# anrieff/fray

Measured on AMD Instinct MI355X. Metric: Mrays/s (closest-hit + shadow rays) at 1920x1080, 64spp path trace, higher is better.
Workload: dtype f64

## Files before the change

### fray_amd/abi.py

```python
import ctypes as C

i32, u32, i64, u64, f32, f64 = C.c_int32, C.c_uint32, C.c_int64, C.c_uint64, C.c_float, C.c_double
P = C.POINTER

ABI_VERSION = 3

OK, E_ARG, E_PARSE, E_NODEVICE, E_UNSUPPORTED, E_NOMEM, E_HIP, E_CANCELLED = 0, -1, -2, -3, -4, -5, -6, -7
GEOM_PLANE, GEOM_SPHERE, GEOM_CUBE, GEOM_MESH, GEOM_CSG = range(5)
TEX_CHECKER, TEX_BITMAP, TEX_BUMP, TEX_FRESNEL = range(4)
SHADER_CONST, SHADER_LAMBERT, SHADER_PHONG, SHADER_REFL, SHADER_REFR, SHADER_LAYERED = range(6)
LIGHT_POINT, LIGHT_RECT = range(2)
MODE_PRIMARY_ID, MODE_RENDER = 0, 1
FRAME_STATS = 1
OPTION_NAMES = ("pt_lanes", "pt_budget_mib", "speculate_fans", "fused_whitted_max", "fp_contract", "seed_table_mib", "skip_null_segments",
                "segment_planes", "certified_segments")
FIGURE_NAMES = ("contracted_launches", "shadow_segments", "segment_plane_nodes", "certified_segments_eligible", "shadow_segments_certified",
                "shadow_nodes_skipped", "seed_table_bytes", "seed_launches", "seed_planes_reused", "batch_lanes", "whitted_path",
                "pt_budget_effective_mib", "scene_updates", "scene_update_bytes", "arena_bytes", "fans_filed", "fan_children",
                "fan_children_looked_up", "fans_given_up")


class Transform(C.Structure):
    _fields_ = [("offset", f64 * 3), ("m", f64 * 9), ("invM", f64 * 9)]

# ... 126 lines not shown
        return {n: getattr(self, n) for n, _ in self._fields_ if n != "rgb"}


PROGRESS_FN = C.CFUNCTYPE(C.c_int, C.c_void_p, P(Progress))


class Progressive(C.Structure):
    _fields_ = [("fn", PROGRESS_FN), ("user", C.c_void_p), ("preview_ms", f64)]


class ShadeRequest(C.Structure):
    _fields_ = [("seed", u32), ("spp", i32), ("sample_first", i32), ("rng_skip", i32), ("flags", i32), ("_pad", i32),
                ("keys", C.c_void_p)]


class Adaptive(C.Structure):
    _fields_ = [("min_spp", i32), ("_pad", i32), ("threshold", f64), ("err_floor", f64), ("rungs", i32), ("_pad2", i32),
                ("samples", u64)]


ACCUM_CHANNELS = 4


class Samples(C.Structure):
    _fields_ = [("sample_first", i32), ("sample_count", i32), ("samples_done", i32), ("_pad", i32)]


class Denoise(C.Structure):
    _fields_ = [("levels", i32), ("demodulate", i32), ("sigma_luminance", C.c_float), ("sigma_normal", C.c_float),
                ("sigma_depth", C.c_float), ("sigma_albedo", C.c_float)]


FEAT_CHANNELS = 10
MOTION_CHANNELS = 8


class View(C.Structure):
    _fields_ = [("pos", f32 * 3), ("right", f32 * 3), ("up", f32 * 3), ("front", f32 * 3), ("tan_x", C.c_float), ("tan_y", C.c_float),
                ("width", i32), ("height", i32)]


class Temporal(C.Structure):
    _fields_ = [("demodulate", i32), ("max_history", i32), ("variance_history", i32), ("alpha_min", C.c_float), ("film_offset", C.c_float),
                ("plane_tolerance", C.c_float), ("normal_min_dot", C.c_float)]


class Change(C.Structure):
    _fields_ = [("radius", i32), ("gain", C.c_float)]


HISTORY_CHANNELS = 12
HISTORY_SPLIT_CHANNELS = 20


STRUCTS = {"frayhip_transform": Transform, "frayhip_geom_ref": GeomRef, "frayhip_node": Node,
           "frayhip_plane": Plane, "frayhip_sphere": Sphere, "frayhip_cube": Cube,
           "frayhip_csg": Csg, "frayhip_triangle": Triangle, "frayhip_kdnode": KDNode,
           "frayhip_mesh": Mesh, "frayhip_texture": Texture, "frayhip_shader": Shader,
           "frayhip_layer": Layer, "frayhip_light": Light, "frayhip_camera": Camera,
           "frayhip_settings": Settings, "frayhip_environment": Environment,
           "frayhip_scene_desc": SceneDesc, "frayhip_frame": Frame, "frayhip_stats": Stats,
           "frayhip_progress": Progress, "frayhip_progressive": Progressive,
           "frayhip_shade_request": ShadeRequest, "frayhip_adaptive": Adaptive, "frayhip_samples": Samples,
           "frayhip_view": View}

VP = C.c_void_p
SYMBOLS = {
    "frayhip_scene_parse": (C.c_int, [C.c_char_p, P(VP)]),
    "frayhip_host_scene_desc": (P(SceneDesc), [VP]),
    "frayhip_host_scene_free": (None, [VP]),
    "frayhip_init": (C.c_int, [C.c_int]),
    "frayhip_scene_create": (C.c_int, [P(SceneDesc), P(VP)]),
    "frayhip_scene_destroy": (None, [VP]),
    "frayhip_scene_set_view": (C.c_int, [VP, P(Camera), P(Settings)]),
    "frayhip_scene_update": (C.c_int, [VP, P(SceneDesc)]),
    "frayhip_transform_identity": (C.c_int, [P(Transform)]),
    "frayhip_transform_scale": (C.c_int, [P(Transform), f64, f64, f64]),
    "frayhip_transform_rotate": (C.c_int, [P(Transform), f64, f64, f64]),
    "frayhip_transform_translate": (C.c_int, [P(Transform), f64, f64, f64]),
    "frayhip_light_begin_frame": (C.c_int, [P(Light)]),
    "frayhip_shader_begin_frame": (C.c_int, [P(Shader)]),
    "frayhip_scene_set_option": (C.c_int, [VP, C.c_char_p, i64]),
    "frayhip_scene_get_option": (C.c_int, [VP, C.c_char_p, P(i64)]),
    "frayhip_render": (C.c_int, [VP, P(Frame), VP, VP, VP, P(Stats)]),
    "frayhip_render_device": (C.c_int, [VP, P(Frame), VP, VP, VP, VP, P(Stats)]),
    "frayhip_render_progressive": (C.c_int, [VP, P(Frame), P(Progressive), VP, VP, VP, P(Stats)]),
    "frayhip_render_device_progressive": (C.c_int, [VP, P(Frame), P(Progressive), VP, VP, VP, VP, P(Stats)]),
    "frayhip_render_adaptive": (C.c_int, [VP, P(Frame), P(Adaptive), VP, VP, VP, P(Stats)]),
    "frayhip_render_device_adaptive": (C.c_int, [VP, P(Frame), P(Adaptive), VP, VP, VP, VP, P(Stats)]),
    "frayhip_render_samples": (C.c_int, [VP, P(Frame), P(Samples), P(Progressive), VP, VP, VP, P(Stats)]),
    "frayhip_render_samples_device": (C.c_int, [VP, P(Frame), P(Samples), P(Progressive), VP, VP, VP, VP, P(Stats)]),
    "frayhip_render_components": (C.c_int, [VP, P(Frame), P(Samples), P(Progressive), VP, VP, VP, VP, VP, VP, P(Stats)]),
    "frayhip_render_components_device": (C.c_int, [VP, P(Frame), P(Samples), P(Progressive), VP, VP, VP, VP, VP, VP, VP, P(Stats)]),
    "frayhip_render_features": (C.c_int, [VP, P(Frame), C.c_int, VP, P(Stats)]),
    "frayhip_render_features_device": (C.c_int, [VP, P(Frame), C.c_int, VP, VP, P(Stats)]),
    "frayhip_render_features_motion": (C.c_int, [VP, P(Frame), C.c_int, P(Transform), C.c_int, VP, VP, P(Stats)]),
    "frayhip_render_features_motion_device": (C.c_int, [VP, P(Frame), C.c_int, P(Transform), C.c_int, VP, VP, VP, P(Stats)]),
    "frayhip_denoise_defaults": (C.c_int, [P(Denoise)]),
    "frayhip_denoise": (C.c_int, [C.c_int, C.c_int, VP, VP, VP, P(Denoise), VP, P(Stats)]),
    "frayhip_denoise_device": (C.c_int, [C.c_int, C.c_int, VP, VP, VP, P(Denoise), VP, VP, P(Stats)]),
    "frayhip_denoise_signal": (C.c_int, [C.c_int, C.c_int, VP, VP, VP, P(Denoise), VP, P(Stats)]),
    "frayhip_denoise_signal_device": (C.c_int, [C.c_int, C.c_int, VP, VP, VP, P(Denoise), VP, VP, P(Stats)]),
    "frayhip_view_from_camera": (C.c_int, [P(Camera), C.c_int, C.c_int, P(View)]),
    "frayhip_temporal_defaults": (C.c_int, [P(Temporal)]),
    "frayhip_temporal_accumulate": (C.c_int, [C.c_int, C.c_int, VP, VP, P(View), VP, P(Temporal), VP, VP, VP, P(Stats)]),
    "frayhip_temporal_accumulate_device": (C.c_int, [C.c_int, C.c_int, VP, VP, P(View), VP, P(Temporal), VP, VP, VP, VP, P(Stats)]),
    "frayhip_temporal_accumulate_motion": (C.c_int, [C.c_int, C.c_int, VP, VP, VP, P(View), VP, P(Temporal), VP, VP, VP, P(Stats)]),
    "frayhip_temporal_accumulate_motion_device": (C.c_int, [C.c_int, C.c_int, VP, VP, VP, P(View), VP, P(Temporal), VP, VP, VP, VP, P(Stats)]),
    "frayhip_temporal_accumulate_split": (C.c_int, [C.c_int, C.c_int, VP, VP, VP, VP, P(View), VP, P(Temporal), P(Temporal), VP, VP, VP, VP, VP, P(Stats)]),
    "frayhip_temporal_accumulate_split_device": (C.c_int, [C.c_int, C.c_int, VP, VP, VP, VP, P(View), VP, P(Temporal), P(Temporal), VP, VP, VP, VP, VP, VP,
                                                           P(Stats)]),
    "frayhip_change_defaults": (C.c_int, [P(Change)]),
    "frayhip_change_frame": (C.c_int, [C.c_int, C.c_int, VP, VP, VP, P(Change), VP, P(Stats)]),
    "frayhip_change_frame_device": (C.c_int, [C.c_int, C.c_int, VP, VP, VP, P(Change), VP, VP, P(Stats)]),
    "frayhip_temporal_accumulate_adaptive": (C.c_int, [C.c_int, C.c_int, VP, VP, VP, VP, P(View), VP, P(Temporal), VP, VP, VP, P(Stats)]),
    "frayhip_temporal_accumulate_adaptive_device": (C.c_int, [C.c_int, C.c_int, VP, VP, VP, VP, P(View), VP, P(Temporal), VP, VP, VP, VP, P(Stats)]),
    "frayhip_temporal_accumulate_split_adaptive": (C.c_int, [C.c_int, C.c_int, VP, VP, VP, VP, VP, VP, P(View), VP, P(Temporal), P(Temporal), VP, VP, VP, VP,
                                                             VP, P(Stats)]),
    "frayhip_temporal_accumulate_split_adaptive_device": (C.c_int, [C.c_int, C.c_int, VP, VP, VP, VP, VP, VP, P(View), VP, P(Temporal), P(Temporal), VP, VP,
                                                                    VP, VP, VP, VP, P(Stats)]),
    "frayhip_camera_rays": (C.c_int, [VP, i64, VP, C.c_int, VP, VP]),
    "frayhip_camera_rays_device": (C.c_int, [VP, i64, VP, C.c_int, VP, VP, VP]),
    "frayhip_trace_rays": (C.c_int, [VP, i64, VP, VP, C.c_int, VP, VP, VP, P(Stats)]),
    "frayhip_trace_rays_device": (C.c_int, [VP, i64, VP, VP, C.c_int, VP, VP, VP, VP, P(Stats)]),
    "frayhip_visible": (C.c_int, [VP, i64, VP, VP, C.c_int, VP, P(Stats)]),
    "frayhip_visible_device": (C.c_int, [VP, i64, VP, VP, C.c_int, VP, VP, P(Stats)]),
    "frayhip_shade_rays": (C.c_int, [VP, i64, VP, VP, P(ShadeRequest), VP, P(Stats)]),
    "frayhip_shade_rays_device": (C.c_int, [VP, i64, VP, VP, P(ShadeRequest), VP, VP, P(Stats)]),
    "frayhip_bucket_count": (C.c_int, [C.c_int, C.c_int, C.c_int, C.c_int]),
    "frayhip_pack_buckets_device": (C.c_int, [VP, VP, C.c_int, C.c_int, C.c_int, C.c_int, C.c_int, VP]),
    "frayhip_unpack_buckets_device": (C.c_int, [VP, VP, C.c_int, C.c_int, C.c_int, C.c_int, C.c_int, VP]),
    "frayhip_bucket_xy": (C.c_int, [C.c_int, C.c_int, C.c_int, C.POINTER(C.c_int), C.POINTER(C.c_int)]),
    "frayhip_comm_available": (C.c_int, []),
    "frayhip_comm_library": (C.c_char_p, []),
    "frayhip_comm_unique_id": (C.c_int, [VP]),
    "frayhip_comm_create": (C.c_int, [VP, C.c_int, C.c_int, P(VP)]),
    "frayhip_comm_from_nccl": (C.c_int, [VP, C.c_int, C.c_int, P(VP)]),
    "frayhip_comm_ranks": (C.c_int, [VP]),
    "frayhip_comm_destroy": (None, [VP]),
    "frayhip_gather_buckets": (C.c_int, [VP, VP, C.c_int, C.c_int, C.c_int, C.c_int, VP]),
    "frayhip_to_rgb32": (C.c_int, [VP, VP, C.c_int]),
    "frayhip_save_bmp": (C.c_int, [C.c_char_p, VP, C.c_int, C.c_int]),
    "frayhip_debug_rng": (C.c_int, [u32, C.c_int, VP, VP, VP, C.c_int]),
    "frayhip_debug_libm": (C.c_int, [C.c_int, VP, VP, VP, VP, VP]),
    "frayhip_debug_arith": (C.c_int, [C.c_int, C.c_int, VP, VP, VP]),
    "frayhip_last_error": (C.c_char_p, []),
    "frayhip_abi_version": (C.c_int, []),
    "frayhip_sizeof": (C.c_int, [C.c_char_p]),
}


def bind(lib):
    for name, (res, args) in SYMBOLS.items():
        fn = getattr(lib, name)
        fn.restype = res
        fn.argtypes = args
    return lib
```

### fray_amd/csrc/capi.hip

```cpp
#include <hip/hip_runtime.h>

#include <algorithm>
#include <chrono>
#include <cstddef>
#include <cmath>
#include <cstring>
#include <string>
#include <vector>
#include <functional>
#include <cstdlib>


#include "entry_support.hpp"
#include "dev_rng.hpp"
#include "dev_pack.hpp"
#include "scene_arena.hpp"

namespace {

using frayhip_detail::set_error;

void put3(double* o, const double* p) { o[0] = p[0]; o[1] = p[1]; o[2] = p[2]; }
}

// ... 147 lines not shown
    SeedTable& T = sc->seedTab;
    if (T.d) (void)hipFree(T.d);
    T.d = nullptr;
    T.bytes = 0;
    T.valid.clear();
    T.serving = false;
}

void seed_table_begin(frayhip_scene* sc, const DFrame& F, int nItems, int spp)
{
    SeedTable& T = sc->seedTab;
    if (!sc->seedTableCapBytes) { seed_table_free(sc); T.keyed = false; return; }
    if (nItems <= 0 || spp <= 0) return;
    const int32_t key[7] = {F.W, F.H, F.BW, F.BH, F.bucketFirst, F.bucketStride, F.nBuckets};
    const size_t planeBytes = (size_t)nItems * sizeof(uint32_t);
    if (!T.keyed || memcmp(key, T.key, sizeof key) != 0 || F.seed != T.seed || nItems != T.nItems) {
        memcpy(T.key, key, sizeof key);
        T.seed = F.seed; T.nItems = nItems; T.keyed = true; T.noGrow = false;
        T.valid.assign(T.bytes / planeBytes, 0);
    }
    const size_t need = (size_t)spp * planeBytes;
    if (need > sc->seedTableCapBytes) return;
    if (T.valid.size() < (size_t)spp) {
        if (T.noGrow) return;
        uint32_t* d = nullptr;
        if (hipMalloc((void**)&d, need) != hipSuccess) {
            (void)hipGetLastError();
            seed_table_free(sc);
            T.noGrow = true;
            return;
        }
        size_t held = 0;
        for (size_t s = 0; s < T.valid.size(); s++) if (T.valid[s]) held = s + 1;
        if (held && hipMemcpy(d, T.d, held * planeBytes, hipMemcpyDeviceToDevice) != hipSuccess) { (void)hipGetLastError(); std::fill(T.valid.begin(), T.valid.end(), (unsigned char)0); }
        if (T.d) (void)hipFree(T.d);
        T.d = d;
        T.bytes = need;
        T.valid.resize((size_t)spp, 0);
    }
    T.serving = true;
}

hipEvent_t pool_event(std::vector<hipEvent_t>& pool, size_t i)
{
    while (pool.size() <= i) {
        hipEvent_t e = nullptr;
        hipError_t rc = hipEventCreate(&e);
        if (rc != hipSuccess) { set_error(std::string("hipEventCreate: ") + hipGetErrorString(rc)); return nullptr; }
        pool.push_back(e);
    }
    return pool[i];
}

int bad(const char* who, const std::string& why)
{
    set_error(std::string(who) + ": " + why);
    return FRAYHIP_E_ARG;
}
int unsupported(const char* who, const std::string& why)
{
    set_error(std::string(who) + ": " + why);
    return FRAYHIP_E_UNSUPPORTED;
}

int frame_spp(const frayhip_scene* s)
{
    int spp = s->settings.wantAA ? 5 : 1;
    if (s->camera.dof) spp = std::max(spp, s->camera.numDOFSamples);
    if (s->settings.gi) spp = std::max(spp, s->settings.numPaths);
    return spp;
}

DScene frame_scene(const frayhip_scene* s)
{
    const frayhip_settings& set = s->settings;
    DScene S = s->S;
    S.ambient[0] = set.ambientLight[0]; S.ambient[1] = set.ambientLight[1]; S.ambient[2] = set.ambientLight[2];
    S.maxTraceDepth = set.maxTraceDepth;
    S.gi = set.gi;
    S.saturation = set.saturation;
    S.skipNullSegments = s->skipNullSegments ? 1 : 0;
    S.segmentPlanes = s->segmentPlanes ? 1 : 0;
    S.certifiedSegments = (s->certifiedSegments && s->segmentPlanes && S.segCertAll) ? 1 : 0;
    return S;
}

DFrame frame_record(const frayhip_scene* s, int bucketFirst, int bucketStride, uint32_t seed)
{
    DFrame F = frame_grid(s->settings.frameWidth, s->settings.frameHeight);
    F.bucketStride = bucketStride > 0 ? bucketStride : 1;
    F.bucketFirst = bucketFirst;
    F.nBuckets = frayhip_bucket_count(F.W, F.H, F.bucketFirst, F.bucketStride);
    F.spp = frame_spp(s);
    F.seed = seed;
    F.jitter = (s->camera.dof || s->settings.gi) ? 1 : 0;
    return F;
}

int check_bucket_range(const char* who, int nBuckets) { return nBuckets < 0 ? bad(who, "bad bucket_first / bucket_stride") : FRAYHIP_OK; }
int check_pixel_cap(const char* who, int nBuckets)
{
    if ((long long)nBuckets * 2304 > (1ll << 30)) return unsupported(who, "more than 2^30 pixels in one call (shard the frame with bucket_first / bucket_stride)");
    return FRAYHIP_OK;
}
int refuse_stereo(const char* who, const frayhip_scene* s) { return s->camera.stereoSeparation > 0 ? unsupported(who, "stereo frames are not supported") : FRAYHIP_OK; }
int refuse_long_generators(const char* who, const frayhip_scene* s, const char* by)
{
    if (s->settings.gi && s->settings.maxTraceDepth >= 0 && long_generators(s->settings.maxTraceDepth))
        return unsupported(who, std::string("path tracing with maxTraceDepth >= 20 (generators past 227 words) is not supported by ") + by);
    return FRAYHIP_OK;
}

frayhip_stats finish_stats(frayhip_scene* sc, const DStats* blocks, int nBlocks, size_t nTraceEvents, size_t nShadowEvents, std::chrono::steady_clock::time_point t0)
{
    frayhip_stats o{};
    for (int k = 0; k < nBlocks; k++) {
        const DStats& d = blocks[k];
        o.closest_rays += d.closest; o.shadow_rays += d.shadow; o.node_tests += d.node; o.kd_inner_visits += d.kdInner; o.leaf_refs += d.leafRefs;
        o.tri_tests += d.tri; o.prim_tests += d.prim; o.smooth_hits += d.smooth; o.samples += d.samples; o.texture_fetches += d.tex;
    }
    float ms = 0;
    (void)hipEventElapsedTime(&ms, sc->evA, sc->evB);
    o.ms_kernels = ms;
    auto sumEvents = [](const std::vector<hipEvent_t>& pool, size_t n) {
        double t = 0;
        for (size_t i = 0; i + 1 < n; i += 2) {
            float m2 = 0;
            (void)hipEventElapsedTime(&m2, pool[i], pool[i + 1]);
            t += m2;
        }
        return t;
    };
    o.ms_trace = sumEvents(sc->evPool, nTraceEvents);
    o.trace_launches = nTraceEvents / 2;
    o.ms_shadow = sumEvents(sc->evPoolShadow, nShadowEvents);
    o.shadow_launches = nShadowEvents / 2;
    o.ms_total = std::chrono::duration<double, std::milli>(std::chrono::steady_clock::now() - t0).count();
    return o;
}

}

struct SceneEdit {
    frayhip_arena::ArenaFacts F;
    std::vector<frayhip_arena::ArenaTable> tables;
    std::vector<frayhip_arena::ArenaMeshTables> meshTables;
    std::vector<int64_t> texelOffset;
    std::vector<unsigned char> host;
    std::vector<int64_t> hostOff;
    int32_t counts[11];
    int64_t nTexels;
    std::vector<frayhip_geom_ref> geoms;
    std::vector<frayhip_csg> csgs;
    std::vector<frayhip_mesh> meshes;
    std::vector<frayhip_texture> textures;
    frayhip_environment environment;
};

namespace frayhip_detail {
const DNode* host_nodes(const frayhip_scene* s) { return (const DNode*)(s->edit->host.data() + s->edit->hostOff[s->edit->F.tNodes]); }
}

namespace {

using frayhip_detail::kStatsBytes;
using frayhip_detail::grid_for;
// ... 166 lines not shown
    sc->kdMeshes = F.kdMeshes != 0;
    sc->textured = F.textured != 0;
    sc->whittedNeedsRecursion = F.whittedNeedsRecursion != 0;
    sc->lightDraws = F.lightDraws != 0;
    sc->lightSampleCount = F.lightSampleCount;
    sc->specFanMax = F.specFanMax;
}

}

extern "C" {

int frayhip_init(int device_id)
{
    int n = 0;
    hipError_t e = hipGetDeviceCount(&n);
    if (e != hipSuccess || n <= 0) { set_error("frayhip_init: no HIP device available"); return FRAYHIP_E_NODEVICE; }
    if (device_id < 0 || device_id >= n) { set_error("frayhip_init: bad device id"); return FRAYHIP_E_ARG; }
    HIP_TRY(hipSetDevice(device_id));
    return FRAYHIP_OK;
}

int frayhip_scene_create(const frayhip_scene_desc* desc, frayhip_scene** out)
{
    if (!desc || !out) { set_error("frayhip_scene_create: null argument"); return FRAYHIP_E_ARG; }
    if (desc->abi_version != FRAYHIP_ABI_VERSION) { set_error("frayhip_scene_create: ABI version mismatch"); return FRAYHIP_E_ARG; }
    const frayhip_scene_desc& d = *desc;
    {
        const std::string why = validate_desc(d);
        if (!why.empty()) { set_error(why); return FRAYHIP_E_ARG; }
    }
    {
        std::vector<int> levels(d.n_csgs, 0);
        std::function<int(int, int)> depth = [&](int i, int guard) -> int {
            if (guard > d.n_csgs) return 1 << 20;
            if (levels[i]) return levels[i];
            int m = 1;
            for (int side = 0; side < 2; side++) {
                const frayhip_geom_ref& g = d.geoms[side == 0 ? d.csgs[i].left : d.csgs[i].right];
                if (g.kind == FRAYHIP_GEOM_CSG) m = std::max(m, 1 + depth(g.index, guard + 1));
            }
            return levels[i] = m;
        };
        for (int i = 0; i < d.n_csgs; i++)
            if (depth(i, 0) > FRAY_CSG_DEPTH) {
                set_error("frayhip_scene_create: CSG operands nested more than " + std::to_string(FRAY_CSG_DEPTH) + " levels deep are not implemented on the device path");
                return FRAYHIP_E_UNSUPPORTED;
            }
    }
    frayhip_arena::ArenaBuilt B;
    frayhip_arena::arena_build(d, B);
    frayhip_scene* sc = new frayhip_scene();
    commit_facts(sc, B.F);
    if (hipMalloc(&sc->d_arena, B.host.size() ? B.host.size() : 256) != hipSuccess) {
        set_error("frayhip_scene_create: hipMalloc failed (no device?)");
        delete sc;
        return FRAYHIP_E_NODEVICE;
    }
    {
        unsigned char* const base = (unsigned char*)sc->d_arena;
        std::vector<unsigned char*> stage(B.tables.size());
        std::vector<const unsigned char*> addr(B.tables.size());
        for (size_t t = 0; t < B.tables.size(); t++) { stage[t] = B.host.data() + B.tables[t].off; addr[t] = base + B.tables[t].off; }
        frayhip_arena::arena_place(B.F, B.meshTables.data(), B.texelOffset.data(), stage.data(), addr.data(), sc->S);
    }
    hipError_t e = hipMemcpy(sc->d_arena, B.host.data(), B.host.size(), hipMemcpyHostToDevice);
    if (e != hipSuccess) { set_error(std::string("frayhip_scene_create: upload failed: ") + hipGetErrorString(e)); (void)hipFree(sc->d_arena); delete sc; return FRAYHIP_E_NODEVICE; }
    sc->arena_bytes = B.host.size();
    sc->edit = make_scene_edit(d, B);
    sc->camera = d.camera;
    sc->settings = d.settings;
    if (hipMalloc((void**)&sc->d_stats, kStatsBytes) != hipSuccess || hipMalloc((void**)&sc->d_qmeta, 3 * FRAY_PT_LANES * sizeof(QMeta)) != hipSuccess ||
        hipEventCreate(&sc->evA) != hipSuccess || hipEventCreate(&sc->evB) != hipSuccess || !create_lanes(sc)) {
        set_error("frayhip_scene_create: could not allocate the per-scene device state");
        frayhip_scene_destroy(sc);
        return FRAYHIP_E_NOMEM;
    }
    if (const char* e = getenv("FRAYHIP_PT_LANES")) { long v = atol(e); if (v >= 1 && v <= FRAY_PT_LANES) sc->ptLanes = (int)v; }
    if (const char* e = getenv("FRAYHIP_SPECULATE_FANS")) sc->speculateFans = atol(e) != 0;
    if (const char* e = getenv("FRAYHIP_FP_CONTRACT")) sc->fpContract = atol(e) == 1;
    if (const char* e = getenv("FRAYHIP_SKIP_NULL_SEGMENTS")) sc->skipNullSegments = atol(e) != 0;
    if (const char* e = getenv("FRAYHIP_SEGMENT_PLANES")) sc->segmentPlanes = atol(e) != 0;
    if (const char* e = getenv("FRAYHIP_CERTIFIED_SEGMENTS")) sc->certifiedSegments = atol(e) != 0;
    if (const char* e = getenv("FRAYHIP_FUSED_WHITTED_MAX")) { long v = atol(e); if (v >= 0 && v <= 1024) sc->fusedWhittedMax = (int)v; }
    if (const char* e = getenv("FRAYHIP_CSG_LANES")) { long v = atol(e); if (v >= 1 && v <= FRAY_PT_LANES) sc->csgLanes = (int)v; }
    if (const char* e = getenv("FRAYHIP_SEED_TABLE_MIB")) { long v = atol(e); if (v >= 0 && v <= (1 << 20)) sc->seedTableCapBytes = (size_t)v << 20; }
    if (const char* e = getenv("FRAYHIP_PT_BUDGET_MIB")) { long v = atol(e); if (v >= 1 && v <= (1 << 20)) { sc->ptBudgetBytes = (size_t)v << 20; sc->ptBudgetEff = 0; } }
    *out = sc;
    return FRAYHIP_OK;
}

int frayhip_scene_get_option(frayhip_scene* s, const char* name, int64_t* value)
{
    if (!s || !name || !value) { set_error("frayhip_scene_get_option: null argument"); return FRAYHIP_E_ARG; }
    const std::string n(name);
    if (n == "pt_lanes") *value = s->ptLanes;
    else if (n == "pt_budget_mib") *value = (int64_t)(s->ptBudgetBytes >> 20);
    else if (n == "speculate_fans") *value = s->speculateFans ? 1 : 0;
    else if (n == "fp_contract") *value = s->fpContract ? 1 : 0;
    else if (n == "contracted_launches") *value = s->lastContracted;
    else if (n == "skip_null_segments") *value = s->skipNullSegments ? 1 : 0;
    else if (n == "shadow_segments") *value = s->lastShadowSegments;
    else if (n == "segment_planes") *value = s->segmentPlanes ? 1 : 0;
    else if (n == "segment_plane_nodes") *value = s->S.nSegNodes;
    else if (n == "certified_segments") *value = s->certifiedSegments ? 1 : 0;
    else if (n == "certified_segments_eligible") *value = s->S.segCertAll;
    else if (n == "shadow_segments_certified") *value = s->lastShadowCertified;
    else if (n == "shadow_nodes_skipped") *value = s->lastShadowNodesSkipped;
    else if (n == "seed_table_mib") *value = (int64_t)(s->seedTableCapBytes >> 20);
    else if (n == "seed_table_bytes") *value = (int64_t)s->seedTab.bytes;
    else if (n == "seed_launches") *value = s->lastSeedLaunches;
    else if (n == "seed_planes_reused") *value = s->lastSeedReused;
    else if (n == "batch_lanes") *value = s->lastBatchLanes;
    else if (n == "whitted_path") *value = s->lastWhittedPath;
    else if (n == "fused_whitted_max") *value = s->fusedWhittedMax;
    else if (n == "pt_budget_effective_mib") *value = (int64_t)(frayhip_detail::work_budget(s) >> 20);
    else if (n == "scene_updates") *value = s->sceneUpdates;
    else if (n == "scene_update_bytes") *value = s->sceneUpdateBytes;
    else if (n == "arena_bytes") *value = (int64_t)s->arena_bytes;
    else if (n == "fans_filed") *value = s->lastFans[0];
    else if (n == "fan_children") *value = s->lastFans[1];
    else if (n == "fan_children_looked_up") *value = s->lastFans[2];
    else if (n == "fans_given_up") *value = s->lastFans[3];
    else { set_error("frayhip_scene_get_option: unknown option " + n); return FRAYHIP_E_ARG; }
    return FRAYHIP_OK;
}

int frayhip_scene_set_option(frayhip_scene* s, const char* name, int64_t value)
{
    if (!s || !name) { set_error("frayhip_scene_set_option: null argument"); return FRAYHIP_E_ARG; }
    if (s->rendering) { set_error("frayhip_scene_set_option: the scene is rendering a frame"); return FRAYHIP_E_ARG; }
    const std::string n(name);
    if (n == "pt_lanes") {
        if (value < 1 || value > FRAY_PT_LANES) { set_error("frayhip_scene_set_option: pt_lanes must be 1.." + std::to_string(FRAY_PT_LANES)); return FRAYHIP_E_ARG; }
        s->ptLanes = (int)value;
    } else if (n == "pt_budget_mib") {
        if (value < 1 || value > (1 << 20)) { set_error("frayhip_scene_set_option: pt_budget_mib must be 1..1048576"); return FRAYHIP_E_ARG; }
        s->ptBudgetBytes = (size_t)value << 20;
        s->ptBudgetEff = 0;
    } else if (n == "speculate_fans") {
        if (value != 0 && value != 1) { set_error("frayhip_scene_set_option: speculate_fans must be 0 or 1"); return FRAYHIP_E_ARG; }
        s->speculateFans = value != 0;
    } else if (n == "fused_whitted_max") {
        if (value < 0 || value > 1024) { set_error("frayhip_scene_set_option: fused_whitted_max must be 0..1024"); return FRAYHIP_E_ARG; }
        s->fusedWhittedMax = (int)value;
    } else if (n == "fp_contract") {
        if (value != 0 && value != 1) { set_error("frayhip_scene_set_option: fp_contract must be 0 or 1"); return FRAYHIP_E_ARG; }
        s->fpContract = value != 0;
    } else if (n == "seed_table_mib") {
        if (value < 0 || value > (1 << 20)) { set_error("frayhip_scene_set_option: seed_table_mib must be 0..1048576"); return FRAYHIP_E_ARG; }
        s->seedTableCapBytes = (size_t)value << 20;
        if (s->seedTab.bytes > s->seedTableCapBytes) { frayhip_detail::seed_table_free(s); s->seedTab.keyed = false; }
    } else if (n == "skip_null_segments") {
        if (value != 0 && value != 1) { set_error("frayhip_scene_set_option: skip_null_segments must be 0 or 1"); return FRAYHIP_E_ARG; }
        s->skipNullSegments = value != 0;
    } else if (n == "segment_planes") {
        if (value != 0 && value != 1) { set_error("frayhip_scene_set_option: segment_planes must be 0 or 1"); return FRAYHIP_E_ARG; }
        s->segmentPlanes = value != 0;
    } else if (n == "certified_segments") {
        if (value != 0 && value != 1) { set_error("frayhip_scene_set_option: certified_segments must be 0 or 1"); return FRAYHIP_E_ARG; }
        s->certifiedSegments = value != 0;
    } else {
        set_error("frayhip_scene_set_option: unknown option " + n);
        return FRAYHIP_E_ARG;
    }
    return FRAYHIP_OK;
}

int frayhip_scene_set_view(frayhip_scene* s, const frayhip_camera* camera, const frayhip_settings* settings)
{
    if (!s) { set_error("frayhip_scene_set_view: null scene"); return FRAYHIP_E_ARG; }
    if (s->rendering) { set_error("frayhip_scene_set_view: the scene is rendering a frame"); return FRAYHIP_E_ARG; }
    if (settings && (settings->frameWidth <= 0 || settings->frameHeight <= 0)) { set_error("frayhip_scene_set_view: bad frame size"); return FRAYHIP_E_ARG; }
    if (camera) s->camera = *camera;
    if (settings) s->settings = *settings;
    return FRAYHIP_OK;
}

int frayhip_scene_update(frayhip_scene* s, const frayhip_scene_desc* desc)
{
    if (!s || !desc) { set_error("frayhip_scene_update: null argument"); return FRAYHIP_E_ARG; }
    if (s->rendering) { set_error("frayhip_scene_update: the scene is rendering a frame"); return FRAYHIP_E_ARG; }
    if (desc->abi_version != FRAYHIP_ABI_VERSION) { set_error("frayhip_scene_update: ABI version mismatch"); return FRAYHIP_E_ARG; }
    const frayhip_scene_desc& d = *desc;
    SceneEdit& E = *s->edit;
    if (const char* what = fixed_part_differs(E, d)) {
        set_error(std::string("frayhip_scene_update: ") + what + " differs from the description the scene was created from (only nodes, primitives, shaders, layers, lights and texture parameters can be edited)");
        return FRAYHIP_E_ARG;
    }
    {
        const std::string why = validate_editable(d, "frayhip_scene_update");
        if (!why.empty()) { set_error(why); return FRAYHIP_E_ARG; }
    }
    std::vector<unsigned char> next(E.host);
    frayhip_arena::ArenaFacts F = E.F;
    std::vector<unsigned char*> tab(E.tables.size());
    std::vector<const unsigned char*> addr(E.tables.size());
    for (size_t t = 0; t < E.tables.size(); t++) {
        tab[t] = E.hostOff[t] >= 0 ? next.data() + E.hostOff[t] : nullptr;
        addr[t] = (const unsigned char*)s->d_arena + E.tables[t].off;
    }
    frayhip_arena::arena_update(d, E.meshTables.data(), F, tab.data());
    DScene S = s->S;
    frayhip_arena::arena_place(F, E.meshTables.data(), E.texelOffset.data(), tab.data(), addr.data(), S);
    long long bytes = 0;
    for (int32_t t : frayhip_arena::arena_editable_tables(F)) {
        if (!E.tables[t].bytes) continue;
// ... 197 lines not shown
```

### fray_amd/csrc/dev_misscert.hpp

```cpp
#pragma once
#ifndef FRAY_CERT_FN
#define FRAY_CERT_FN __device__ __forceinline__
#endif
#ifndef FRAY_MISSCERT_SCALE
#define FRAY_MISSCERT_SCALE 1.0
#endif

FRAY_CERT_FN bool ray_surely_misses_box(double cx, double cy, double cz, double hx, double hy, double hz, double M,
                                        double sx, double sy, double sz, double dx, double dy, double dz)
{
    const double px = sx - cx, py = sy - cy, pz = sz - cz;
    const double sm = __builtin_fmax(__builtin_fmax(__builtin_fabs(sx), __builtin_fabs(sy)), __builtin_fabs(sz));
    const double eta = FRAY_MISSCERT_SCALE * 0x1p-22 * (sm + M);
    const double Hx = hx + eta, Hy = hy + eta, Hz = hz + eta;
    bool miss = (px > Hx && dx >= 0) || (px < -Hx && dx <= 0) || (py > Hy && dy >= 0) || (py < -Hy && dy <= 0) || (pz > Hz && dz >= 0) || (pz < -Hz && dz <= 0);
    const double pm = FRAY_MISSCERT_SCALE * 0x1p-40 * __builtin_fmax(__builtin_fmax(__builtin_fabs(px), __builtin_fabs(py)), __builtin_fabs(pz));
    const double g = 1.0 + FRAY_MISSCERT_SCALE * 0x1p-40;
    const double ax = __builtin_fabs(dx), ay = __builtin_fabs(dy), az = __builtin_fabs(dz);
    miss = miss || __builtin_fabs(dy * pz - dz * py) > (az * Hy + ay * Hz) * g + pm;
    miss = miss || __builtin_fabs(dx * pz - dz * px) > (az * Hx + ax * Hz) * g + pm;
    miss = miss || __builtin_fabs(dx * py - dy * px) > (ay * Hx + ax * Hy) * g + pm;
    return miss;
}

FRAY_CERT_FN bool ray_surely_misses_box_f32(float cx, float cy, float cz, float hx, float hy, float hz, float M,
                                            float ox, float oy, float oz, float dx, float dy, float dz, float omax, float dsum)
{
    const float px = ox - cx, py = oy - cy, pz = oz - cz;
    const float pmax = __builtin_fmaxf(__builtin_fmaxf(__builtin_fabsf(px), __builtin_fabsf(py)), __builtin_fabsf(pz));
    const float slack = (float)FRAY_MISSCERT_SCALE * 0x1p-19f * (omax + pmax);
    const float eta = (float)FRAY_MISSCERT_SCALE * 0x1p-21f * (omax + M) + slack;
    const float Hx = hx + eta, Hy = hy + eta, Hz = hz + eta;
    bool miss = (px > Hx && dx >= 0) || (px < -Hx && dx <= 0) || (py > Hy && dy >= 0) || (py < -Hy && dy <= 0) || (pz > Hz && dz >= 0) || (pz < -Hz && dz <= 0);
    const float g = 1.0f + (float)FRAY_MISSCERT_SCALE * 0x1p-20f, sl = slack * dsum;
    const float ax = __builtin_fabsf(dx), ay = __builtin_fabsf(dy), az = __builtin_fabsf(dz);
    miss = miss || __builtin_fabsf(dy * pz - dz * py) > (az * Hy + ay * Hz) * g + sl;
    miss = miss || __builtin_fabsf(dx * pz - dz * px) > (az * Hx + ax * Hz) * g + sl;
    miss = miss || __builtin_fabsf(dx * py - dy * px) > (ay * Hx + ax * Hy) * g + sl;
    return miss;
}
```

### fray_amd/csrc/dev_scene.hpp

```cpp
#pragma once
#include <stdint.h>
#include "frayhip.h"
#include "dev_tricert.hpp"
#include "dev_segcert.hpp"

#ifdef __HIP_DEVICE_COMPILE__
#define FRAY_RO __attribute__((address_space(4)))
#else
#define FRAY_RO
#endif

#define FRAY_CSG_MAX 30
#ifndef FRAY_CSG_DEPTH
#define FRAY_CSG_DEPTH 16
#endif

#define FRAY_KD_LDS_STACK 16
#define FRAY_KD_MAX_DEPTH 72

struct DXform { double off[3]; double m[9]; double inv[9]; };

struct DTri;
struct DNode {
    DXform T;
// ... 24 lines not shown
    double A[3];
    double N[3];
    double AC[3];
    double AB[3];
    int32_t index;
    int32_t pad;
};

struct DTriAttr {
    double nA[3], nB[3], nC[3];
    double tA[2], tB[2], tC[2];
    double dNdx[3], dNdy[3];
};

struct alignas(16) DKd {
    union {
        double split;
        struct { int32_t triBegin, triCount; };
    };
    int32_t child0;
    int32_t meta;
};
struct DKdBox { double lo[3], hi[3]; };

struct DMesh {
    double bmin[3], bmax[3];
    const FRAY_RO DTri* tris;
    const FRAY_RO DTriAttr* attrs;
    const FRAY_RO DKd* kd;
    const FRAY_RO DKdBox* kdBox;
    const FRAY_RO int32_t* refs;
    const FRAY_RO DTri* ltris;
    int32_t nTris, hasKd, smooth, culling, hasUV, pad;
    double boxMax;
    const FRAY_RO DTri32* ltris32;
    double ref[3];
};

struct DTexture {
    int32_t kind, width, height, pad;
    float color1[3], color2[3];
    double scaling, bumpIntensity, ior;
    const FRAY_RO float* texels;
};

struct DShader {
    int32_t kind, texture;
    float color[3], specularColor[3], mult[3];
    int32_t numSamples;
    double exponent, specularMultiplier, glossiness, deflectionScaling, ior;
    int32_t layerBegin, layerCount;
    int32_t usesUV, pad;
};

struct DLayer { int32_t shader, texture; float opacity[3]; int32_t pad; };

struct DLight {
    int32_t kind, xSubd, ySubd, pad;
    float color[3], power;
    double pos[3];
    DXform T;
    double center[3];
    double area;
    double areaXsize, areaYsize;
};

struct DEnv {
    int32_t present, loaded;
    int32_t width[6], height[6];
    const FRAY_RO float* face[6];
};

struct DCamera {
    double topLeft[3], topRight[3], bottomLeft[3];
    double frontDir[3], upDir[3], rightDir[3], pos[3];
    double w, h, apertureSize, focalPlaneDist, stereoSeparation;
    float leftMask[3], rightMask[3];
    int32_t dof, pad;
};

#define FRAY_MAX_GATES 8
#define FRAY_GATE_MIN_TRIS 6
struct DGate { double lo[3], hi[3]; float cf[3], hf[3]; float Mf; int32_t exact; };

struct DScene {
    const FRAY_RO DNode* nodes;
    const FRAY_RO DNodeX* nodesX;
    const FRAY_RO DGate* gates;
    int32_t nGates, gatesExact;
    const FRAY_RO DPlane* planes;
    const FRAY_RO DSphere* spheres;
    const FRAY_RO DCube* cubes;
    const FRAY_RO DCsg* csgs;
    const FRAY_RO DMesh* meshes;
    const FRAY_RO DShader* shaders;
    const FRAY_RO DLayer* layers;
    const FRAY_RO DTexture* textures;
    const FRAY_RO DLight* lights;
    DEnv env;
    int32_t nNodes, nLights;
    float probPickLight;
    float ambient[3];
    int32_t maxTraceDepth, gi;
    float saturation;
    const FRAY_RO DSegPlane* segPlanes;
    const FRAY_RO uint32_t* segNodeMasks;
    int32_t nSegPlanes, nSegNodes;
    int32_t segmentPlanes;
    int32_t skipNullSegments;
    int32_t segCertAll;
    int32_t certifiedSegments;
};

struct DFrame {
    int32_t W, H, BW, BH;
    int32_t bucketFirst, bucketStride, nBuckets , spp;
    uint32_t seed;
    int32_t jitter;
};

struct DStats {
    unsigned long long closest, shadow, node, kdInner, leafRefs, tri, prim, smooth, samples, tex, rngOverflow;
#ifdef FRAY_STAMPS
    unsigned long long stamp[24];
    unsigned long long stampLanes[24];
#endif
};
struct DCursors { unsigned int v[8][32]; };
```

### fray_amd/csrc/dev_trace.hpp

```cpp
#pragma once
#ifndef FRAY_IDENTITY_SKIP
#define FRAY_IDENTITY_SKIP 1
#endif
#ifndef FRAY_FILTER_STRAIGHT
#define FRAY_FILTER_STRAIGHT 1
#endif
#include "dev_math.hpp"
#include "dev_scene.hpp"
#include "dev_sort.hpp"
#define FRAY_CERT_SEQ() __builtin_amdgcn_sched_barrier(0)
#include "dev_boxcert.hpp"
#include "dev_misscert.hpp"
#include "dev_segcert.hpp"

#ifdef FRAY_LEAFSTAT
static __device__ unsigned long long g_leafStat[4];
#endif
struct Cnt {
    unsigned long long closest, shadow, node, kdInner, leafRefs, tri, prim, smooth, samples, tex;
    unsigned envelope;
};
template <int ST> FD void bump(unsigned long long& c, unsigned long long n = 1) { if (ST & 1) c += n; }
constexpr bool kd_variant(int st) { return (st & 6) != 0; }
constexpr bool tex_variant(int st) { return (st & 14) != 0; }
// ... 832 lines not shown
    V3 ip = ls + ldir * scaling;
    if (fabs(ip.x) > 0.5 || fabs(ip.z) > 0.5) return false;
    ip = mulM(ip, L.T.m) + ld3(L.T.off);
    dist = length(o - ip);
    return true;
}

FD void light_record(const FRAY_RO DLight& L, V3 o, V3 d, V3& ip, V3& norm)
{
    V3 ls = mulM(o - ld3(L.T.off), L.T.inv);
    V3 ldir = normalized(mulM(d, L.T.inv));
    double scaling = fray_div(fabs(ls.y), fabs(ldir.y));
    ip = mulM(ls + ldir * scaling, L.T.m) + ld3(L.T.off);
    norm = normalized(mulM(v3(0, -1, 0), L.T.m));
}

template <int ST>
FD void closest_hit(const DScene& S, V3 o, V3 d, HitT<ST>& best, Cnt& c, bool gateFree = false)
{
    bump<ST>(c.closest);
    best.node = -1;
    best.tri = -1;
    best.dist = 1e99;
    best.t = 0; best.l2 = 0; best.l3 = 0;
    const int nn = S.nNodes;
    LocalRay lr;
    lr.cls = -1;
    lr.haveRd = false;
    for (int i = 0; i < nn; i++) {
        double dist, t, l2 = 0, l3 = 0;
        int tri = -1;
        if constexpr (!(ST & 1)) { if (S.nodes[i].gated) { if (gateFree) continue; } }
        if constexpr ((ST & 2) != 0) {
            V3 ipl;
            LeafOut lo{0, 0};
            if (node_intersect<ST>(S, i, o, d, lr, dist, t, tri, l2, l3, &ipl, &lo, c) && dist < best.dist) {
                best.node = i; best.tri = tri; best.dist = dist; best.t = t; best.l2 = l2; best.l3 = l3;
                best.ipl = ipl; best.leafKind = lo.kind; best.leafIndex = lo.index;
            }
        } else if (node_intersect<ST>(S, i, o, d, lr, dist, t, tri, l2, l3, nullptr, nullptr, c) && dist < best.dist) {
            best.node = i; best.tri = tri; best.dist = dist; best.t = t; best.l2 = l2; best.l3 = l3;
        }
    }
    if ((ST & 1) && best.node >= 0) {
        const FRAY_RO DNode& W = S.nodes[best.node];
        if (W.geomKind == 3 && S.meshes[W.geomIndex].smooth) c.smooth++;
    }
    STAMP(6);
    const int nl = S.nLights;
    for (int i = 0; i < nl; i++) {
        double dist;
        if (light_intersect<ST>(S.lights[i], o, d, dist, c) && dist < best.dist) {
            best.node = -2 - i;
            best.dist = dist;
        }
    }
    STAMP(7);
}

FD uint32_t segment_skip_nodes(const DScene& S, V3 a, V3 b, bool live)
{
    const int nP = S.segmentPlanes ? S.nSegPlanes : 0;
    if (nP <= 0) return 0u;
    const V3 e = b - a;
    const double m = seg_cert_scale(a.x, a.y, a.z, b.x, b.y, b.z, e.x, e.y, e.z);
    const lanes_t all = lanes(true);
    uint32_t certified = 0;
    for (int p = 0; p < nP; p++) {
        const FRAY_RO DSegPlane& P = S.segPlanes[p];
        if (lanes(!live || seg_same_side(P.N[0], P.N[1], P.N[2], P.k, P.t0, P.t1, m, a.x, a.y, a.z, b.x, b.y, b.z)) == all) certified |= 1u << p;
    }
    uint32_t skipNodes = 0;
    const int nS = S.nSegNodes;
    for (int j = 0; j < nS; j++)
        if ((S.segNodeMasks[j] & ~certified) == 0u) skipNodes |= 1u << j;
    return skipNodes;
}

#ifdef __HIP__
#define FRAY_RCPF(x) __builtin_amdgcn_rcpf(x)
#else
#define FRAY_RCPF(x) (1.0f / (x))
#endif
FD uint32_t ray_gate_class(const DScene& S, V3 o, V3 d)
{
    const int ng = S.nGates;
    if (ng == 0) return 0u;
    const float ox = (float)o.x, oy = (float)o.y, oz = (float)o.z;
    if (S.gatesExact) {
        const float dx = (float)d.x, dy = (float)d.y, dz = (float)d.z;
        const float omax = fmaxf(fmaxf(fabsf(ox), fabsf(oy)), fabsf(oz)), dsum = fabsf(dx) + fabsf(dy) + fabsf(dz);
        uint32_t first = 0;
        for (int g = ng - 1; g >= 0; g--) {
            const FRAY_RO DGate& G = S.gates[g];
            if (!ray_surely_misses_box_f32(G.cf[0], G.cf[1], G.cf[2], G.hf[0], G.hf[1], G.hf[2], G.Mf, ox, oy, oz, dx, dy, dz, omax, dsum)) first = (uint32_t)g + 1u;
        }
        return !(omax < 1e9f) && !first ? 1u : first;
    }
    const float rx = FRAY_RCPF((float)d.x), ry = FRAY_RCPF((float)d.y), rz = FRAY_RCPF((float)d.z);
    uint32_t first = 0;
    for (int g = ng - 1; g >= 0; g--) {
        const FRAY_RO DGate& G = S.gates[g];
        const float ax = ((float)G.lo[0] - ox) * rx, bx = ((float)G.hi[0] - ox) * rx;
        const float ay = ((float)G.lo[1] - oy) * ry, by = ((float)G.hi[1] - oy) * ry;
        const float az = ((float)G.lo[2] - oz) * rz, bz = ((float)G.hi[2] - oz) * rz;
        const float t0 = fmaxf(fmaxf(fminf(ax, bx), fminf(ay, by)), fmaxf(fminf(az, bz), 0.0f));
        const float t1 = fminf(fminf(fmaxf(ax, bx), fmaxf(ay, by)), fmaxf(az, bz));
        if (!(t0 > t1 * 1.0001f + 1e-3f)) first = (uint32_t)g + 1u;
    }
    return first;
}

FD bool segment_certified(const DScene& S, V3 a, V3 b)
{
    const int nP = S.nSegPlanes;
    const V3 e = b - a;
    const double m = seg_cert_scale(a.x, a.y, a.z, b.x, b.y, b.z, e.x, e.y, e.z);
    bool ok = m == m;
    for (int p = 0; p < nP; p++) {
        const FRAY_RO DSegPlane& P = S.segPlanes[p];
        ok = ok & seg_same_side(P.N[0], P.N[1], P.N[2], P.k, P.t0, P.t1, m, a.x, a.y, a.z, b.x, b.y, b.z);
    }
    return ok;
}
FD bool segment_surely_visible(const DScene& S, V3 a, V3 b, uint32_t gateClass)
{
    return S.certifiedSegments && gateClass == 0u && segment_certified(S, a, b);
}

template <int ST, bool GATES = false, bool SEGP = false>
FD bool visible(const DScene& S, V3 a, V3 b, Cnt& c, bool gateFree = false, uint32_t skipNodes = 0u)
{
    bump<ST>(c.shadow);
    V3 d = b - a;
    const double maxDist = length(d);
    d = d * fray_rcp(maxDist);
    const int nn = S.nNodes;
    LocalRay lr;
    lr.cls = -1;
    lr.haveRd = false;
    for (int i = 0; i < nn; i++) {
        double dist, t, l2, l3;
        int tri;
        LeafOut lo;
        if constexpr (GATES && !(ST & 1)) { if (S.nodes[i].gated) { if (gateFree) continue; } }
        if constexpr (SEGP) { const int sn = S.nodes[i].segNode; if (sn && ((skipNodes >> (sn - 1)) & 1u)) continue; }
        if (node_intersect<ST>(S, i, a, d, lr, dist, t, tri, l2, l3, nullptr, (ST & 2) ? &lo : nullptr, c) && dist < maxDist) return false;
    }
    return true;
}
```

### fray_amd/csrc/kernels.hpp

```cpp
#pragma once
#include "dev_shade.hpp"
#include "dev_whitted.hpp"
#include "dev_queues.hpp"
#include <type_traits>

#ifndef FRAY_PRIMARY_WAVES
#define FRAY_PRIMARY_WAVES 5
#endif
#ifndef FRAY_WHITTED_WAVES
#define FRAY_WHITTED_WAVES 3
#endif
#ifndef FRAY_WHITTED_REFILL
#define FRAY_WHITTED_REFILL 64
#endif
#ifndef FRAY_CSG_WAVES
#define FRAY_CSG_WAVES 3
#endif
constexpr int waves_for(int st, int n) { return (st & 2) ? (FRAY_CSG_WAVES < n ? FRAY_CSG_WAVES : n) : ((st & 1) && n > 2 ? n - 1 : n); }
#ifndef FRAY_MT_EARLY
#define FRAY_MT_EARLY 160
#endif
#ifndef FRAY_WH_SHADE_WAVES
#define FRAY_WH_SHADE_WAVES 4
#endif
// ... 618 lines not shown
    if ((threadIdx.x & 63) < 24) { atomicAdd(&st->stamp[threadIdx.x & 63], g_stampAcc[threadIdx.x >> 6][threadIdx.x & 63]); atomicAdd(&st->stampLanes[threadIdx.x & 63], g_stampLanes[threadIdx.x >> 6][threadIdx.x & 63]); }
#endif
    if (ST & 1) flush_stats(st, c);
    if ((ST & 2) && c.envelope) atomicAdd(&st->rngOverflow, 1ull);
}

static __global__ __launch_bounds__(256) void k_wh_gather(DScene S, WhittedQueue Q, size_t N, size_t slots, float* __restrict__ radL, float* __restrict__ radR)
{
    for (size_t e = (size_t)blockIdx.x * blockDim.x + threadIdx.x; e < N; e += (size_t)gridDim.x * blockDim.x) {
        C3 result = c3(Q.base[3 * e], Q.base[3 * e + 1], Q.base[3 * e + 2]);
        if (Q.hit[e]) {
            size_t t = e;
            const int nl = S.nLights;
            for (int li = 0; li < nl; li++) {
                const int ns = light_num_samples(S.lights[li]);
                C3 sum = c3(0, 0, 0);
                for (int k = 0; k < ns; k++, t += N)
                    if (Q.vis[t]) sum = sum + c3(Q.rr[t], Q.rg[t], Q.rb[t]);
                result = result + sum / (float)ns;
            }
        }
        float* out = e < slots ? radL + 3 * e : radR + 3 * (e - slots);
        out[0] = result.r; out[1] = result.g; out[2] = result.b;
    }
}

template <class G>
struct PathStateT {
    V3 o, d;
    C3 pm;
    uint32_t slot;
    int depth;
    unsigned flags;
    G rnd, tab;
};
typedef PathStateT<Mt> PathState;
FD Mt& cursor(Mt& g) { return g; }
FD Mt& cursor(MtPath& g) { return g.r; }
FD const Mt& cursor(const Mt& g) { return g; }
FD const Mt& cursor(const MtPath& g) { return g.r; }

template <int ST>
FD uint32_t ray_sort_class(V3 d, uint32_t gate)
{
    const uint32_t g = (d.x < 0 ? 1u : 0u) | (d.y < 0 ? 2u : 0u) | (d.z < 0 ? 4u : 0u);
    if constexpr ((ST & 2) != 0) { if (gate) return 8u + (gate - 1u < 6u ? gate - 1u : 6u); }
    return (g ^ (g >> 1) ^ (g >> 2)) | (gate ? 8u : 0u);
}
template <bool STORE_CLS, class G>
FD void path_store(const PathQueue& Q, uint32_t i, const PathStateT<G>& s, uint32_t cls)
{
    PathRec* r = Q.rec + i;
    r->o[0] = s.o.x; r->o[1] = s.o.y; r->o[2] = s.o.z;
    r->d[0] = s.d.x; r->d[1] = s.d.y; r->d[2] = s.d.z;
    r->pm[0] = s.pm.r; r->pm[1] = s.pm.g; r->pm[2] = s.pm.b;
    r->slot = s.slot;
    r->depthFlags = (uint32_t)s.depth | (s.flags << 16);
    const Mt &g = cursor(s.rnd), &t = cursor(s.tab);
    r->rnd[0] = g.j; r->rnd[1] = g.a; r->rnd[2] = g.b;
    r->tab[0] = t.j; r->tab[1] = t.a; r->tab[2] = t.b;
    if constexpr (STORE_CLS) Q.cls[i] = (unsigned char)cls;
}
template <class G>
FD void path_load_ray(const PathQueue& Q, uint32_t i, PathStateT<G>& s)
{
    const PathRec* r = Q.rec + i;
    s.o = v3(r->o[0], r->o[1], r->o[2]);
    s.d = v3(r->d[0], r->d[1], r->d[2]);
}
template <class G>
FD void path_load_rest(const PathQueue& Q, uint32_t i, PathStateT<G>& s)
{
    const PathRec* r = Q.rec + i;
    s.pm = c3(r->pm[0], r->pm[1], r->pm[2]);
    s.slot = r->slot;
    uint32_t df = r->depthFlags;
    s.depth = (int)(df & 0xffffu);
    s.flags = df >> 16;
    Mt &g = cursor(s.rnd), &t = cursor(s.tab);
    g.j = r->rnd[0]; g.a = r->rnd[1]; g.b = r->rnd[2];
    t.j = r->tab[0]; t.a = r->tab[1]; t.b = r->tab[2];
}

static __global__ __launch_bounds__(1024) void k_scan(QMeta* m0, QMeta* m1, unsigned long long* shadowTotal)
{
    QMeta* m = blockIdx.x == 0 ? m0 : m1;
    __shared__ uint32_t part[1024];
    const uint32_t nSeg = m->nSeg;
    const uint32_t per = (nSeg + 1023u) / 1024u;
    const uint32_t b = threadIdx.x * per;
    uint32_t sum = 0;
    for (uint32_t k = 0; k < per; k++) if (b + k < nSeg) sum += m->cnt[b + k];
    part[threadIdx.x] = sum;
    __syncthreads();
    for (uint32_t d = 1; d < 1024; d <<= 1) {
        uint32_t v = threadIdx.x >= d ? part[threadIdx.x - d] : 0;
        __syncthreads();
        part[threadIdx.x] += v;
        __syncthreads();
    }
    uint32_t run = part[threadIdx.x] - sum;
    for (uint32_t k = 0; k < per; k++)
        if (b + k < nSeg) { m->off[b + k] = run; run += m->cnt[b + k]; }
    if (threadIdx.x == 1023) {
        m->off[nSeg] = part[1023]; m->n = part[1023];
        if (blockIdx.x == 1 && shadowTotal) *shadowTotal += part[1023];
    }
}

static __global__ void k_meta_dense(QMeta* m, uint32_t n)
{
    if (blockIdx.x == 0 && threadIdx.x == 0) { m->n = n; m->chunk = n; m->nSeg = 1; m->certFront = 0; m->nf[0] = n; m->off[0] = 0; m->off[1] = n; }
}

FD uint32_t seg_first(const FRAY_RO uint32_t* off, uint32_t nSeg, uint32_t begin)
{
    uint32_t lo = 0, hi = nSeg;
    while (hi - lo > 1) {
        const uint32_t mid = (lo + hi) >> 1;
        if (off[mid] <= begin) lo = mid; else hi = mid;
    }
    return lo;
}
FD uint32_t seg_slot_of(uint32_t s, uint32_t chunk, uint32_t e, uint32_t nf) { return s * chunk + (e < nf ? e : chunk - 1u - (e - nf)); }
#define FRAY_FRONT_BIT 0x80000000u
FD uint32_t seg_map(const FRAY_RO uint32_t* off, const FRAY_RO uint32_t* nf, uint32_t nSeg, uint32_t chunk, uint32_t base, uint32_t di, bool live, uint32_t& seg)
{
    while (seg + 1 < nSeg && off[seg + 1] <= base) seg++;
    uint32_t i = 0, s = seg, lo = off[s];
    for (;;) {
        const uint32_t hi = off[s + 1];
        if (live && di >= lo && di < hi) i = seg_slot_of(s, chunk, di - lo, nf[s]) | (di - lo < nf[s] ? FRAY_FRONT_BIT : 0u);
        if (hi >= base + 64u || s + 1 >= nSeg) break;
        s++;
        lo = hi;
    }
    return i;
}

#ifndef FRAY_SORT
#define FRAY_SORT 1
#endif
#ifndef FRAY_SORT_N
#define FRAY_SORT_N 1024
#endif
#ifdef FRAY_SORT_BY_MATERIAL
constexpr bool sort_variant(int) { return true; }
#else
#ifndef FRAY_SORT_CSG
#define FRAY_SORT_CSG 0
#endif
constexpr bool sort_variant(int st) { return (st & 6) == 4 || (FRAY_SORT_CSG && (st & 2) != 0); }
#endif
FD void wave_lds_sync()
{
    __builtin_amdgcn_fence(__ATOMIC_RELEASE, "wavefront");
    __builtin_amdgcn_wave_barrier();
    __builtin_amdgcn_fence(__ATOMIC_ACQUIRE, "wavefront");
}
template <class KeyOf>
FD void sort_share(const FRAY_RO uint32_t* off, const FRAY_RO uint32_t* nf, uint32_t nSeg, uint32_t chunk, uint32_t b0, uint32_t b1, uint32_t& seg,
                   uint32_t* buf, uint32_t* cnt, KeyOf keyOf)
{
    const uint32_t lane = threadIdx.x & 63u;
    if (lane < 16) cnt[lane] = 0;
    wave_lds_sync();
    uint32_t s1 = seg;
    for (uint32_t base = b0; base < b1; base += 64u) {
        const uint32_t di = base + lane;
        const bool live = di < b1;
        const uint32_t i = seg_map(off, nf, nSeg, chunk, base, di, live, s1) & ~FRAY_FRONT_BIT;
        if (live) atomicAdd(cnt + keyOf(i), 1u);
    }
    wave_lds_sync();
    {
        const uint32_t v = lane < 16 ? cnt[lane] : 0u;
        uint32_t inc = v;
        for (int d = 1; d < 16; d <<= 1) { const uint32_t t = __shfl_up(inc, d, 64); if ((int)lane >= d) inc += t; }
        wave_lds_sync();
        if (lane < 16) cnt[lane] = inc - v;
    }
    wave_lds_sync();
    uint32_t s2 = seg;
    for (uint32_t base = b0; base < b1; base += 64u) {
        const uint32_t di = base + lane;
        const bool live = di < b1;
        const uint32_t raw = seg_map(off, nf, nSeg, chunk, base, di, live, s2);
        if (live) buf[atomicAdd(cnt + keyOf(raw & ~FRAY_FRONT_BIT), 1u)] = raw;
    }
// ... 47 lines not shown
                }
            } else {
                ps.rnd.j = SB.g[0][slot]; ps.rnd.a = SB.g[1][slot]; ps.rnd.b = SB.g[2][slot];
                ps.tab.j = SB.g[3][slot]; ps.tab.a = SB.g[4][slot]; ps.tab.b = SB.g[5][slot];
                ps.o = v3(SB.r[0][slot], SB.r[1][slot], SB.r[2][slot]);
                ps.d = v3(SB.r[3][slot], SB.r[4][slot], SB.r[5][slot]);
            }
            ps.pm = c3(1, 1, 1);
            ps.slot = slot;
            ps.depth = 0;
            ps.flags = 0;
            bump<ST>(c.samples);
            path_store<FRAY_SORT && sort_variant(ST)>(Q, slot, ps, ray_sort_class<ST>(ps.d, 0u));
        } else {
            PathRec* r = Q.rec + slot;
            r->d[0] = 0; r->d[1] = 0; r->d[2] = 0;
            r->depthFlags = FRAY_DEAD;
            if constexpr (FRAY_SORT && sort_variant(ST)) Q.cls[slot] = 15;
        }
        termCount[slot] = 0;
    }
    if (ST & 1) flush_stats(st, c);
}

struct WaveShare { uint32_t begin, end, chunk, w, W; };
FD WaveShare wave_share(uint32_t n)
{
    WaveShare r;
    r.W = gridDim.x * (blockDim.x >> 6);
    r.w = blockIdx.x * (blockDim.x >> 6) + (threadIdx.x >> 6);
    r.chunk = (((n + r.W - 1u) / r.W) + 63u) & ~63u;
    r.begin = r.w * r.chunk;
    r.end = r.begin + r.chunk < n ? r.begin + r.chunk : n;
    if (r.begin > n) r.begin = r.end = n;
    return r;
}


struct SegEnds { uint32_t begin, chunk, nF, nB; };
struct SegEndsShared { uint32_t begin, chunk; uint32_t* n; };
FD uint32_t seg_take(const SegEndsShared& E, bool back)
{
    const uint32_t k = atomicAdd(E.n + (back ? 1 : 0), 1u);
    return back ? E.begin + E.chunk - 1u - k : E.begin + k;
}
FD uint32_t seg_slot(const SegEnds& E, bool put, bool back)
{
    const uint32_t lane = threadIdx.x & 63u;
    const unsigned long long mF = __ballot(put && !back), mB = __ballot(put && back);
    const unsigned long long below = (1ull << lane) - 1ull;
    return back ? E.begin + E.chunk - 1u - (E.nB + (uint32_t)__popcll(mB & below)) : E.begin + E.nF + (uint32_t)__popcll(mF & below);
}
FD void seg_advance(SegEnds& E, bool put, bool back)
{
    E.nF += (uint32_t)__popcll(__ballot(put && !back));
    E.nB += (uint32_t)__popcll(__ballot(put && back));
}

template <int ST, bool BARY, class G>
FD void path_shade(const DScene& S, PathStateT<G>& ps, const HitT<ST>& h, const TermBuf& TB, DStats* st, const StereoBuf& SB, bool& cont, bool& shadow, uint32_t& shadowBack,
                   const ShadowQueue& SQ, const SegEndsShared& shadowEnds, Cnt& c)
{
    C3 own = c3(0, 0, 0);
    if (h.node <= -2) {
        own = (ps.flags & RF_DIFFUSE) ? c3(0, 0, 0) : light_color(S.lights[-2 - h.node]) * ps.pm;
        path_finish(TB, st, ps, SB);
    } else if (h.node < 0) {
        own = environment<ST>(S, ps.d, c) * ps.pm;
        path_finish(TB, st, ps, SB);
    } else {
        const FRAY_RO DNode& N = S.nodes[h.node];
        const FRAY_RO DShader& sh = S.shaders[N.shader];
        HitInfo info;
        finalize_hit<ST, BARY>(S, h, ps.o, ps.d, sh.usesUV || N.bumpTex >= 0, info);
        apply_bump<ST>(S, h.node, info, c);
        mt_skip(ps.tab, spawn_words(sh));
        {
            V3 sa, sb;
            C3 sc;
            shadow = nee_prepare(S, ps.d, info, ps.pm, sh, ps.rnd, ps.tab, sa, sb, sc, !(ST & 1) && S.skipNullSegments != 0);
            if (shadow) {
                bool planesPass = false;
                if constexpr (ST == 0 && FRAY_ARITH == 0) { if (S.certifiedSegments) planesPass = segment_certified(S, sa, sb); }
                shadowBack = ray_gate_class(S, sa, sb - sa);
                if constexpr (ST == 0) {
                    if (FRAY_ARITH == 0 ? planesPass && shadowBack == 0 : segment_surely_visible(S, sa, sb, shadowBack)) {
                        own = sc;
                        shadow = false;
                        atomicAdd(shadowEnds.n + 2, 1u);
                    }
                }
                if (ST != 0 || shadow) {
                    const uint32_t j = seg_take(shadowEnds, shadowBack != 0);
                    SQ.ax[j] = sa.x; SQ.ay[j] = sa.y; SQ.az[j] = sa.z;
                    SQ.bx[j] = sb.x; SQ.by[j] = sb.y; SQ.bz[j] = sb.z;
                    SQ.cr[j] = sc.r; SQ.cg[j] = sc.g; SQ.cb[j] = sc.b;
                    SQ.slot[j] = ps.slot;
                    if constexpr (FRAY_SORT && sort_variant(ST)) SQ.cls[j] = (unsigned char)ray_sort_class<ST>(sb - sa, shadowBack);
                }
            }
        }
        PathRay win, wout;
        win.o = ps.o; win.d = ps.d; win.depth = ps.depth; win.flags = ps.flags;
        C3 brdf;
        float pdf;
        spawn_ray(sh, info, win, ps.tab, wout, brdf, pdf);
        {
            ps.pm = ps.pm * brdf / pdf;
            ps.o = wout.o; ps.d = wout.d; ps.depth = wout.depth; ps.flags = wout.flags;
#ifdef FRAY_SORT_BY_MATERIAL
            ps.flags = (ps.flags & 0xffu) | ((sh.kind == 1 ? 0u : sh.kind == 3 ? 1u : sh.kind == 4 ? 2u : 3u) << 8);
#endif
            if (ps.depth > S.maxTraceDepth || intensity(ps.pm) < 0.01) path_finish(TB, st, ps, SB);
            else cont = true;
        }
    }
    if (!shadow) term_store(TB, ps.slot, own);
}

struct LongRng { uint32_t* cols; uint32_t nPaths; DFrame F; int nItems, s0; };
struct FirstArgs { DCamera C; DFrame F; int nItems, s0; uint32_t n; const uint32_t* x397; unsigned short* termCount; };
struct BounceArgs { DScene S; PathQueue Qin, Qout; ShadowQueue SQ; QMetaRO metaIn; QMeta* metaOut; QMeta* metaShadow; TermBuf TB; StereoBuf SB; LongRng LR; DStats* st; FirstArgs FA; unsigned long long* segCertified; };
#ifndef FRAY_ARITH
#define FRAY_ARITH 0
#endif
template <int ST, bool LONG, bool FIRST = false, int ARITH = FRAY_ARITH>
static __global__ __launch_bounds__(256, waves_for(ST, kd_variant(ST) ? FRAY_BOUNCE_WAVES : FRAY_BOUNCE_WAVES_NOKD)) void k_pt_bounce(BounceArgs A)
{
    static_assert(!(LONG && FIRST), "long generators start from k_pt_init");
    typedef typename std::conditional<LONG, MtPath, Mt>::type G;
    Cnt c = zero_cnt();
    const QMetaRO metaIn = A.metaIn;
    QMeta* const metaOut = A.metaOut;
    QMeta* const metaShadow = A.metaShadow;
    DStats* const st = A.st;
    const FRAY_RO uint32_t* off = FIRST ? nullptr : metaIn.p->off;
    const FRAY_RO uint32_t* nfIn = FIRST ? nullptr : metaIn.p->nf;
    const uint32_t nSeg = FIRST ? 1u : metaIn.p->nSeg, chunkIn = FIRST ? A.FA.n : metaIn.p->chunk;
    const bool certFront = !FIRST && metaIn.p->certFront != 0;
    const WaveShare ws = wave_share(FIRST ? A.FA.n : metaIn.p->n);
    const uint32_t lane = threadIdx.x & 63u;
    SegEnds outEnds{ws.begin, ws.chunk, 0, 0};
    __shared__ uint32_t shadowCount[4][ST == 0 ? 3 : 2];
    if (lane < (ST == 0 ? 3u : 2u)) shadowCount[threadIdx.x >> 6][lane] = 0;
    const SegEndsShared shadowEnds{ws.begin, ws.chunk, shadowCount[threadIdx.x >> 6]};
    uint32_t seg = (!FIRST && ws.begin < ws.end) ? seg_first(off, nSeg, ws.begin) : 0;
#ifdef FRAY_STAMPS
    stamp_begin();
#endif
    constexpr bool SORT = FRAY_SORT && !FIRST && sort_variant(ST);
    const uint32_t sortN = (uint32_t)FRAY_SORT_N;
    for (uint32_t b0 = ws.begin, b1 = 0; b0 < ws.end; b0 = b1) {
    b1 = (SORT && ws.end - b0 > sortN) ? b0 + sortN : ws.end;
    uint32_t* sorted = nullptr;
    if constexpr (SORT) {
        __shared__ uint32_t sortBuf[4][FRAY_SORT_N];
        __shared__ uint32_t sortCnt[4][16];
        sorted = sortBuf[threadIdx.x >> 6];
        const unsigned char* const cls = KARG(BounceArgs, kernel_args<BounceArgs>(), Qin).cls;
        sort_share(off, nfIn, nSeg, chunkIn, b0, b1, seg, sorted, sortCnt[threadIdx.x >> 6], [&](uint32_t i) { return (uint32_t)cls[i] & 15u; });
    }
    for (uint32_t base = b0; base < b1; base += 64u) {
        const FRAY_RO BounceArgs* AP = kernel_args<BounceArgs>();
        const FirstArgs& FA = KARG(BounceArgs, AP, FA);
        const DScene& S = KARG(BounceArgs, AP, S);
        const PathQueue& Qin = KARG(BounceArgs, AP, Qin);
        const PathQueue& Qout = KARG(BounceArgs, AP, Qout);
        const ShadowQueue& SQ = KARG(BounceArgs, AP, SQ);
        const TermBuf& TB = KARG(BounceArgs, AP, TB);
        const StereoBuf& SB = KARG(BounceArgs, AP, SB);
        const LongRng& LR = KARG(BounceArgs, AP, LR);
        const uint32_t di = base + lane;
        bool cont = false, shadow = false, gateFree = false;
        uint32_t shadowBack = 0;
        PathStateT<G> ps;
        bool live = di < b1;
        uint32_t i = di, seed0 = 0;
        if constexpr (FIRST) {
            if (live) {
                FA.termCount[di] = 0;
                int px, py;
                live = item_pixel(FA.F, (int)(di % (uint32_t)FA.nItems), px, py);
                if (live) {
                    seed0 = sample_seed(FA.F.seed, (uint32_t)py * (uint32_t)FA.F.W + (uint32_t)px, (uint32_t)(FA.s0 + (int)(di / (uint32_t)FA.nItems)));
                    Mt rnd = mt_seed_with(seed0, FA.x397[di]), tab = rnd;
                    const float ox = rng_float(rnd), oy = rng_float(rnd);
                    const double fx = (double)((float)px + ox), fy = (double)((float)py + oy);
                    if (FA.C.dof) dof_ray(FA.C, fx, fy, tab, ps.o, ps.d, 0); else screen_ray(FA.C, fx, fy, ps.o, ps.d, 0);
                }
            }
        } else {
            if constexpr (SORT) i = live ? sorted[di - b0] : 0u;
            else i = seg_map(off, nfIn, nSeg, chunkIn, base, di, live, seg);
            gateFree = certFront && (i & FRAY_FRONT_BIT);
            i &= ~FRAY_FRONT_BIT;
            if (live) {
                path_load_ray(Qin, i, ps);
                live = !(ps.d.x == 0 && ps.d.y == 0 && ps.d.z == 0);
            }
        }
        if (live) {
            STAMP(0);
            HitT<ST> h;
            closest_hit<ST>(S, ps.o, ps.d, h, c, gateFree);
            if constexpr (FIRST) {
                ps.pm = c3(1, 1, 1); ps.slot = di; ps.depth = 0; ps.flags = 0;
                ps.rnd = mt_seed_with(seed0, FA.x397[di]);
                ps.tab = ps.rnd;
                mt_skip(ps.rnd, 2);
                if (FA.C.dof) mt_skip(ps.tab, 4);
                bump<ST>(c.samples);
            } else {
                path_load_rest(Qin, i, ps);
            }
#ifdef FRAY_QCHECK
            if (ps.slot >= TB.nPaths) { atomicAdd(&st->rngOverflow, 1ull << 32); ps.slot = 0; ps.pm = c3(0, 0, 0); ps.depth = 0x7fff; }
            else Qin.rec[i].slot = 0xffffffffu;
#endif
            if constexpr (LONG) {
                int px, py;
                item_pixel(LR.F, (int)(ps.slot % (uint32_t)LR.nItems), px, py);
                const uint32_t sd = sample_seed(LR.F.seed, (uint32_t)py * (uint32_t)LR.F.W + (uint32_t)px, (uint32_t)(LR.s0 + (int)(ps.slot / (uint32_t)LR.nItems)));
                ps.rnd.seed = ps.tab.seed = sd;
                ps.rnd.stride = ps.tab.stride = LR.nPaths;
                ps.rnd.col = LR.cols + ps.slot;
                ps.tab.col = LR.cols + (size_t)624 * LR.nPaths + ps.slot;
            }
            STAMP(8);
            path_shade<ST, false>(S, ps, h, TB, st, SB, cont, shadow, shadowBack, SQ, shadowEnds, c);
            STAMP(10);
        }
        const uint32_t gate = cont ? ray_gate_class(S, ps.o, ps.d) : 0u;
        const bool back = gate != 0;
        const uint32_t slotOut = seg_slot(outEnds, cont, back);
#ifdef FRAY_SORT_BY_MATERIAL
        if (cont) path_store<true>(Qout, slotOut, ps, (ps.flags >> 8) & 3u);
#else
        if (cont) path_store<FRAY_SORT && sort_variant(ST)>(Qout, slotOut, ps, ray_sort_class<ST>(ps.d, gate));
#endif
        seg_advance(outEnds, cont, back);
        STAMP(13);
    }
    }
#ifdef FRAY_STAMPS
    if (lane < 24) { atomicAdd(&st->stamp[lane], g_stampAcc[threadIdx.x >> 6][lane]); atomicAdd(&st->stampLanes[lane], g_stampLanes[threadIdx.x >> 6][lane]); }
#endif
    if (lane == 0) {
        metaOut->cnt[ws.w] = outEnds.nF + outEnds.nB; metaOut->nf[ws.w] = outEnds.nF;
        metaShadow->cnt[ws.w] = shadowCount[threadIdx.x >> 6][0] + shadowCount[threadIdx.x >> 6][1]; metaShadow->nf[ws.w] = shadowCount[threadIdx.x >> 6][0];
        if constexpr (ST == 0) {
            unsigned long long* const total = KARG(BounceArgs, kernel_args<BounceArgs>(), segCertified);
            const uint32_t nCert = shadowCount[threadIdx.x >> 6][2];
            if (total && nCert) atomicAdd(total, (unsigned long long)nCert);
        }
    }
    if (blockIdx.x == 0 && threadIdx.x == 0) {
        metaOut->chunk = ws.chunk; metaOut->nSeg = ws.W; metaShadow->chunk = ws.chunk; metaShadow->nSeg = ws.W;
        metaOut->certFront = metaShadow->certFront = A.S.gatesExact ? 1u : 0u;
    }
    if (ST & 1) flush_stats(st, c);
    if ((ST & 2) && c.envelope) atomicAdd(&st->rngOverflow, 1ull);
}

struct ShadowArgs { DScene S; ShadowQueue SQ; QMetaRO meta; TermBuf TB; DStats* st; unsigned long long* segSkipped; };
template <int ST, int ARITH = FRAY_ARITH>
static __global__ __launch_bounds__(256, anyhit_waves(ST)) void k_pt_shadow(ShadowArgs A)
{
    Cnt c = zero_cnt();
    const QMetaRO meta = A.meta;
    DStats* const st = A.st;
    const FRAY_RO uint32_t* off = meta.p->off;
    const FRAY_RO uint32_t* nfIn = meta.p->nf;
    const uint32_t nSeg = meta.p->nSeg, chunkIn = meta.p->chunk;
    const bool certFront = meta.p->certFront != 0;
    const WaveShare ws = wave_share(meta.p->n);
    const uint32_t lane = threadIdx.x & 63u;
    if (ws.begin >= ws.end) return;
    uint32_t seg = seg_first(off, nSeg, ws.begin);
#ifdef FRAY_STAMPS
    stamp_begin();
#endif
    constexpr bool SORT = FRAY_SORT && sort_variant(ST);
    constexpr bool SEGP = identity_variant(ST) && !(ST & 1);
    uint32_t segSkipped = 0;
    const uint32_t sortN = (uint32_t)FRAY_SORT_N;
    for (uint32_t b0 = ws.begin, b1 = 0; b0 < ws.end; b0 = b1) {
    b1 = (SORT && ws.end - b0 > sortN) ? b0 + sortN : ws.end;
    uint32_t* sorted = nullptr;
    if constexpr (SORT) {
        __shared__ uint32_t sortBuf[4][FRAY_SORT_N];
        __shared__ uint32_t sortCnt[4][16];
        sorted = sortBuf[threadIdx.x >> 6];
        const unsigned char* const cls = KARG(ShadowArgs, kernel_args<ShadowArgs>(), SQ).cls;
        sort_share(off, nfIn, nSeg, chunkIn, b0, b1, seg, sorted, sortCnt[threadIdx.x >> 6], [&](uint32_t i) { return (uint32_t)cls[i] & 15u; });
    }
    for (uint32_t base = b0; base < b1; base += 64u) {
        const FRAY_RO ShadowArgs* AP = kernel_args<ShadowArgs>();
        const DScene& S = KARG(ShadowArgs, AP, S);
        const ShadowQueue& SQ = KARG(ShadowArgs, AP, SQ);
        const TermBuf& TB = KARG(ShadowArgs, AP, TB);
        const uint32_t di = base + lane;
        const bool live = di < b1;
        uint32_t i;
        if constexpr (SORT) i = live ? sorted[di - b0] : 0u;
        else i = seg_map(off, nfIn, nSeg, chunkIn, base, di, live, seg);
        const bool gateFree = certFront && (i & FRAY_FRONT_BIT);
        i &= ~FRAY_FRONT_BIT;
        if constexpr (SEGP) {
            V3 a = v3(0, 0, 0), b = a;
            if (live) { a = v3(SQ.ax[i], SQ.ay[i], SQ.az[i]); b = v3(SQ.bx[i], SQ.by[i], SQ.bz[i]); }
            const uint32_t skipNodes = segment_skip_nodes(S, a, b, live);
            segSkipped += (uint32_t)__builtin_popcount(skipNodes);
            if (live) {
                STAMP(0);
                const bool vis = certFront ? visible<ST, true, true>(S, a, b, c, gateFree, skipNodes) : visible<ST, false, true>(S, a, b, c, false, skipNodes);
// ... 138 lines not shown
```

### fray_amd/csrc/render_impl.hpp

```cpp
#pragma once
#include <algorithm>
#include <chrono>
#include <cstring>
#include <cstdio>

#include "accum.hpp"
#include "entry_support.hpp"
#include "kernels.hpp"

namespace frayhip_detail {

namespace {
unsigned char* carve_queue(unsigned char* p, size_t n, PathQueue& Q)
{
    Carve c{p};
    Q.rec = (PathRec*)c.take(n * sizeof(PathRec));
    Q.cls = c.take(n);
    return c.p;
}
size_t queue_bytes(size_t n) { return r256(n * sizeof(PathRec)) + r256(n); }
unsigned char* carve_shadow(unsigned char* p, size_t n, ShadowQueue& Q)
{
    Carve c{p};
    Q.ax = (double*)c.take(n * 8); Q.ay = (double*)c.take(n * 8); Q.az = (double*)c.take(n * 8);
    Q.bx = (double*)c.take(n * 8); Q.by = (double*)c.take(n * 8); Q.bz = (double*)c.take(n * 8);
    Q.cr = (float*)c.take(n * 4); Q.cg = (float*)c.take(n * 4); Q.cb = (float*)c.take(n * 4);
    Q.slot = (uint32_t*)c.take(n * 4);
    Q.cls = c.take(n);
    return c.p;
}
size_t shadow_bytes(size_t n) { return 6 * r256(n * 8) + 4 * r256(n * 4) + r256(n); }

template <int ST>
int pt_bounces(frayhip_scene* sc, const DScene& S, const PathQueue (&Q)[2], const ShadowQueue& SQ, TermBuf TB, int nBounce, int grid, hipStream_t stream,
               size_t& nTraceEvents, size_t& nShadowEvents)
{
    QMeta* meta = sc->d_qmeta;
    for (int b = 0; b < nBounce; b++) {
        const QMetaRO mIn{(const FRAY_RO QMeta*)(meta + (b & 1))}, mSh{(const FRAY_RO QMeta*)(meta + 2)};
        hipEvent_t ea = pool_event(sc->evPool, nTraceEvents), eb = pool_event(sc->evPool, nTraceEvents + 1);
        hipEvent_t ec = pool_event(sc->evPoolShadow, nShadowEvents), ed = pool_event(sc->evPoolShadow, nShadowEvents + 1);
        if (!ea || !eb || !ec || !ed) return FRAYHIP_E_NOMEM;
        TB.b = b;
        const BounceArgs BA{S, Q[b & 1], Q[(b + 1) & 1], SQ, mIn, meta + ((b + 1) & 1), meta + 2, TB, StereoBuf{}, LongRng{}, sc->d_stats, FirstArgs{}};
        HIP_TRY(hipEventRecord(ea, stream));
        hipLaunchKernelGGL((k_pt_bounce<ST, false>), dim3(grid), dim3(256), 0, stream, BA);
        HIP_TRY(hipEventRecord(eb, stream));
        nTraceEvents += 2;
        hipLaunchKernelGGL(k_scan, dim3(2), dim3(1024), 0, stream, meta + ((b + 1) & 1), meta + 2, (unsigned long long*)nullptr);
        HIP_TRY(hipEventRecord(ec, stream));
        hipLaunchKernelGGL(k_pt_shadow<ST>, dim3(grid), dim3(256), 0, stream, ShadowArgs{S, SQ, mSh, TB, sc->d_stats + 1, (unsigned long long*)((unsigned char*)sc->d_stats + kSegSkippedOffset)});
        HIP_TRY(hipEventRecord(ed, stream));
        nShadowEvents += 2;
    }
    return FRAYHIP_OK;
}

inline int seed_batch(frayhip_scene* sc, const DFrame& F, int nItems, int s0, int cn, uint32_t* scratch, hipStream_t ls, const uint32_t*& out)
{
    auto launch = [&](int a, int n, uint32_t* to) {
        hipLaunchKernelGGL(k_seed, dim3(seed_grid(((size_t)nItems * n + FRAY_SEED_CHAINS - 1) / FRAY_SEED_CHAINS)), dim3(256), 0, ls, F, nItems, a, n, to);
        sc->lastSeedLaunches++;
    };
    SeedTable& T = sc->seedTab;
    if (!T.serving) { launch(s0, cn, scratch); out = scratch; return FRAYHIP_OK; }
    for (int a = s0; a < s0 + cn;) {
        if (T.valid[a]) { sc->lastSeedReused++; a++; continue; }
        int n = 1;
        while (a + n < s0 + cn && !T.valid[a + n]) n++;
        launch(a, n, T.d + (size_t)a * nItems);
        HIP_TRY(hipGetLastError());
        std::fill(T.valid.begin() + a, T.valid.begin() + a + n, (unsigned char)1);
        a += n;
    }
    out = T.d + (size_t)s0 * nItems;
    return FRAYHIP_OK;
}

struct Batches {
    frayhip_scene* sc = nullptr;
    const Progress* prog = nullptr;
    std::chrono::steady_clock::time_point t0;
    DFrame F{};
    int nItems = 0;
    float* d_rgb = nullptr;
    size_t frameBytes = 0;
    float* sum = nullptr;
    AccumCall* acc = nullptr;
    int first = 0;
    int total = 1, chunk = 1, nBatches = 1, window = 1;
    int resolved = 1, samplesDone = 1;
    bool cancelled = false;
    double lastPreviewMs = 0;

    double elapsed_ms() const { return std::chrono::duration<double, std::milli>(std::chrono::steady_clock::now() - t0).count(); }
    int call(bool preview, bool final, const float* rgb) const
    {
        if (!prog->req->fn) return 0;
        frayhip_progress p{};
        p.samples_done = samplesDone; p.samples_total = total;
        p.batches_done = resolved; p.batches_total = nBatches;
        p.ms_elapsed = elapsed_ms();
        p.preview = preview ? 1 : 0; p.final = final ? 1 : 0;
        p.rgb = rgb;
        return prog->req->fn(prog->req->user, &p);
    }
    int samples_after(int r) const { return std::min(total, first + (r + 1) * chunk); }
    void mean(hipStream_t ls, int n, bool withNoise) const
    {
        if (acc) {
            launch_acc_mean(grid_for(nItems), ls, F, nItems, n, acc->accum, acc->accum2 ? acc->rgb1 : d_rgb, withNoise ? acc->noise : nullptr);
            if (acc->accum2) launch_acc_mean(grid_for(nItems), ls, F, nItems, n, acc->accum2, acc->rgb2, withNoise ? acc->noise2 : nullptr);
        }
        else hipLaunchKernelGGL(k_resolve_mean, dim3(grid_for(nItems)), dim3(256), 0, ls, F, nItems, n, (const float*)sum, d_rgb);
    }
    bool preview_due()
    {
        const double every = prog->req->preview_ms;
        if (every < 0 || !d_rgb) return false;
        const double now = elapsed_ms();
        if (every > 0 && now - lastPreviewMs < every) return false;
        lastPreviewMs = now;
        return true;
    }
    template <class Trace, class Resolve, class LaneOf>
    int run(Trace&& trace, Resolve&& resolve, LaneOf&& laneOf, hipEvent_t* evOrder)
    {
        if (!prog) {
            for (int j = 0; j < nBatches; j++) {
                if (const int rc = trace(j)) return rc;
                if (const int rc = resolve(j)) return rc;
                if (evOrder) HIP_TRY(hipEventRecord(evOrder[j % window], laneOf(j)));
// ... 257 lines not shown
                };
                auto resolve = [&](int j) -> int {
                    const int s0 = first + j * chunk, cn = std::min(chunk, spp - j * chunk);
                    if (acc) launch_acc_resolve(grid_for(nItems), stream, F, C, set.saturation, nItems, s0, cn, radL, stereo ? radR : nullptr, acc->accum);
                    else if (!direct) hipLaunchKernelGGL(k_pt_resolve, dim3(grid_for(nItems)), dim3(256), 0, stream, F, C, set.saturation, nItems, s0, cn, radL, stereo ? radR : nullptr, sum, d_rgb);
                    return FRAYHIP_OK;
                };
                B.sum = sum; B.chunk = chunk; B.nBatches = (spp + chunk - 1) / chunk;
                if (const int rc = B.run(trace, resolve, [&](int) { return stream; }, nullptr)) return rc;
            }
        } else if (nItems > 0) {
            if (set.maxTraceDepth > 2000) { set_error("frayhip_render: maxTraceDepth above 2000 is not supported (three launches per level and batch)"); return FRAYHIP_E_UNSUPPORTED; }
            const bool longRng = long_generators(set.maxTraceDepth);
            const size_t termBytes = (size_t)(set.maxTraceDepth + 2) * 12 + 2;
            const size_t perPath = 240 + termBytes + (longRng ? 2 * 624 * sizeof(uint32_t) : 0);
            int maxLanes = std::max(1, std::min(sc->ptLanes, FRAY_PT_LANES));
            if (ST & 2) maxLanes = std::max(1, std::min(maxLanes, sc->csgLanes));
            if (ST & 1) maxLanes = 1;
            const bool longRngW = long_generators(set.maxTraceDepth);
            const unsigned warmKey = 1u << ((longRngW ? 1 : 0) | (sc->fpContract ? 2 : 0) | (sc->camera.stereoSeparation > 0 ? 4 : 0));
            if (maxLanes > 1 && !(sc->warmMask & warmKey) && !getenv("FRAYHIP_NO_PRIME")) {
                HIP_TRY(hipMemsetAsync(sc->d_qmeta, 0, 3 * FRAY_PT_LANES * sizeof(QMeta), stream));
                HIP_TRY(hipStreamSynchronize(stream));
                for (int k = 0; k < maxLanes; k++) {
                    hipStream_t ws = k == 0 ? stream : sc->laneStream[k];
                    QMeta* m = sc->d_qmeta + 3 * k;
                    const QMetaRO mIn{(const FRAY_RO QMeta*)m};
                    BounceArgs BA{};
                    BA.S = S; BA.metaIn = mIn; BA.metaOut = m + 1; BA.metaShadow = m + 2; BA.st = sc->d_stats;
                    ShadowArgs SA{};
                    SA.S = S; SA.meta = mIn; SA.st = sc->d_stats + 1;
                    if (longRngW) hipLaunchKernelGGL((k_pt_bounce<ST, true>), dim3(1), dim3(256), 0, ws, BA);
                    else {
                        hipLaunchKernelGGL((k_pt_bounce<ST, false>), dim3(1), dim3(256), 0, ws, BA);
                        hipLaunchKernelGGL((k_pt_bounce<ST, false, true>), dim3(1), dim3(256), 0, ws, BA);
                    }
                    hipLaunchKernelGGL(k_pt_shadow<ST>, dim3(1), dim3(256), 0, ws, SA);
                    if constexpr (!(ST & 2)) {
                        if (sc->fpContract) { launch_bounce_contracted<ST>(1, ws, BA); launch_shadow_contracted<ST>(1, ws, SA); }
                    }
                    HIP_TRY(hipStreamSynchronize(ws));
                }
                sc->warmMask |= warmKey;
            }
            if (maxLanes > 3 && (size_t)nItems * (size_t)spp < ((size_t)24 << 20)) maxLanes = 3;
            const bool stereo = sc->camera.stereoSeparation > 0;
            int chunk = 0, nBatches = 0, nLanes = 0;
            size_t nPaths = 0, nQueue = 0, laneBytes = 0;
            if (first == 0) seed_table_begin(sc, F, nItems, spp);
            for (;;) {
                const bool tabled = sc->seedTab.serving;
                const size_t budget = std::max<size_t>(work_budget(sc) / perPath, 1);
                chunk = f->spp_chunk > 0 ? f->spp_chunk : (int)std::max<size_t>(1, budget / maxLanes / (size_t)nItems);
                if (chunk > spp) chunk = spp;
                if (f->spp_chunk <= 0 && spp >= 2 * maxLanes && chunk * maxLanes > spp) chunk = (spp + maxLanes - 1) / maxLanes;
                while (chunk > 1 && (size_t)nItems * chunk > ((size_t)1 << 30)) chunk /= 2;
                nBatches = (spp + chunk - 1) / chunk;
                nLanes = std::min(nBatches, maxLanes);
                nPaths = (size_t)nItems * chunk;
                nQueue = nPaths + (size_t)bounce_grid(nPaths, (ST & 2) != 0 && maxLanes == 1) * 4 * 128;
                laneBytes = 2 * queue_bytes(nQueue) + shadow_bytes(nQueue) + nPaths * 12 + (tabled ? 0 : nPaths * 4) + 4096 + nPaths * termBytes + 512 + (longRng ? nPaths * 2 * 624 * sizeof(uint32_t) + 256 : 0) +
                            (stereo ? nPaths * (12 + 6 * 8 + 6 * 4) + 16 * 256 : 0);
                const int rc = ensure_work_or_shrink(sc, (size_t)nLanes * laneBytes + (size_t)nItems * 12 + 4096, f->spp_chunk <= 0 && (chunk > 1 || nLanes > 1));
                if (rc == FRAYHIP_RETRY_SMALLER) { if (chunk == 1 && maxLanes > 1) maxLanes--; continue; }
                if (rc) return rc;
                if (tabled && !sc->seedTab.serving) continue;
                break;
            }
            sc->lastBatchLanes = nLanes;
            struct Lane {
                hipStream_t stream;
                PathQueue Q[2];
                ShadowQueue SQ;
                float *sampleRad, *sampleRadR;
                uint32_t* seedWords;
                uint32_t* mtCols;
                float* terms;
                unsigned short* termCount;
                StereoBuf SB;
                QMeta* meta;
                unsigned long long* segTotal;
                unsigned long long* segSkipped;
                unsigned long long* segCertified;
            } lane[FRAY_PT_LANES];
            unsigned char* p = (unsigned char*)sc->d_work;
            float* sum = (float*)p; p += ((size_t)nItems * 12 + 255) / 256 * 256;
            for (int k = 0; k < nLanes; k++) {
                Lane& L = lane[k];
                L.stream = k == 0 ? stream : sc->laneStream[k];
                L.meta = sc->d_qmeta + 3 * k;
                L.segTotal = (unsigned long long*)((unsigned char*)sc->d_stats + kSegTotalsOffset) + k;
                L.segSkipped = (unsigned long long*)((unsigned char*)sc->d_stats + kSegSkippedOffset) + k;
                L.segCertified = (unsigned long long*)((unsigned char*)sc->d_stats + kSegCertifiedOffset) + k;
                p = carve_queue(p, nQueue, L.Q[0]);
                p = carve_queue(p, nQueue, L.Q[1]);
                p = carve_shadow(p, nQueue, L.SQ);
                L.sampleRad = (float*)p; p += (nPaths * 12 + 255) / 256 * 256;
                L.seedWords = nullptr;
                if (!sc->seedTab.serving) { L.seedWords = (uint32_t*)p; p += (nPaths * 4 + 255) / 256 * 256; }
                L.terms = (float*)p; p += (nPaths * (size_t)(set.maxTraceDepth + 2) * 12 + 255) / 256 * 256;
                L.termCount = (unsigned short*)p; p += (nPaths * 2 + 255) / 256 * 256;
                L.mtCols = nullptr;
                if (longRng) { L.mtCols = (uint32_t*)p; p += (nPaths * 2 * 624 * sizeof(uint32_t) + 255) / 256 * 256; }
                L.SB = StereoBuf{};
                L.sampleRadR = nullptr;
                if (stereo) {
                    L.sampleRadR = (float*)p; p += (nPaths * 12 + 255) / 256 * 256;
                    for (int q = 0; q < 6; q++) { L.SB.r[q] = (double*)p; p += (nPaths * 8 + 255) / 256 * 256; }
                    for (int q = 0; q < 6; q++) { L.SB.g[q] = (uint32_t*)p; p += (nPaths * 4 + 255) / 256 * 256; }
                }
            }
            const StereoBuf SBnone{};
            const int nBounce = set.maxTraceDepth + 2;
            HIP_TRY(hipEventRecord(sc->evLaneStart, stream));
            for (int k = 1; k < nLanes; k++) HIP_TRY(hipStreamWaitEvent(sc->laneStream[k], sc->evLaneStart, 0));
            auto trace = [&](int batch) -> int {
                const int s0 = first + batch * chunk, cn = std::min(chunk, spp - batch * chunk);
                Lane& L = lane[batch % nLanes];
                hipStream_t ls = L.stream;
                const uint32_t* x397 = nullptr;
                if (const int rc = seed_batch(sc, F, nItems, s0, cn, L.seedWords, ls, x397)) return rc;
                for (int eye = 0; eye < (stereo ? 2 : 1); eye++) {
                    const bool fused = !stereo && !longRng;
                    float* rad = eye == 0 ? L.sampleRad : L.sampleRadR;
                    const StereoBuf& save = (stereo && eye == 0) ? L.SB : SBnone;
                    if (!fused) {
                        hipLaunchKernelGGL(k_meta_dense, dim3(1), dim3(64), 0, ls, L.meta, (uint32_t)((size_t)nItems * cn));
                        hipLaunchKernelGGL(k_pt_init<ST>, dim3(grid_for((size_t)nItems * cn)), dim3(256), 0, ls, S, C, F, nItems, s0, cn, L.Q[0],
                                           L.termCount, x397, L.SB, eye, sc->d_stats);
                    }
                    for (int b = 0; b < nBounce; b++) {
                        const QMetaRO mIn{(const FRAY_RO QMeta*)(L.meta + (b & 1))}, mSh{(const FRAY_RO QMeta*)(L.meta + 2)};
                        const int grid = bounce_grid((size_t)nItems * cn, (ST & 2) != 0 && nLanes == 1);
                        hipEvent_t ea = pool_event(sc->evPool, nTraceEvents), eb = pool_event(sc->evPool, nTraceEvents + 1);
                        hipEvent_t ec = pool_event(sc->evPoolShadow, nShadowEvents), ed = pool_event(sc->evPoolShadow, nShadowEvents + 1);
                        if (!ea || !eb || !ec || !ed) return FRAYHIP_E_NOMEM;
                        HIP_TRY(hipEventRecord(ea, ls));
                        const LongRng LR{L.mtCols, (uint32_t)nPaths, F, nItems, s0};
                        const TermBuf TB{L.terms, L.termCount, (uint32_t)nPaths, b};
                        const FirstArgs FA{C, F, nItems, s0, (uint32_t)((size_t)nItems * cn), x397, L.termCount};
                        const BounceArgs BA{S, L.Q[b & 1], L.Q[(b + 1) & 1], L.SQ, mIn, L.meta + ((b + 1) & 1), L.meta + 2, TB, save, LR, sc->d_stats, FA, L.segCertified};
                        bool contractedLaunch = false;
                        if constexpr (!(ST & 2)) {
                            if (sc->fpContract && !longRng && b > 0) { launch_bounce_contracted<ST>(grid, ls, BA); contractedLaunch = true; nContracted++; }
                        }
                        if (contractedLaunch) {}
                        else if (longRng) hipLaunchKernelGGL((k_pt_bounce<ST, true>), dim3(grid), dim3(256), 0, ls, BA);
                        else if (fused && b == 0) hipLaunchKernelGGL((k_pt_bounce<ST, false, true>), dim3(grid), dim3(256), 0, ls, BA);
                        else hipLaunchKernelGGL((k_pt_bounce<ST, false>), dim3(grid), dim3(256), 0, ls, BA);
                        HIP_TRY(hipEventRecord(eb, ls));
                        nTraceEvents += 2;
                        hipLaunchKernelGGL(k_scan, dim3(2), dim3(1024), 0, ls, L.meta + ((b + 1) & 1), L.meta + 2, L.segTotal);
                        HIP_TRY(hipEventRecord(ec, ls));
                        bool contractedShadow = false;
                        if constexpr (!(ST & 2)) {
                            if (sc->fpContract) { launch_shadow_contracted<ST>(grid, ls, ShadowArgs{S, L.SQ, mSh, TB, sc->d_stats + 1, L.segSkipped}); contractedShadow = true; nContracted++; }
                        }
                        if (!contractedShadow) hipLaunchKernelGGL(k_pt_shadow<ST>, dim3(grid), dim3(256), 0, ls, ShadowArgs{S, L.SQ, mSh, TB, sc->d_stats + 1, L.segSkipped});
                        HIP_TRY(hipEventRecord(ed, ls));
                        nShadowEvents += 2;
                    }
                    if (stereo) hipLaunchKernelGGL(k_pt_fold, dim3(grid_for((size_t)nItems * cn)), dim3(256), 0, ls, TermBuf{L.terms, L.termCount, (uint32_t)nPaths, 0},
                                                   (uint32_t)((size_t)nItems * cn), rad);
                }
                return FRAYHIP_OK;
            };
            auto resolve = [&](int batch) -> int {
                const int s0 = first + batch * chunk, cn = std::min(chunk, spp - batch * chunk);
                Lane& L = lane[batch % nLanes];
                hipStream_t ls = L.stream;
                if (batch > 0 && nLanes > 1) HIP_TRY(hipStreamWaitEvent(ls, sc->evResolved[(batch - 1) % nLanes], 0));
                if (acc && stereo) launch_acc_resolve(grid_for(nItems), ls, F, C, set.saturation, nItems, s0, cn, L.sampleRad, L.sampleRadR, acc->accum);
                else if (acc && acc->accum2) launch_acc_resolve_terms_split(grid_for(nItems), ls, F, nItems, s0, cn, TermBuf{L.terms, L.termCount, (uint32_t)nPaths, 0}, acc->accum, acc->accum2);
                else if (acc) launch_acc_resolve_terms(grid_for(nItems), ls, F, nItems, s0, cn, TermBuf{L.terms, L.termCount, (uint32_t)nPaths, 0}, acc->accum);
                else if (stereo) hipLaunchKernelGGL(k_pt_resolve, dim3(grid_for(nItems)), dim3(256), 0, ls, F, C, set.saturation, nItems, s0, cn, L.sampleRad, L.sampleRadR, sum, d_rgb);
                else hipLaunchKernelGGL(k_pt_resolve_terms, dim3(grid_for(nItems)), dim3(256), 0, ls, F, nItems, s0, cn, TermBuf{L.terms, L.termCount, (uint32_t)nPaths, 0}, sum, d_rgb);
                return FRAYHIP_OK;
            };
            B.sum = sum; B.chunk = chunk; B.nBatches = nBatches; B.window = nLanes;
            if (const int rc = B.run(trace, resolve, [&](int batch) { return lane[batch % nLanes].stream; }, sc->evResolved)) return rc;
            if (nLanes > 1) HIP_TRY(hipStreamWaitEvent(stream, sc->evResolved[(B.resolved - 1) % nLanes], 0));
        }
    } else {
        set_error("frayhip_render: unknown mode");
        return FRAYHIP_E_ARG;
    }
    B.finish(stream);
    HIP_TRY(hipGetLastError());
    HIP_TRY(hipEventRecord(sc->evB, stream));
    HIP_TRY(hipStreamSynchronize(stream));
    drain.armed = false;
    struct Back { DStats ds[2]; unsigned long long segTotal[FRAY_PT_LANES], segSkipped[FRAY_PT_LANES], segCertified[FRAY_PT_LANES]; } back;
    static_assert(offsetof(Back, segTotal) == kSegTotalsOffset && offsetof(Back, segSkipped) == kSegSkippedOffset && offsetof(Back, segCertified) == kSegCertifiedOffset,
                  "the shadow-queue totals, the skipped nodes and the certified segments follow the counter blocks");
    HIP_TRY(hipMemcpy(&back, sc->d_stats, sizeof back, hipMemcpyDeviceToHost));
    const DStats (&dsv)[2] = back.ds;
    sc->lastShadowSegments = 0;
    for (int k = 0; k < FRAY_PT_LANES; k++) sc->lastShadowSegments += (long long)back.segTotal[k];
    sc->lastShadowCertified = 0;
    for (int k = 0; k < FRAY_PT_LANES; k++) sc->lastShadowCertified += (long long)back.segCertified[k];
    sc->lastShadowSegments += sc->lastShadowCertified;
    sc->lastShadowNodesSkipped = 0;
    for (int k = 0; k < FRAY_PT_LANES; k++) sc->lastShadowNodesSkipped += (long long)back.segSkipped[k];
    {
        unsigned long long ft[4] = {0, 0, 0, 0};
        if (fanTotals) HIP_TRY(hipMemcpy(ft, fanTotals, sizeof ft, hipMemcpyDeviceToHost));
        for (int q = 0; q < 4; q++) sc->lastFans[q] = (long long)ft[q];
        sc->lastContracted = nContracted;
    }
#ifdef FRAY_LEAFSTAT
    {
        unsigned long long ls[4] = {0, 0, 0, 0}, zero[4] = {0, 0, 0, 0};
        (void)hipMemcpyFromSymbol(ls, HIP_SYMBOL(g_leafStat), sizeof ls);
        (void)hipMemcpyToSymbol(HIP_SYMBOL(g_leafStat), zero, sizeof zero);
        if (ls[0]) fprintf(stderr, "[leafstat] wave leaf phases %llu, all active lanes in ONE leaf %.1f %%, active lanes per phase %.1f, distinct leaves per phase %.2f\n",
                           ls[0], 100.0 * (double)ls[1] / (double)ls[0], (double)ls[2] / (double)ls[0], (double)ls[3] / (double)ls[0]);
    }
#endif
#ifdef FRAY_TILESTAT
    if (const char* out = getenv("FRAY_TILESTAT_OUT")) {
        std::vector<unsigned long long> ts(65536 * 8);
        (void)hipMemcpyFromSymbol(ts.data(), HIP_SYMBOL(g_tileStat), ts.size() * sizeof(unsigned long long));
        if (FILE* fp = fopen(out, "wb")) { fwrite(ts.data(), sizeof(unsigned long long), ts.size(), fp); fclose(fp); }
    }
#endif
#ifdef FRAY_STAMPS
    {
        static const char* names[24] = {"queue lookup + ray load / camera ray", "local ray (transform)", "root box test", "tree-less triangle loop", "KD walk: child tests", "other geometry (plane / sphere / KD leaf accept)",
                                        "node result + world distance", "lights", "load rest of path", "KD walk: climbs", "shading (finalize .. spawn / light loops)", "KD leaves: FP64 tests of the candidates",
                                        "k_whitted: cheap steps (returns, loop heads, pushes; pixel / sample set-up)", "queue stores / loop overhead", "k_whitted: rest of the trace step (attributes, bump)", "KD leaves: FP32 filter",
                                        "CsgOp: bounding-box certificate", "CsgOp over two plain operands (no machine)", "CsgOp machine: plain operand asked", "CsgOp machine: answers delivered (sort, in / out walk)", "CsgOp machine: pushes, mesh operand's remainder", "", "", ""};
        for (int q = 0; q < 2; q++) {
            double tot = 0;
            for (int k = 0; k < 24; k++) tot += (double)dsv[q].stamp[k];
            fprintf(stderr, "[stamps] %s: total %.4g wave-cycles\n", q == 0 ? "closest-hit kernel (k_pt_bounce / k_primary / k_wh_shade)" : "any-hit kernel (k_pt_shadow / k_wh_visible)", tot);
            for (int k = 0; k < 24; k++) if (dsv[q].stamp[k]) fprintf(stderr, "[stamps]   %2d %-36s %6.2f %%   lanes %.3f   (%llu)\n", k, names[k], 100.0 * (double)dsv[q].stamp[k] / tot, (double)dsv[q].stampLanes[k] / (64.0 * (double)dsv[q].stamp[k]), (unsigned long long)dsv[q].stamp[k]);
        }
    }
#endif
    if (dsv[0].rngOverflow || dsv[1].rngOverflow) {
#ifdef FRAY_QCHECK
        fprintf(stderr, "[qcheck] bounce kernel: %llu stale path entries, %llu other events; shadow kernel: %llu stale segments\n", (unsigned long long)(dsv[0].rngOverflow >> 32),
                (unsigned long long)(dsv[0].rngOverflow & 0xffffffffull), (unsigned long long)dsv[1].rngOverflow);
#endif
        set_error("frayhip_render: a camera sample left the supported envelope (Whitted: shade() nesting deeper than 40, or a camera sample whose pixel jitter stream passed 227 words)");
        return FRAYHIP_E_UNSUPPORTED;
    }
    if (st) {
        auto model = [](const DStats& d) {
            return 88.0 * (double)d.closest + 73.0 * (double)d.shadow + 168.0 * (double)d.node + 16.0 * (double)d.kdInner + 4.0 * (double)d.leafRefs +
                   120.0 * (double)d.tri + 32.0 * (double)d.prim + 144.0 * (double)d.smooth + 12.0 * (double)d.tex;
        };
        frayhip_stats o = finish_stats(sc, dsv, 2, nTraceEvents, nShadowEvents, t0);
        const DStats &a = dsv[0], &b = dsv[1];
        o.alg_bytes_trace = model(a);
        o.alg_bytes_shadow = model(b);
        auto flops = [](const DStats& d) {
            return 90.0 * (double)d.node + 45.0 * (double)d.tri + 30.0 * (double)d.prim + 30.0 * ((double)d.node + 2.0 * (double)d.kdInner);
        };
        o.alg_flops_trace = flops(a);
        o.alg_flops_shadow = flops(b);
        *st = o;
    }
    if (prog) {
        const bool rgbOut = f->mode == FRAYHIP_MODE_RENDER && d_rgb;
        if (rgbOut && prog->h_rgb) HIP_TRY(hipMemcpy(prog->h_rgb, d_rgb, B.frameBytes, hipMemcpyDeviceToHost));
        (void)B.call(rgbOut, true, rgbOut ? (prog->h_rgb ? prog->h_rgb : d_rgb) : nullptr);
        if (B.cut_short()) { set_error(std::string(who) + ": cancelled by the progress callback"); return FRAYHIP_E_CANCELLED; }
    }
    return FRAYHIP_OK;
}

}
```

### fray_amd/csrc/render_state.hpp

```cpp
#pragma once
#include <hip/hip_runtime.h>

#include <cstddef>
#include <string>
#include <vector>

#include "capi_common.h"
#include "dev_scene.hpp"
#include "dev_queues.hpp"

namespace frayhip_detail {
inline int hip_error_code(hipError_t e)
{
    switch (e) {
        case hipErrorOutOfMemory: return FRAYHIP_E_NOMEM;
        case hipErrorNoDevice: case hipErrorInvalidDevice: case hipErrorInsufficientDriver: case hipErrorNotInitialized: return FRAYHIP_E_NODEVICE;
        default: return FRAYHIP_E_HIP;
    }
}
}
#define HIP_TRY(expr)                                                                             \
    do {                                                                                          \
        hipError_t e_ = (expr);                                                                   \
        if (e_ != hipSuccess) {                                                                   \
            frayhip_detail::set_error(std::string(#expr) + ": " + hipGetErrorString(e_));         \
            return frayhip_detail::hip_error_code(e_);                                            \
        }                                                                                         \
    } while (0)

#ifndef FRAY_PT_BUDGET_MIB
#define FRAY_PT_BUDGET_MIB 24576
#endif
#ifndef FRAY_SEED_TABLE_MIB
#define FRAY_SEED_TABLE_MIB 4096
#endif
#ifndef FRAY_PT_LANES
#define FRAY_PT_LANES 4
#endif

struct SeedTable {
    uint32_t* d = nullptr;
    size_t bytes = 0;
    bool keyed = false;
    int32_t key[7] = {};
    uint32_t seed = 0;
    int nItems = 0;
    std::vector<unsigned char> valid;
    bool noGrow = false;
    bool serving = false;
};

struct SceneEdit;

struct frayhip_scene {
    void* d_arena = nullptr;
    size_t arena_bytes = 0;
    SceneEdit* edit = nullptr;
    long long sceneUpdates = 0, sceneUpdateBytes = 0;
    DScene S{};
    frayhip_camera camera{};
    frayhip_settings settings{};
    bool whittedNeedsRecursion = false;
    int specFanMax = 0;
    bool speculateFans = true;
    bool lightDraws = false;
    int lastWhittedPath = 0;
    int fusedWhittedMax = 4;
    int csgLanes = 1;
    unsigned warmMask = 0;
    bool fpContract = false;
    long long lastContracted = 0;
    bool skipNullSegments = true;
    bool segmentPlanes = true;
    bool certifiedSegments = true;
    long long lastShadowCertified = 0;
    long long lastShadowNodesSkipped = 0;
    long long lastShadowSegments = 0;
    long long lastFans[4] = {0, 0, 0, 0};
    int lightSampleCount = 0;
    bool extGeometry = false;
    bool textured = false;
    bool kdMeshes = false;
    void* d_work = nullptr;
    size_t work_bytes = 0;
    DStats* d_stats = nullptr;
    void* d_motionTab = nullptr;
    size_t motionTabBytes = 0;
    std::vector<unsigned char> motionTabHost;
    QMeta* d_qmeta = nullptr;
    hipEvent_t evA = nullptr, evB = nullptr;
    std::vector<hipEvent_t> evPool, evPoolShadow;
    hipStream_t laneStream[FRAY_PT_LANES] = {};
    hipEvent_t evLaneStart = nullptr, evResolved[FRAY_PT_LANES] = {};
    int ptLanes = FRAY_PT_LANES;
    size_t ptBudgetBytes = (size_t)FRAY_PT_BUDGET_MIB << 20;
    size_t ptBudgetEff = 0;
    size_t seedTableCapBytes = (size_t)FRAY_SEED_TABLE_MIB << 20;
    SeedTable seedTab;
    int lastBatchLanes = 0;
    long long lastSeedLaunches = 0, lastSeedReused = 0;
    bool rendering = false;
};

namespace frayhip_detail {

constexpr size_t kSegTotalsOffset = 2 * sizeof(DStats);
constexpr size_t kSegSkippedOffset = kSegTotalsOffset + FRAY_PT_LANES * sizeof(unsigned long long);
constexpr size_t kSegCertifiedOffset = kSegSkippedOffset + FRAY_PT_LANES * sizeof(unsigned long long);
constexpr size_t kCursorOffset = (kSegCertifiedOffset + FRAY_PT_LANES * sizeof(unsigned long long) + 255) / 256 * 256;
constexpr size_t kStatsBytes = kCursorOffset + 3 * sizeof(DCursors);

DCamera camera_begin_frame(const frayhip_camera& c, int W, int H);
int persistent_grid(size_t n, int wavesPerSimd);
size_t work_budget(frayhip_scene* sc);
enum { FRAYHIP_RETRY_SMALLER = 1 };
int ensure_work_or_shrink(frayhip_scene* sc, size_t bytes, bool canRetry);
int bounce_grid(size_t n, bool alone);
int grid_for(size_t n);
int seed_grid(size_t n);
int ensure_work(frayhip_scene* sc, size_t bytes);
void seed_table_begin(frayhip_scene* sc, const DFrame& F, int nItems, int spp);
void seed_table_invalidate(frayhip_scene* sc);
void seed_table_free(frayhip_scene* sc);

struct Progress {
    const frayhip_progressive* req;
    float* h_rgb;
};
hipEvent_t pool_event(std::vector<hipEvent_t>& pool, size_t i);

}
```

### fray_amd/csrc/scene_arena.hpp

```cpp
#pragma once
#include <algorithm>
#include <cmath>
#include <cstddef>
#include <cstdint>
#include <cstring>
#include <functional>
#include <vector>

#include "dev_scene.hpp"

namespace frayhip_arena {

struct ArenaTable { uint64_t off, bytes; };

struct ArenaMeshTables { int32_t tris, attrs, kd, kdBox, refs, ltris, ltris32; };

struct ArenaFacts {
    int32_t extGeometry, kdMeshes, textured, whittedNeedsRecursion, lightDraws, lightSampleCount, specFanMax;
    int32_t nGates, gatesExact, nSegPlanes, nSegNodes, segCertAll;
    int32_t nNodes, nLights, nMeshes, nTextures;
    int32_t envPresent, envLoaded, envWidth[6], envHeight[6];
    int64_t envTexelOffset[6];
    int32_t tNodes, tNodesX, tGates, tSegPlanes, tSegMasks, tPlanes, tSpheres, tCubes, tCsgs, tTexels, tShaders, tLayers, tLights, tMeshes, tTex;
};

struct ArenaBuilt {
    std::vector<unsigned char> host;
    std::vector<ArenaTable> tables;
    std::vector<ArenaMeshTables> meshTables;
    std::vector<int64_t> texelOffset;
    ArenaFacts F;
};

namespace detail {

struct Arena {
    std::vector<unsigned char>& host;
    std::vector<ArenaTable>& tables;
    size_t add(const void* p, size_t bytes, size_t align = 256)
    {
        size_t off = (host.size() + align - 1) / align * align;
        host.resize(off + bytes);
        if (bytes) memcpy(host.data() + off, p, bytes);
        tables.push_back(ArenaTable{(uint64_t)off, (uint64_t)bytes});
        return off;
    }
    size_t reserve(size_t bytes)
    {
        size_t off = add(nullptr, 0);
        host.resize(off + bytes);
        tables.back().bytes = bytes;
        return off;
    }
    int32_t last() const { return (int32_t)tables.size() - 1; }
};

inline void put3(double* o, const double* p) { o[0] = p[0]; o[1] = p[1]; o[2] = p[2]; }
inline void putX(DXform& X, const frayhip_transform& T)
{
    put3(X.off, T.offset);
    memcpy(X.m, T.m, sizeof X.m);
    memcpy(X.inv, T.invM, sizeof X.inv);
}

inline bool shader_uses_uv(const frayhip_scene_desc& d, int s, int depth = 0)
{
    if (s < 0 || s >= d.n_shaders || depth > 40) return false;
    const frayhip_shader& sh = d.shaders[s];
    auto texUV = [&](int t) { return t >= 0 && t < d.n_textures && d.textures[t].kind != FRAYHIP_TEX_FRESNEL; };
    if (texUV(sh.texture)) return true;
    if (sh.kind == FRAYHIP_SHADER_LAYERED)
        for (int i = 0; i < sh.layer_count; i++) {
            const frayhip_layer& L = d.layers[sh.layer_begin + i];
            if (texUV(L.texture) || shader_uses_uv(d, L.shader, depth + 1)) return true;
        }
    return false;
}

inline bool arena_keeps_tris(const DMesh& M) { return !M.hasKd && M.nTris > 0 && M.nTris < FRAY_GATE_MIN_TRIS; }
inline void fill_editable(const frayhip_scene_desc& d, const ArenaMeshTables* meshTables, ArenaFacts& F, unsigned char* const* tab)
{
    const DMesh* const meshes = (const DMesh*)tab[F.tMeshes];
    F.extGeometry = F.whittedNeedsRecursion = F.lightDraws = F.lightSampleCount = F.specFanMax = 0;
    for (int i = 0; i < d.n_nodes; i++) {
        int k = d.geoms[d.nodes[i].geom].kind;
        if (k == FRAYHIP_GEOM_CUBE || k == FRAYHIP_GEOM_CSG) F.extGeometry = 1;
    }
    std::vector<DNode> nodes(d.n_nodes);
    for (int i = 0; i < d.n_nodes; i++) {
        const frayhip_node& n = d.nodes[i];
        putX(nodes[i].T, n.T);
        nodes[i].geomKind = d.geoms[n.geom].kind;
        nodes[i].geomIndex = d.geoms[n.geom].index;
        nodes[i].shader = n.shader;
        nodes[i].bumpTex = n.bump_tex;
        nodes[i].xfClass = i;
        {
            static const double I9[9] = {1, 0, 0, 0, 1, 0, 0, 0, 1}, Z3[3] = {0, 0, 0};
            nodes[i].xfIdentity = (!memcmp(n.T.offset, Z3, sizeof Z3) && !memcmp(n.T.m, I9, sizeof I9) && !memcmp(n.T.invM, I9, sizeof I9)) ? 1 : 0;
        }
        for (int j = 0; j < i; j++)
            if (!memcmp(d.nodes[j].T.offset, n.T.offset, sizeof n.T.offset) && !memcmp(d.nodes[j].T.invM, n.T.invM, sizeof n.T.invM) &&
                !memcmp(d.nodes[j].T.m, n.T.m, sizeof n.T.m)) {
                nodes[i].xfClass = nodes[j].xfClass;
                break;
            }
        int sk = d.shaders[n.shader].kind;
        if (sk == FRAYHIP_SHADER_REFL || sk == FRAYHIP_SHADER_REFR || sk == FRAYHIP_SHADER_LAYERED) F.whittedNeedsRecursion = 1;
    }
    DPlane* const planes = (DPlane*)tab[F.tPlanes];
    for (int i = 0; i < d.n_planes; i++) { planes[i].limit = d.planes[i].limit; planes[i].height = d.planes[i].height; }
    DSphere* const spheres = (DSphere*)tab[F.tSpheres];
    for (int i = 0; i < d.n_spheres; i++) { put3(spheres[i].O, d.spheres[i].O); spheres[i].R = d.spheres[i].R; }
    DCube* const cubes = (DCube*)tab[F.tCubes];
    for (int i = 0; i < d.n_cubes; i++) { put3(cubes[i].O, d.cubes[i].O); cubes[i].halfSide = d.cubes[i].halfSide; }
    std::vector<DTexture> tex(d.n_textures);
    for (int i = 0; i < d.n_textures; i++) {
        const frayhip_texture& t = d.textures[i];
        DTexture& o = tex[i];
        o.kind = t.kind; o.width = t.width; o.height = t.height; o.pad = 0;
        memcpy(o.color1, t.color1, sizeof o.color1);
        memcpy(o.color2, t.color2, sizeof o.color2);
        o.scaling = t.scaling; o.bumpIntensity = t.bumpIntensity; o.ior = t.ior;
        o.texels = nullptr;
    }
    std::vector<DShader> shaders(d.n_shaders);
    for (int i = 0; i < d.n_shaders; i++) {
        const frayhip_shader& s = d.shaders[i];
        DShader& o = shaders[i];
        o.kind = s.kind; o.texture = s.texture;
        memcpy(o.color, s.color, sizeof o.color);
        memcpy(o.specularColor, s.specularColor, sizeof o.specularColor);
        memcpy(o.mult, s.mult, sizeof o.mult);
        o.numSamples = s.numSamples;
        o.exponent = s.exponent; o.specularMultiplier = s.specularMultiplier; o.glossiness = s.glossiness;
        o.deflectionScaling = s.deflectionScaling; o.ior = s.ior;
        o.layerBegin = s.layer_begin; o.layerCount = s.layer_count;
        o.usesUV = shader_uses_uv(d, i);
        o.pad = 0;
    }
    if (!shaders.empty()) memcpy(tab[F.tShaders], shaders.data(), shaders.size() * sizeof(DShader));
    std::vector<DLayer> layers(d.n_layers);
    for (int i = 0; i < d.n_layers; i++) {
        layers[i].shader = d.layers[i].shader; layers[i].texture = d.layers[i].texture;
        memcpy(layers[i].opacity, d.layers[i].opacity, sizeof layers[i].opacity);
        layers[i].pad = 0;
    }
    if (!layers.empty()) memcpy(tab[F.tLayers], layers.data(), layers.size() * sizeof(DLayer));
    std::vector<DLight> lights(d.n_lights);
    bool anyLightDraws = false;
    for (int i = 0; i < d.n_lights; i++) {
        const frayhip_light& l = d.lights[i];
        DLight& o = lights[i];
        o.kind = l.kind; o.xSubd = l.xSubd; o.ySubd = l.ySubd; o.pad = 0;
        memcpy(o.color, l.color, sizeof o.color);
        o.power = l.power;
        put3(o.pos, l.pos);
        putX(o.T, l.T);
        put3(o.center, l.center);
        o.area = l.area;
        F.lightSampleCount += l.kind == FRAYHIP_LIGHT_RECT ? l.xSubd * l.ySubd : 1;
        if (l.kind == FRAYHIP_LIGHT_RECT) F.lightDraws = 1;
// ... 25 lines not shown
    std::function<GB(int, int)> bounds = [&](int g, int depth) -> GB {
        GB b{true, {0, 0, 0}, {0, 0, 0}};
        if (g < 0 || g >= d.n_geoms || depth > FRAY_CSG_DEPTH + 1) { b.ok = false; return b; }
        const int kind = d.geoms[g].kind, idx = d.geoms[g].index;
        if (kind == FRAYHIP_GEOM_PLANE) {
            b.ok = false; return b;
        } else if (kind == FRAYHIP_GEOM_SPHERE) {
            for (int k = 0; k < 3; k++) { b.lo[k] = d.spheres[idx].O[k] - std::fabs(d.spheres[idx].R); b.hi[k] = d.spheres[idx].O[k] + std::fabs(d.spheres[idx].R); }
        } else if (kind == FRAYHIP_GEOM_CUBE) {
            for (int k = 0; k < 3; k++) { b.lo[k] = d.cubes[idx].O[k] - std::fabs(d.cubes[idx].halfSide); b.hi[k] = d.cubes[idx].O[k] + std::fabs(d.cubes[idx].halfSide); }
        } else if (kind == FRAYHIP_GEOM_MESH) {
            for (int k = 0; k < 3; k++) { b.lo[k] = meshes[idx].bmin[k]; b.hi[k] = meshes[idx].bmax[k]; }
        } else if (kind == FRAYHIP_GEOM_CSG) {
            const frayhip_csg& C = d.csgs[idx];
            const GB L = bounds(C.left, depth + 1), R = bounds(C.right, depth + 1);
            auto vol = [](const GB& q) { return (q.hi[0] - q.lo[0]) * (q.hi[1] - q.lo[1]) * (q.hi[2] - q.lo[2]); };
            if (C.op == FRAYHIP_CSG_MINUS) return L;
            if (C.op == FRAYHIP_CSG_AND) { if (L.ok && R.ok) return vol(L) <= vol(R) ? L : R; return L.ok ? L : R; }
            if (!L.ok || !R.ok) { b.ok = false; return b; }
            for (int k = 0; k < 3; k++) { b.lo[k] = std::min(L.lo[k], R.lo[k]); b.hi[k] = std::max(L.hi[k], R.hi[k]); }
        } else b.ok = false;
        for (int k = 0; k < 3; k++) if (!(std::isfinite(b.lo[k]) && std::isfinite(b.hi[k]) && b.lo[k] <= b.hi[k])) b.ok = false;
        return b;
    };
    std::vector<GB> csgLocal(d.n_nodes, GB{false, {0, 0, 0}, {0, 0, 0}});
    for (int i = 0; i < d.n_nodes; i++) {
        DNodeX& X = nodesX[i];
        for (int k = 0; k < 3; k++) X.cc[k] = X.ch[k] = 0;
        X.cM = 0; X.csgBox = 0; X.padX = 0;
        if (nodes[i].geomKind != FRAYHIP_GEOM_CSG) continue;
        const GB b = bounds(d.nodes[i].geom, 0);
        if (!b.ok) continue;
        csgLocal[i] = b;
        for (int k = 0; k < 3; k++) {
            X.cc[k] = 0.5 * (b.lo[k] + b.hi[k]);
            X.ch[k] = std::max(b.hi[k] - X.cc[k], X.cc[k] - b.lo[k]) * (1.0 + 1e-12) + 1e-5;
            X.cM = std::max(X.cM, std::fabs(X.cc[k]) + X.ch[k]);
        }
        X.csgBox = X.cM < 1e9 ? 1 : 0;
    }
    int nSegPlanes = 0, nSegNodes = 0;
    {
        DSegPlane planes[FRAY_SEG_MAX_PLANES];
        double planeAmax[FRAY_SEG_MAX_PLANES];
        uint32_t masks[FRAY_SEG_MAX_NODES];
        int segNodeOf[FRAY_SEG_MAX_NODES];
        bool fits = true;
        for (int i = 0; i < d.n_nodes && fits; i++) {
            const DNode& N = nodes[i];
            if (!(N.tlTris > 0 && N.tlTris < FRAY_GATE_MIN_TRIS && N.xfIdentity)) continue;
            const DTri* const tris = (const DTri*)tab[meshTables[N.geomIndex].tris];
            bool ok = true;
            for (int t = 0; t < N.tlTris && ok; t++) ok = segcert_triangle_ok(tris[t].N, tris[t].A);
            if (!ok) continue;
            if (nSegNodes == FRAY_SEG_MAX_NODES) { fits = false; break; }
            uint32_t mask = 0;
            for (int t = 0; t < N.tlTris; t++) {
                const double* TN = tris[t].N;
                const double* TA = tris[t].A;
                const double k = segcert_offset(TN, TA), am = std::max(std::fabs(TA[0]), std::max(std::fabs(TA[1]), std::fabs(TA[2])));
                int p = 0;
                while (p < nSegPlanes && (memcmp(planes[p].N, TN, 3 * sizeof(double)) != 0 || memcmp(&planes[p].k, &k, sizeof k) != 0)) p++;
                if (p == nSegPlanes) {
                    if (nSegPlanes == FRAY_SEG_MAX_PLANES) { fits = false; break; }
                    memcpy(planes[p].N, TN, 3 * sizeof(double)); planes[p].k = k; planeAmax[p] = 0;
                    nSegPlanes++;
                }
                planeAmax[p] = std::max(planeAmax[p], am);
                mask |= 1u << p;
            }
            if (!fits) break;
            segNodeOf[nSegNodes] = i;
            masks[nSegNodes++] = mask;
        }
        if (!fits) nSegPlanes = nSegNodes = 0;
        for (int p = 0; p < nSegPlanes; p++) { const DSegPlane q = planes[p]; segcert_make(planes[p], q.N, q.k, planeAmax[p]); }
        for (int j = 0; j < nSegNodes; j++) nodes[segNodeOf[j]].segNode = j + 1;
        memset(tab[F.tSegPlanes], 0, FRAY_SEG_MAX_PLANES * sizeof(DSegPlane));
        memset(tab[F.tSegMasks], 0, FRAY_SEG_MAX_NODES * sizeof(uint32_t));
        if (nSegPlanes) memcpy(tab[F.tSegPlanes], planes, (size_t)nSegPlanes * sizeof(DSegPlane));
        if (nSegNodes) memcpy(tab[F.tSegMasks], masks, (size_t)nSegNodes * sizeof(uint32_t));
    }
    if (!nodesX.empty()) memcpy(tab[F.tNodesX], nodesX.data(), nodesX.size() * sizeof(DNodeX));
    int nGates = 0;
    bool gatesExact = false;
    {
        DGate gates[FRAY_MAX_GATES];
        int gateNode[FRAY_MAX_GATES];
        double smallest = 1e300;
        for (int i = 0; i < d.n_nodes; i++)
            if (csgLocal[i].ok) for (int k = 0; k < 3; k++) smallest = std::min(smallest, std::max(csgLocal[i].hi[k] - csgLocal[i].lo[k], 1e-9));
        for (int i = 0; i < d.n_nodes && nGates < FRAY_MAX_GATES; i++) {
            const DNode& N = nodes[i];
            double bmin[3], bmax[3];
            if (N.tlTris >= FRAY_GATE_MIN_TRIS) { put3(bmin, N.bmin); put3(bmax, N.bmax); }
            else if (csgLocal[i].ok) {
                bool huge = false;
                for (int k = 0; k < 3; k++) { bmin[k] = csgLocal[i].lo[k]; bmax[k] = csgLocal[i].hi[k]; huge = huge || bmax[k] - bmin[k] > 30.0 * smallest; }
                if (huge) continue;
            } else continue;
            DGate g;
            for (int k = 0; k < 3; k++) { g.lo[k] = 1e300; g.hi[k] = -1e300; }
            for (int c = 0; c < 8; c++) {
                const double p[3] = {c & 1 ? bmax[0] : bmin[0], c & 2 ? bmax[1] : bmin[1], c & 4 ? bmax[2] : bmin[2]};
                for (int k = 0; k < 3; k++) {
                    const double w = p[0] * N.T.m[k] + p[1] * N.T.m[3 + k] + p[2] * N.T.m[6 + k] + N.T.off[k];
                    g.lo[k] = std::min(g.lo[k], w); g.hi[k] = std::max(g.hi[k], w);
                }
            }
            g.exact = N.xfIdentity ? 1 : 0;
            g.Mf = 0;
            for (int k = 0; k < 3; k++) {
                const double c = 0.5 * (bmin[k] + bmax[k]), half = std::max(bmax[k] - c, c - bmin[k]);
                g.cf[k] = (float)c;
                g.hf[k] = std::nextafterf((float)(half * (1.0 + 1e-12) + 1e-5 + std::fabs(c - (double)g.cf[k])), INFINITY);
                g.Mf = std::max(g.Mf, std::nextafterf(std::fabs(g.cf[k]) + g.hf[k], INFINITY));
            }
            if (!(g.Mf < 1e9f)) g.exact = 0;
            for (int k = 0; k < 3; k++) { const double e = 1e-6 * (1.0 + std::fabs(g.lo[k]) + std::fabs(g.hi[k])); g.lo[k] -= e; g.hi[k] += e; }
            gateNode[nGates] = i;
            gates[nGates++] = g;
        }
        gatesExact = nGates > 0;
        for (int q = 0; q < nGates; q++) gatesExact = gatesExact && gates[q].exact;
        if (gatesExact)
            for (int q = 0; q < nGates; q++) nodes[gateNode[q]].gated = 1;
        memset(tab[F.tGates], 0, FRAY_MAX_GATES * sizeof(DGate));
        if (nGates) memcpy(tab[F.tGates], gates, (size_t)nGates * sizeof(DGate));
    }
    if (!nodes.empty()) memcpy(tab[F.tNodes], nodes.data(), nodes.size() * sizeof(DNode));
    if (!tex.empty()) memcpy(tab[F.tTex], tex.data(), tex.size() * sizeof(DTexture));

    F.nGates = nGates; F.gatesExact = gatesExact ? 1 : 0;
    F.nSegPlanes = nSegPlanes; F.nSegNodes = nSegNodes;
    bool segCertAll = true;
    for (int i = 0; i < d.n_nodes; i++) segCertAll = segCertAll && (nodes[i].segNode != 0 || nodes[i].gated != 0);
    segCertAll = segCertAll && d.n_lights > 0;
    const DSegPlane* const entries = (const DSegPlane*)tab[F.tSegPlanes];
    for (int p = 0; p < nSegPlanes && segCertAll; p++) {
        const DSegPlane& P = entries[p];
        bool off = false;
        for (int i = 0; i < d.n_lights && !off; i++) {
            const frayhip_light& l = d.lights[i];
            for (int c = 0; c < (l.kind == FRAYHIP_LIGHT_RECT ? 4 : 1) && !off; c++) {
                const double px = c & 1 ? 0.5 : -0.5, pz = c & 2 ? 0.5 : -0.5;
                double w[3];
                for (int k = 0; k < 3; k++) w[k] = l.kind == FRAYHIP_LIGHT_RECT ? px * l.T.m[k] + pz * l.T.m[6 + k] + l.T.offset[k] : l.pos[k];
                off = std::fabs(P.N[0] * w[0] + P.N[1] * w[1] + P.N[2] * w[2] - P.k) > P.t0;
            }
        }
        segCertAll = off;
    }
    const uint32_t* const nodeMasks = (const uint32_t*)tab[F.tSegMasks];
    bool starts = false;
    for (int j = 0; j < nSegNodes && !starts; j++) {
        bool clear = true;
        for (int p = 0; p < nSegPlanes; p++)
            if (nodeMasks[j] >> p & 1u) {
                const DSegPlane& P = entries[p];
                clear = clear && 1e-6 * std::sqrt(P.N[0] * P.N[0] + P.N[1] * P.N[1] + P.N[2] * P.N[2]) > P.t0;
            }
        starts = clear;
    }
    segCertAll = segCertAll && starts;
    F.segCertAll = segCertAll ? 1 : 0;
}

}

inline void arena_build(const frayhip_scene_desc& d, ArenaBuilt& B)
{
    using detail::put3;
    B.host.clear(); B.tables.clear(); B.meshTables.clear(); B.texelOffset.clear();
    ArenaFacts& F = B.F;
    memset(&F, 0, sizeof F);
    detail::Arena A{B.host, B.tables};
    A.reserve((size_t)d.n_nodes * sizeof(DNode));
    F.tNodes = A.last();
    A.reserve((size_t)d.n_nodes * sizeof(DNodeX));
    F.tNodesX = A.last();
    A.reserve(FRAY_MAX_GATES * sizeof(DGate));
    F.tGates = A.last();
    A.reserve(FRAY_SEG_MAX_PLANES * sizeof(DSegPlane));
    F.tSegPlanes = A.last();
    A.reserve(FRAY_SEG_MAX_NODES * sizeof(uint32_t));
    F.tSegMasks = A.last();
    A.reserve((size_t)d.n_planes * sizeof(DPlane));
    F.tPlanes = A.last();
    A.reserve((size_t)d.n_spheres * sizeof(DSphere));
    F.tSpheres = A.last();
    A.reserve((size_t)d.n_cubes * sizeof(DCube));
    F.tCubes = A.last();
    std::vector<DCsg> csgs(d.n_csgs);
    for (int i = 0; i < d.n_csgs; i++) {
        const frayhip_csg& g = d.csgs[i];
        csgs[i].op = g.op;
        csgs[i].leftKind = d.geoms[g.left].kind; csgs[i].leftIndex = d.geoms[g.left].index; csgs[i].leftGeom = g.left;
        csgs[i].rightKind = d.geoms[g.right].kind; csgs[i].rightIndex = d.geoms[g.right].index; csgs[i].rightGeom = g.right;
        csgs[i].flat = (csgs[i].leftKind <= FRAYHIP_GEOM_CUBE && csgs[i].rightKind <= FRAYHIP_GEOM_CUBE) ? 1 : 0;
    }
    A.add(csgs.data(), csgs.size() * sizeof(DCsg));
    F.tCsgs = A.last();
    std::vector<DMesh> meshes(d.n_meshes);
    B.meshTables.resize(d.n_meshes);
    for (int mi = 0; mi < d.n_meshes; mi++) {
        const frayhip_mesh& m = d.meshes[mi];
        DMesh& M = meshes[mi];
        put3(M.bmin, m.bbox_min);
        put3(M.bmax, m.bbox_max);
        M.boxMax = 0;
        for (int k = 0; k < 3; k++) M.boxMax = std::max(M.boxMax, std::max(std::fabs(m.bbox_min[k]), std::fabs(m.bbox_max[k])));
        M.nTris = m.n_triangles;
        M.hasKd = m.has_kd;
        if (m.has_kd) F.kdMeshes = 1;
        M.smooth = !(m.faceted || m.n_normals == 0);
        M.culling = m.backfaceCulling;
        M.hasUV = m.n_uvs != 0;
        std::vector<DTri> tris(m.n_triangles);
        std::vector<DTriAttr> attrs(m.n_triangles);
        for (int t = 0; t < m.n_triangles; t++) {
            const frayhip_triangle& T = m.triangles[t];
            DTri& o = tris[t];
            put3(o.g, T.gnormal);
            put3(o.A, m.vertices + 3 * (size_t)T.v[0]);
            put3(o.N, T.ABcrossAC);
            put3(o.AC, T.AC);
            put3(o.AB, T.AB);
            o.index = t; o.pad = 0;
            DTriAttr& a = attrs[t];
            memset(&a, 0, sizeof a);
            if (M.smooth) {
                put3(a.nA, m.normals + 3 * (size_t)T.n[0]);
                put3(a.nB, m.normals + 3 * (size_t)T.n[1]);
                put3(a.nC, m.normals + 3 * (size_t)T.n[2]);
            }
            if (M.hasUV) {
                const double* tA = m.uvs + 3 * (size_t)T.t[0]; const double* tB = m.uvs + 3 * (size_t)T.t[1]; const double* tC = m.uvs + 3 * (size_t)T.t[2];
                a.tA[0] = tA[0]; a.tA[1] = tA[1]; a.tB[0] = tB[0]; a.tB[1] = tB[1]; a.tC[0] = tC[0]; a.tC[1] = tC[1];
            }
            put3(a.dNdx, T.dNdx);
            put3(a.dNdy, T.dNdy);
        }
        std::vector<DKd> kd(m.n_kdnodes);
        std::vector<DKdBox> kdBox(m.n_kdnodes);
        if (m.n_kdnodes > 0) {
            for (int k = 0; k < 3; k++) { kdBox[0].lo[k] = m.bbox_min[k]; kdBox[0].hi[k] = m.bbox_max[k]; }
            for (int n = 0; n < m.n_kdnodes; n++) {
                const frayhip_kdnode& K = m.kdnodes[n];
                DKd& o = kd[n];
                o.child0 = K.child0; o.meta = K.axis;
                if (K.axis != 3) {
                    o.split = K.split;
                    o.meta |= (m.kdnodes[K.child0].axis == 3 ? 4 : 0) | (m.kdnodes[K.child0 + 1].axis == 3 ? 8 : 0);
                    kdBox[K.child0] = kdBox[n];
                    kdBox[K.child0 + 1] = kdBox[n];
                    kdBox[K.child0].hi[K.axis] = K.split;
                    kdBox[K.child0 + 1].lo[K.axis] = K.split;
                } else {
                    o.triBegin = K.tri_begin; o.triCount = K.tri_count;
                }
            }
        }
        ArenaMeshTables& MT = B.meshTables[mi];
        A.add(tris.data(), tris.size() * sizeof(DTri)); MT.tris = A.last();
        A.add(attrs.data(), attrs.size() * sizeof(DTriAttr)); MT.attrs = A.last();
        A.add(kd.data(), kd.size() * sizeof(DKd)); MT.kd = A.last();
        A.add(kdBox.data(), kdBox.size() * sizeof(DKdBox)); MT.kdBox = A.last();
        A.add(m.trirefs, (size_t)m.n_trirefs * sizeof(int32_t)); MT.refs = A.last();
        std::vector<DTri> ltris((size_t)m.n_trirefs);
        for (int r = 0; r < m.n_trirefs; r++) ltris[r] = tris[m.trirefs[r]];
        A.add(ltris.data(), ltris.size() * sizeof(DTri)); MT.ltris = A.last();
        for (int k = 0; k < 3; k++) M.ref[k] = (m.bbox_min[k] + m.bbox_max[k]) * 0.5;
        std::vector<DTri32> l32(ltris.size());
        for (size_t r = 0; r < ltris.size(); r++) tricert_make(l32[r], ltris[r].A, ltris[r].AB, ltris[r].AC, ltris[r].N, M.ref);
        A.add(l32.data(), l32.size() * sizeof(DTri32)); MT.ltris32 = A.last();
    }
    A.add(d.texels, (size_t)d.n_texels * sizeof(float));
    F.tTexels = A.last();
    B.texelOffset.resize(d.n_textures);
    for (int i = 0; i < d.n_textures; i++) B.texelOffset[i] = d.textures[i].texel_offset;
    A.reserve((size_t)d.n_shaders * sizeof(DShader));
    F.tShaders = A.last();
    A.reserve((size_t)d.n_layers * sizeof(DLayer));
    F.tLayers = A.last();
    A.reserve((size_t)d.n_lights * sizeof(DLight));
    F.tLights = A.last();
    size_t oMeshes = A.reserve(meshes.size() * sizeof(DMesh));
    F.tMeshes = A.last();
    A.reserve((size_t)d.n_textures * sizeof(DTexture));
    F.tTex = A.last();
    if (!meshes.empty()) memcpy(A.host.data() + oMeshes, meshes.data(), meshes.size() * sizeof(DMesh));

    F.nNodes = d.n_nodes; F.nLights = d.n_lights; F.nMeshes = d.n_meshes; F.nTextures = d.n_textures;
    F.envPresent = d.environment.present;
    F.envLoaded = d.environment.loaded;
    if (d.n_textures > 0 || (d.environment.present && d.environment.loaded)) F.textured = 1;
    for (int f = 0; f < 6; f++) {
        F.envWidth[f] = d.environment.width[f];
        F.envHeight[f] = d.environment.height[f];
        F.envTexelOffset[f] = d.environment.texel_offset[f];
    }
    std::vector<unsigned char*> tab(B.tables.size());
    for (size_t t = 0; t < B.tables.size(); t++) tab[t] = B.host.data() + B.tables[t].off;
    detail::fill_editable(d, B.meshTables.data(), F, tab.data());
}

inline void arena_update(const frayhip_scene_desc& d, const ArenaMeshTables* meshTables, ArenaFacts& F, unsigned char* const* tab)
{
    detail::fill_editable(d, meshTables, F, tab);
}
inline void arena_update(const frayhip_scene_desc& d, ArenaBuilt& B)
{
    std::vector<unsigned char*> tab(B.tables.size());
    for (size_t t = 0; t < B.tables.size(); t++) tab[t] = B.host.data() + B.tables[t].off;
    arena_update(d, B.meshTables.data(), B.F, tab.data());
}
inline std::vector<int32_t> arena_editable_tables(const ArenaFacts& F)
{
    return {F.tNodes, F.tNodesX, F.tGates, F.tSegPlanes, F.tSegMasks, F.tPlanes, F.tSpheres, F.tCubes, F.tShaders, F.tLayers, F.tLights, F.tTex};
}

inline void arena_place(const ArenaFacts& F, const ArenaMeshTables* meshTables, const int64_t* texelOffset, unsigned char* const* write,
                        const unsigned char* const* addr, DScene& S)
{
    DMesh* const meshes = (DMesh*)write[F.tMeshes];
    for (int mi = 0; mi < F.nMeshes; mi++) {
        const ArenaMeshTables& MT = meshTables[mi];
        meshes[mi].tris = (const FRAY_RO DTri*)addr[MT.tris];
        meshes[mi].attrs = (const FRAY_RO DTriAttr*)addr[MT.attrs];
        meshes[mi].kd = (const FRAY_RO DKd*)addr[MT.kd];
        meshes[mi].kdBox = (const FRAY_RO DKdBox*)addr[MT.kdBox];
        meshes[mi].refs = (const FRAY_RO int32_t*)addr[MT.refs];
        meshes[mi].ltris = (const FRAY_RO DTri*)addr[MT.ltris];
        meshes[mi].ltris32 = (const FRAY_RO DTri32*)addr[MT.ltris32];
    }
    DNode* const nodes = (DNode*)write[F.tNodes];
    for (int i = 0; i < F.nNodes; i++)
        if (nodes[i].geomKind == FRAYHIP_GEOM_MESH && !meshes[nodes[i].geomIndex].hasKd) nodes[i].tlPtr = meshes[nodes[i].geomIndex].tris;
    DTexture* const tex = (DTexture*)write[F.tTex];
    for (int i = 0; i < F.nTextures; i++) tex[i].texels = (const FRAY_RO float*)addr[F.tTexels] + texelOffset[i];

    S.nodes = (const FRAY_RO DNode*)addr[F.tNodes];
    S.nodesX = (const FRAY_RO DNodeX*)addr[F.tNodesX];
    S.gates = (const FRAY_RO DGate*)addr[F.tGates];
    S.nGates = F.nGates; S.gatesExact = F.gatesExact;
    S.segPlanes = (const FRAY_RO DSegPlane*)addr[F.tSegPlanes];
    S.segNodeMasks = (const FRAY_RO uint32_t*)addr[F.tSegMasks];
    S.nSegPlanes = F.nSegPlanes; S.nSegNodes = F.nSegNodes; S.segCertAll = F.segCertAll;
    S.planes = (const FRAY_RO DPlane*)addr[F.tPlanes];
    S.spheres = (const FRAY_RO DSphere*)addr[F.tSpheres];
    S.cubes = (const FRAY_RO DCube*)addr[F.tCubes];
    S.csgs = (const FRAY_RO DCsg*)addr[F.tCsgs];
    S.meshes = (const FRAY_RO DMesh*)addr[F.tMeshes];
    S.shaders = (const FRAY_RO DShader*)addr[F.tShaders];
    S.layers = (const FRAY_RO DLayer*)addr[F.tLayers];
    S.textures = (const FRAY_RO DTexture*)addr[F.tTex];
    S.lights = (const FRAY_RO DLight*)addr[F.tLights];
    S.env.present = F.envPresent;
    S.env.loaded = F.envLoaded;
    for (int f = 0; f < 6; f++) {
        S.env.width[f] = F.envWidth[f];
        S.env.height[f] = F.envHeight[f];
        S.env.face[f] = (const FRAY_RO float*)addr[F.tTexels] + F.envTexelOffset[f];
    }
    S.nNodes = F.nNodes;
    S.nLights = F.nLights;
    S.probPickLight = F.nLights > 0 ? 1.0f / (float)F.nLights : 0.0f;
}

}
```

### fray_amd/scene.py

```python
import ctypes as C
import math
import os
import sys

import numpy as np

from . import abi

P = C.POINTER

_HERE = os.path.dirname(os.path.abspath(__file__))
_LIB_PATH = os.environ.get("FRAYHIP_LIB") or os.path.join(_HERE, "libfrayhip.so")


class FrayError(RuntimeError):
    def __init__(self, code, msg):
        super().__init__("frayhip error %d: %s" % (code, msg))
        self.code = code


def _load():
    if "torch" not in sys.modules and not os.environ.get("FRAYHIP_NO_TORCH"):
        try:
            import torch
# ... 477 lines not shown
            state = np.ascontiguousarray(z["state"], dtype=np.float32)
            return cls(state, int(z["samples_done"]), int(z["seed"]), tuple(int(v) for v in z["size"]), int(z["share"][0]), int(z["share"][1]))


class Scene:

    def __init__(self):
        self._hs = C.c_void_p()
        self._dev = C.c_void_p()
        self.desc = None

    @classmethod
    def parseScene(cls, path):
        s = cls()
        _check(lib.frayhip_scene_parse(os.fspath(path).encode(), C.byref(s._hs)))
        s.desc = lib.frayhip_host_scene_desc(s._hs).contents
        return s

    @property
    def settings(self):
        return self.desc.settings

    @property
    def camera(self):
        return self.desc.camera

    def _table(self, name, rec):
        n = getattr(self.desc, "n_" + name)
        return C.cast(getattr(self.desc, name), P(rec * n)).contents if n else (rec * 0)()

    nodes = property(lambda self: self._table("nodes", abi.Node), doc="desc.nodes[] as a mutable array of abi.Node")
    lights = property(lambda self: self._table("lights", abi.Light), doc="desc.lights[] (abi.Light)")
    shaders = property(lambda self: self._table("shaders", abi.Shader), doc="desc.shaders[] (abi.Shader)")
    layers = property(lambda self: self._table("layers", abi.Layer), doc="desc.layers[] (abi.Layer)")
    textures = property(lambda self: self._table("textures", abi.Texture), doc="desc.textures[] (abi.Texture): color1, color2, scaling, bumpIntensity and ior are editable")
    spheres = property(lambda self: self._table("spheres", abi.Sphere), doc="desc.spheres[] (abi.Sphere)")
    planes = property(lambda self: self._table("planes", abi.Plane), doc="desc.planes[] (abi.Plane)")
    cubes = property(lambda self: self._table("cubes", abi.Cube), doc="desc.cubes[] (abi.Cube)")

    @property
    def frame_size(self):
        return self.desc.settings.frameWidth, self.desc.settings.frameHeight

    def samples_per_pixel(self):
        spp = 5 if self.settings.wantAA else 1
        if self.camera.dof:
            spp = max(spp, self.camera.numDOFSamples)
        if self.settings.gi:
            spp = max(spp, self.settings.numPaths)
        return spp

    def beginRender(self, device=None):
        if device is not None:
            _check(lib.frayhip_init(int(device)))
        self.endRender()
        _check(lib.frayhip_scene_create(C.byref(self.desc), C.byref(self._dev)))
        return self

    def beginFrame(self):
        self._need_dev()
        _check(lib.frayhip_scene_set_view(self._dev, C.byref(self.desc.camera), C.byref(self.desc.settings)))
        return self

    def update(self):
        self._need_dev()
        _check(lib.frayhip_scene_update(self._dev, C.byref(self.desc)))
        return self

    def endRender(self):
        if self._dev:
            lib.frayhip_scene_destroy(self._dev)
            self._dev = C.c_void_p()

    def set_option(self, name, value):
        self._need_dev()
        _check(lib.frayhip_scene_set_option(self._dev, name.encode(), int(value)))
        return self

    def get_option(self, name):
        self._need_dev()
        v = C.c_int64(0)
        _check(lib.frayhip_scene_get_option(self._dev, name.encode(), C.byref(v)))
        return int(v.value)

    def _frame(self, mode, seed, bucket_first, bucket_stride, spp_chunk, stats):
        return abi.Frame(mode=mode, seed=seed, bucket_first=bucket_first, bucket_stride=bucket_stride,
                         spp_chunk=spp_chunk, flags=abi.FRAME_STATS if stats else 0)

    def _need_dev(self):
        if not self._dev:
            raise FrayError(abi.E_ARG, "Scene.beginRender() has not been called")

    def render(self, seed=42, bucket_first=0, bucket_stride=1, spp_chunk=0, stats=False, out=None, progress=None, preview_ms=-1):
        self._need_dev()
        W, H = self.frame_size
        rgb = out if out is not None else np.zeros((H, W, 3), np.float32)
        st = abi.Stats()
        fr = self._frame(abi.MODE_RENDER, seed, bucket_first, bucket_stride, spp_chunk, stats)
        if progress is None:
            _check(lib.frayhip_render(self._dev, C.byref(fr), rgb.ctypes.data, None, None, C.byref(st)))
            return rgb, st.as_dict()
        req, run = _progress_request(progress, preview_ms, lambda p: {"image": np.ctypeslib.as_array(p.rgb, shape=(H, W, 3))})
        rc = lib.frayhip_render_progressive(self._dev, C.byref(fr), C.byref(req), rgb.ctypes.data, None, None, C.byref(st))
        return rgb, run.finish(rc, st)

    def primary_hits(self, bucket_first=0, bucket_stride=1, stats=False):
        self._need_dev()
        W, H = self.frame_size
        ids = np.full((H, W), -9, np.int32)
        dist = np.zeros((H, W), np.float64)
        st = abi.Stats()
        fr = self._frame(abi.MODE_PRIMARY_ID, 0, bucket_first, bucket_stride, 0, stats)
        _check(lib.frayhip_render(self._dev, C.byref(fr), None, ids.ctypes.data, dist.ctypes.data, C.byref(st)))
        return ids, dist, st.as_dict()

    def render_device(self, d_rgb_ptr, seed=42, bucket_first=0, bucket_stride=1, spp_chunk=0, stats=False,
                      stream=None, mode=abi.MODE_RENDER, d_id_ptr=None, d_dist_ptr=None, progress=None, preview_ms=-1):
        self._need_dev()
        st = abi.Stats()
        fr = self._frame(mode, seed, bucket_first, bucket_stride, spp_chunk, stats)
        if progress is None:
            _check(lib.frayhip_render_device(self._dev, C.byref(fr), d_rgb_ptr, d_id_ptr, d_dist_ptr, stream, C.byref(st)))
            return st.as_dict()
        req, run = _progress_request(progress, preview_ms, lambda p: {"d_rgb": C.cast(p.rgb, C.c_void_p).value})
        rc = lib.frayhip_render_device_progressive(self._dev, C.byref(fr), C.byref(req), d_rgb_ptr, d_id_ptr, d_dist_ptr, stream, C.byref(st))
        return run.finish(rc, st)

    def camera_rays(self, xy=None, eye=0, stream=None):
        self._need_dev()
        if xy is None:
            W, H = self.frame_size
            org, dirs = np.empty((H, W, 3)), np.empty((H, W, 3))
            _check(lib.frayhip_camera_rays(self._dev, W * H, None, int(eye), org.ctypes.data, dirs.ctypes.data))
            return org, dirs
        (xy,), shape, device = _query_inputs([("xy", xy)], 2)
        n = int(np.prod(shape, dtype=np.int64))
        if device is None:
            xy = np.ascontiguousarray(xy)
            org, dirs = np.empty(shape + (3,)), np.empty(shape + (3,))
            _check(lib.frayhip_camera_rays(self._dev, n, xy.ctypes.data, int(eye), org.ctypes.data, dirs.ctypes.data))
            return org, dirs
        with _DeviceCall(device, stream) as call:
            torch = call.torch
            xy = xy.contiguous()
            org = torch.empty(shape + (3,), dtype=torch.float64, device=device)
            dirs = torch.empty(shape + (3,), dtype=torch.float64, device=device)
            if n:
                _check(lib.frayhip_camera_rays_device(self._dev, n, xy.data_ptr(), int(eye), org.data_ptr(), dirs.data_ptr(), call.handle))
        return org, dirs

    def trace_rays(self, origin, dir, record=False, stats=False, stream=None):
        self._need_dev()
        (o, d), shape, device = _query_inputs([("origin", origin), ("dir", dir)])
        n = int(np.prod(shape, dtype=np.int64))
        st = abi.Stats()
        flags = abi.FRAME_STATS if stats else 0
        if device is None:
            o, d = np.ascontiguousarray(o), np.ascontiguousarray(d)
            ids, dist = np.empty(shape, np.int32), np.empty(shape, np.float64)
            rec = np.empty(shape + (9,), np.float64) if record else None
            _check(lib.frayhip_trace_rays(self._dev, n, o.ctypes.data, d.ctypes.data, flags, ids.ctypes.data, dist.ctypes.data,
                                          rec.ctypes.data if record else None, C.byref(st)))
        else:
            with _DeviceCall(device, stream) as call:
                torch = call.torch
                o, d = o.contiguous(), d.contiguous()
# ... 446 lines not shown
```

### include/frayhip.h

```cpp
#ifndef FRAYHIP_H
#define FRAYHIP_H

#include <stdint.h>

#ifdef __cplusplus
extern "C" {
#endif

#define FRAYHIP_ABI_VERSION 3

enum {
    FRAYHIP_OK            = 0,
    FRAYHIP_E_ARG         = -1,
    FRAYHIP_E_PARSE       = -2,
    FRAYHIP_E_NODEVICE    = -3,
    FRAYHIP_E_UNSUPPORTED = -4,
    FRAYHIP_E_NOMEM       = -5,
    FRAYHIP_E_HIP         = -6,
    FRAYHIP_E_CANCELLED   = -7,
};


typedef struct frayhip_transform {
    double offset[3];
// ... 113 lines not shown
    int64_t n_texels;
    const frayhip_node*     nodes;
    const frayhip_geom_ref* geoms;
    const frayhip_plane*    planes;
    const frayhip_sphere*   spheres;
    const frayhip_cube*     cubes;
    const frayhip_csg*      csgs;
    const frayhip_mesh*     meshes;
    const frayhip_shader*   shaders;
    const frayhip_layer*    layers;
    const frayhip_texture*  textures;
    const frayhip_light*    lights;
    const float*            texels;
    frayhip_environment environment;
    frayhip_camera      camera;
    frayhip_settings    settings;
} frayhip_scene_desc;

enum {
    FRAYHIP_MODE_PRIMARY_ID = 0,
    FRAYHIP_MODE_RENDER     = 1,
};

#define FRAYHIP_BUCKET_SKEW 3
typedef struct frayhip_frame {
    int32_t  mode;
    uint32_t seed;
    int32_t  bucket_first, bucket_stride;
    int32_t  spp_chunk;
    int32_t  flags;
} frayhip_frame;

enum {
    FRAYHIP_FRAME_STATS = 1,
};

typedef struct frayhip_stats {
    uint64_t closest_rays;
    uint64_t shadow_rays;
    uint64_t node_tests;
    uint64_t kd_inner_visits;
    uint64_t leaf_refs;
    uint64_t tri_tests;
    uint64_t prim_tests;
    uint64_t smooth_hits;
    uint64_t samples;
    uint64_t texture_fetches;
    double   ms_total;
    double   ms_kernels;
    double   ms_trace;
    uint64_t trace_launches;
    double   alg_bytes_trace;
    double   ms_shadow;
    uint64_t shadow_launches;
    double   alg_bytes_shadow;
    double   alg_flops_trace;
    double   alg_flops_shadow;
} frayhip_stats;

typedef struct frayhip_host_scene frayhip_host_scene;

int  frayhip_scene_parse(const char* fray_path, frayhip_host_scene** out);
frayhip_scene_desc* frayhip_host_scene_desc(frayhip_host_scene* hs);
void frayhip_host_scene_free(frayhip_host_scene* hs);

typedef struct frayhip_scene frayhip_scene;

int  frayhip_init(int device_id);
int  frayhip_scene_create(const frayhip_scene_desc* desc, frayhip_scene** out);
void frayhip_scene_destroy(frayhip_scene* s);
int  frayhip_scene_set_view(frayhip_scene* s, const frayhip_camera* camera, const frayhip_settings* settings);

int  frayhip_scene_update(frayhip_scene* s, const frayhip_scene_desc* desc);

int  frayhip_transform_identity(frayhip_transform* T);
int  frayhip_transform_scale(frayhip_transform* T, double x, double y, double z);
int  frayhip_transform_rotate(frayhip_transform* T, double yaw, double pitch, double roll);
int  frayhip_transform_translate(frayhip_transform* T, double x, double y, double z);
int  frayhip_light_begin_frame(frayhip_light* light);
int  frayhip_shader_begin_frame(frayhip_shader* shader);

int  frayhip_scene_set_option(frayhip_scene* s, const char* name, int64_t value);
int  frayhip_scene_get_option(frayhip_scene* s, const char* name, int64_t* value);

int  frayhip_render(frayhip_scene* s, const frayhip_frame* f,
                    float* rgb, int32_t* hit_id, double* hit_dist, frayhip_stats* st);
int  frayhip_render_device(frayhip_scene* s, const frayhip_frame* f,
                           float* d_rgb, int32_t* d_hit_id, double* d_hit_dist,
                           void* hip_stream, frayhip_stats* st);

typedef struct frayhip_progress {
    int32_t samples_done;
    int32_t samples_total;
    int32_t batches_done, batches_total;
    double  ms_elapsed;
    int32_t preview;
    int32_t final;
    const float* rgb;
} frayhip_progress;

typedef struct frayhip_progressive {
    int  (*fn)(void* user, const frayhip_progress* p);
    void*  user;
    double preview_ms;
} frayhip_progressive;

int  frayhip_render_progressive(frayhip_scene* s, const frayhip_frame* f, const frayhip_progressive* p,
                                float* rgb, int32_t* hit_id, double* hit_dist, frayhip_stats* st);
int  frayhip_render_device_progressive(frayhip_scene* s, const frayhip_frame* f, const frayhip_progressive* p,
                                       float* d_rgb, int32_t* d_hit_id, double* d_hit_dist, void* hip_stream, frayhip_stats* st);

int  frayhip_camera_rays(frayhip_scene* s, int64_t n, const double* xy, int eye, double* origin, double* dir);
int  frayhip_camera_rays_device(frayhip_scene* s, int64_t n, const double* d_xy, int eye,
                                double* d_origin, double* d_dir, void* hip_stream);
int  frayhip_trace_rays(frayhip_scene* s, int64_t n, const double* origin, const double* dir, int flags,
                        int32_t* hit_id, double* hit_dist, double* hit_rec, frayhip_stats* st);
int  frayhip_trace_rays_device(frayhip_scene* s, int64_t n, const double* d_origin, const double* d_dir, int flags,
                               int32_t* d_hit_id, double* d_hit_dist, double* d_hit_rec, void* hip_stream, frayhip_stats* st);
int  frayhip_visible(frayhip_scene* s, int64_t n, const double* a, const double* b, int flags, uint8_t* vis, frayhip_stats* st);
int  frayhip_visible_device(frayhip_scene* s, int64_t n, const double* d_a, const double* d_b, int flags,
                            uint8_t* d_vis, void* hip_stream, frayhip_stats* st);

typedef struct frayhip_shade_request {
    uint32_t seed;
    int32_t  spp;
    int32_t  sample_first;
    int32_t  rng_skip;
    int32_t  flags;
    int32_t  _pad;
    const uint32_t* keys;
} frayhip_shade_request;

int  frayhip_shade_rays(frayhip_scene* s, int64_t n, const double* origin, const double* dir,
                        const frayhip_shade_request* r, float* rgb, frayhip_stats* st);
int  frayhip_shade_rays_device(frayhip_scene* s, int64_t n, const double* d_origin, const double* d_dir,
                               const frayhip_shade_request* r, float* d_rgb, void* hip_stream, frayhip_stats* st);

typedef struct frayhip_adaptive {
    int32_t  min_spp;
    int32_t  _pad;
    double   threshold;
    double   err_floor;
    int32_t  rungs;
    int32_t  _pad2;
    uint64_t samples;
} frayhip_adaptive;

int  frayhip_render_adaptive(frayhip_scene* s, const frayhip_frame* f, frayhip_adaptive* a,
                             float* rgb, int32_t* spp_out, float* err_out, frayhip_stats* st);
int  frayhip_render_device_adaptive(frayhip_scene* s, const frayhip_frame* f, frayhip_adaptive* a,
                                    float* d_rgb, int32_t* d_spp, float* d_err, void* hip_stream, frayhip_stats* st);

#define FRAYHIP_ACCUM_CHANNELS 4
typedef struct frayhip_samples {
    int32_t sample_first;
    int32_t sample_count;
    int32_t samples_done;
    int32_t _pad;
} frayhip_samples;

int  frayhip_render_samples(frayhip_scene* s, const frayhip_frame* f, frayhip_samples* r, const frayhip_progressive* p,
                            float* accum, float* rgb, float* noise, frayhip_stats* st);
int  frayhip_render_samples_device(frayhip_scene* s, const frayhip_frame* f, frayhip_samples* r, const frayhip_progressive* p,
                                   float* d_accum, float* d_rgb, float* d_noise, void* hip_stream, frayhip_stats* st);

int  frayhip_render_components(frayhip_scene* s, const frayhip_frame* f, frayhip_samples* r, const frayhip_progressive* p,
// ... 144 lines not shown
```

Baseline: 13310.

## Use tight triangle-bound gates with plane-normal guards for ray gate classification

For small identity-transformed meshes, builds a tighter gate box around the actual triangle vertices and records up to eight distinct face normals as guard planes. At classification time, rays nearly parallel to any guard plane fall back to the conservative gate, and all other rays are tested against the tight box. The aim is to classify more rays as gate-free so they go to the cheaper front queue instead of the full back-traversal path. In exchange it adds per-ray guard-plane tests, larger arena tables and a mesh-size threshold raised from 6 to 64 triangles for keeping triangles, plus filed-ray counters in the scan kernel.

```diff
diff --git a/fray_amd/abi.py b/fray_amd/abi.py
--- a/fray_amd/abi.py
+++ b/fray_amd/abi.py
@@ -232,6 +232,7 @@
     "frayhip_shader_begin_frame": (C.c_int, [P(Shader)]),
     "frayhip_scene_set_option": (C.c_int, [VP, C.c_char_p, i64]),
     "frayhip_scene_get_option": (C.c_int, [VP, C.c_char_p, P(i64)]),
+    "frayhip_scene_gate_figures": (C.c_int, [VP, P(i64)]),
     "frayhip_render": (C.c_int, [VP, P(Frame), VP, VP, VP, P(Stats)]),
     "frayhip_render_device": (C.c_int, [VP, P(Frame), VP, VP, VP, VP, P(Stats)]),
     "frayhip_render_progressive": (C.c_int, [VP, P(Frame), P(Progressive), VP, VP, VP, P(Stats)]),
diff --git a/fray_amd/csrc/capi.hip b/fray_amd/csrc/capi.hip
--- a/fray_amd/csrc/capi.hip
+++ b/fray_amd/csrc/capi.hip
@@ -253,6 +253,7 @@
     S.skipNullSegments = s->skipNullSegments ? 1 : 0;
     S.segmentPlanes = s->segmentPlanes ? 1 : 0;
     S.certifiedSegments = (s->certifiedSegments && s->segmentPlanes && S.segCertAll) ? 1 : 0;
+    if (s->tightGates && S.nTightGates > 0) S.gates = S.gatesTight; else S.nGuardChunks = 0;
     return S;
 }
 
@@ -585,6 +586,7 @@
     if (const char* e = getenv("FRAYHIP_SKIP_NULL_SEGMENTS")) sc->skipNullSegments = atol(e) != 0;
     if (const char* e = getenv("FRAYHIP_SEGMENT_PLANES")) sc->segmentPlanes = atol(e) != 0;
     if (const char* e = getenv("FRAYHIP_CERTIFIED_SEGMENTS")) sc->certifiedSegments = atol(e) != 0;
+    if (const char* e = getenv("FRAYHIP_TIGHT_GATES")) sc->tightGates = atol(e) != 0;
     if (const char* e = getenv("FRAYHIP_FUSED_WHITTED_MAX")) { long v = atol(e); if (v >= 0 && v <= 1024) sc->fusedWhittedMax = (int)v; }
     if (const char* e = getenv("FRAYHIP_CSG_LANES")) { long v = atol(e); if (v >= 1 && v <= FRAY_PT_LANES) sc->csgLanes = (int)v; }
     if (const char* e = getenv("FRAYHIP_SEED_TABLE_MIB")) { long v = atol(e); if (v >= 0 && v <= (1 << 20)) sc->seedTableCapBytes = (size_t)v << 20; }
@@ -626,6 +628,16 @@
     else if (n == "fan_children_looked_up") *value = s->lastFans[2];
     else if (n == "fans_given_up") *value = s->lastFans[3];
     else { set_error("frayhip_scene_get_option: unknown option " + n); return FRAYHIP_E_ARG; }
+    return FRAYHIP_OK;
+}
+
+int frayhip_scene_gate_figures(frayhip_scene* s, int64_t out[4])
+{
+    if (!s || !out) { set_error("frayhip_scene_gate_figures: null argument"); return FRAYHIP_E_ARG; }
+    out[0] = s->tightGates ? 1 : 0;
+    out[1] = s->S.nTightGates;
+    out[2] = s->lastRaysFiled;
+    out[3] = s->lastRaysFiledFront;
     return FRAYHIP_OK;
 }
 
diff --git a/fray_amd/csrc/dev_misscert.hpp b/fray_amd/csrc/dev_misscert.hpp
--- a/fray_amd/csrc/dev_misscert.hpp
+++ b/fray_amd/csrc/dev_misscert.hpp
@@ -39,3 +39,61 @@
     miss = miss || __builtin_fabsf(dx * py - dy * px) > (ay * Hx + ax * Hy) * g + sl;
     return miss;
 }
+
+#ifndef FRAY_GATEGUARD_SCALE
+#define FRAY_GATEGUARD_SCALE 1.0
+#endif
+#define FRAY_GATE_KAPPA_MAX 64.0
+#define FRAY_GATE_NORMALS_MAX 8
+
+template <class NP>
+FRAY_CERT_FN bool ray_crosses_planes(NP n, int count, double dx, double dy, double dz, double dsum)
+{
+    bool ok = true;
+    for (int j = 0; j < count; j++) ok = ok & (__builtin_fabs(n[3 * j] * dx + n[3 * j + 1] * dy + n[3 * j + 2] * dz) >= FRAY_GATEGUARD_SCALE * 0x1p-16 * dsum);
+    return ok;
+}
+FRAY_CERT_FN bool ray_crosses_plane_f32(float nx, float ny, float nz, float dx, float dy, float dz, float dsum)
+{
+    return __builtin_fabsf(nx * dx + ny * dy + nz * dz) >= (float)FRAY_GATEGUARD_SCALE * 0x1p-16f * dsum;
+}
+
+template <class TRI>
+inline bool gate_tight_build(const TRI* tris, int n, double lo[3], double hi[3], double* normals, int& nNormals)
+{
+    nNormals = 0;
+    if (n <= 0) return false;
+    for (int k = 0; k < 3; k++) { lo[k] = 1e300; hi[k] = -1e300; }
+    for (int t = 0; t < n; t++)
+        for (int k = 0; k < 3; k++) {
+            const double v[3] = {tris[t].A[k], tris[t].A[k] + tris[t].AB[k], tris[t].A[k] + tris[t].AC[k]};
+            for (int q = 0; q < 3; q++) {
+                if (!(__builtin_fabs(v[q]) < 1e9) || !(__builtin_fabs(tris[t].AB[k]) < 1e9) || !(__builtin_fabs(tris[t].AC[k]) < 1e9)) return false;
+                const double r = 0x1p-52 * __builtin_fabs(v[q]);
+                lo[k] = __builtin_fmin(lo[k], v[q] - r); hi[k] = __builtin_fmax(hi[k], v[q] + r);
+            }
+        }
+    const double ext = __builtin_fmax(__builtin_fmax(hi[0] - lo[0], hi[1] - lo[1]), hi[2] - lo[2]);
+    for (int t = 0; t < n; t++) {
+        const double *AB = tris[t].AB, *AC = tris[t].AC, *N = tris[t].N;
+        const double X[3] = {AB[1] * AC[2] - AB[2] * AC[1], AB[2] * AC[0] - AB[0] * AC[2], AB[0] * AC[1] - AB[1] * AC[0]};
+        const double lab = __builtin_sqrt(AB[0] * AB[0] + AB[1] * AB[1] + AB[2] * AB[2]), lac = __builtin_sqrt(AC[0] * AC[0] + AC[1] * AC[1] + AC[2] * AC[2]);
+        const double ln = __builtin_sqrt(N[0] * N[0] + N[1] * N[1] + N[2] * N[2]);
+        for (int k = 0; k < 3; k++) if (!(__builtin_fabs(N[k] - X[k]) <= 0x1p-51 * lab * lac)) return false;
+        if (!(ln > 0) || !(ext * __builtin_fmax(lab, lac) <= FRAY_GATE_KAPPA_MAX * ln)) return false;
+        const double u[3] = {N[0] / ln, N[1] / ln, N[2] / ln};
+        int j = 0;
+        for (; j < nNormals; j++) {
+            const double* q = normals + 3 * j;
+            const double same = __builtin_fmax(__builtin_fmax(__builtin_fabs(u[0] - q[0]), __builtin_fabs(u[1] - q[1])), __builtin_fabs(u[2] - q[2]));
+            const double opp = __builtin_fmax(__builtin_fmax(__builtin_fabs(u[0] + q[0]), __builtin_fabs(u[1] + q[1])), __builtin_fabs(u[2] + q[2]));
+            if (same <= 0x1p-30 || opp <= 0x1p-30) break;
+        }
+        if (j == nNormals) {
+            if (nNormals == FRAY_GATE_NORMALS_MAX) return false;
+            normals[3 * j] = u[0]; normals[3 * j + 1] = u[1]; normals[3 * j + 2] = u[2];
+            nNormals++;
+        }
+    }
+    return true;
+}
diff --git a/fray_amd/csrc/dev_scene.hpp b/fray_amd/csrc/dev_scene.hpp
--- a/fray_amd/csrc/dev_scene.hpp
+++ b/fray_amd/csrc/dev_scene.hpp
@@ -130,6 +130,9 @@
 #define FRAY_MAX_GATES 8
 #define FRAY_GATE_MIN_TRIS 6
 struct DGate { double lo[3], hi[3]; float cf[3], hf[3]; float Mf; int32_t exact; };
+#define FRAY_GATE_MAX_NORMALS 8
+#define FRAY_GATE_TIGHT_MAX_TRIS 64
+struct DGuard { float n[3]; uint32_t mask; };
 
 struct DScene {
     const FRAY_RO DNode* nodes;
@@ -158,6 +161,10 @@
     int32_t skipNullSegments;
     int32_t segCertAll;
     int32_t certifiedSegments;
+    const FRAY_RO DGate* gatesTight;
+    const FRAY_RO DGuard* guards;
+    int32_t nTightGates;
+    int32_t nGuardChunks;
 };
 
 struct DFrame {
diff --git a/fray_amd/csrc/dev_trace.hpp b/fray_amd/csrc/dev_trace.hpp
--- a/fray_amd/csrc/dev_trace.hpp
+++ b/fray_amd/csrc/dev_trace.hpp
@@ -938,12 +938,34 @@
 #else
 #define FRAY_RCPF(x) (1.0f / (x))
 #endif
+template <bool GUARD = true>
 FD uint32_t ray_gate_class(const DScene& S, V3 o, V3 d)
 {
     const int ng = S.nGates;
     if (ng == 0) return 0u;
+    if constexpr (GUARD) {
+        if (S.gatesExact) {
+            const float dx = (float)d.x, dy = (float)d.y, dz = (float)d.z;
+            const float dsum = fabsf(dx) + fabsf(dy) + fabsf(dz);
+            uint32_t guardFails = 0;
+            for (int c = 0, nc = S.nGuardChunks; c < nc; c++) {
+                const FRAY_RO DGuard* Q = S.guards + 4 * c;
+#pragma unroll
+                for (int j = 0; j < 4; j++) guardFails |= ray_crosses_plane_f32(Q[j].n[0], Q[j].n[1], Q[j].n[2], dx, dy, dz, dsum) ? 0u : Q[j].mask;
+            }
+            const float ox = (float)o.x, oy = (float)o.y, oz = (float)o.z;
+            const float omax = fmaxf(fmaxf(fabsf(ox), fabsf(oy)), fabsf(oz));
+            uint32_t first = 0;
+            for (int g = ng - 1; g >= 0; g--) {
+                const FRAY_RO DGate& G = S.gates[g];
+                const bool miss = ray_surely_misses_box_f32(G.cf[0], G.cf[1], G.cf[2], G.hf[0], G.hf[1], G.hf[2], G.Mf, ox, oy, oz, dx, dy, dz, omax, dsum);
+                if (!miss || (guardFails >> g & 1u)) first = (uint32_t)g + 1u;
+            }
+            return !(omax < 1e9f) && !first ? 1u : first;
+        }
+    }
     const float ox = (float)o.x, oy = (float)o.y, oz = (float)o.z;
-    if (S.gatesExact) {
+    if (!GUARD && S.gatesExact) {
         const float dx = (float)d.x, dy = (float)d.y, dz = (float)d.z;
         const float omax = fmaxf(fmaxf(fabsf(ox), fabsf(oy)), fabsf(oz)), dsum = fabsf(dx) + fabsf(dy) + fabsf(dz);
         uint32_t first = 0;
diff --git a/fray_amd/csrc/kernels.hpp b/fray_amd/csrc/kernels.hpp
--- a/fray_amd/csrc/kernels.hpp
+++ b/fray_amd/csrc/kernels.hpp
@@ -724,16 +724,23 @@
     t.j = r->tab[0]; t.a = r->tab[1]; t.b = r->tab[2];
 }
 
-static __global__ __launch_bounds__(1024) void k_scan(QMeta* m0, QMeta* m1, unsigned long long* shadowTotal)
+static __global__ __launch_bounds__(1024) void k_scan(QMeta* m0, QMeta* m1, unsigned long long* shadowTotal, unsigned long long* filed)
 {
     QMeta* m = blockIdx.x == 0 ? m0 : m1;
     __shared__ uint32_t part[1024];
+    __shared__ uint32_t frontTotal;
+    if (threadIdx.x == 0) frontTotal = 0;
     const uint32_t nSeg = m->nSeg;
     const uint32_t per = (nSeg + 1023u) / 1024u;
     const uint32_t b = threadIdx.x * per;
-    uint32_t sum = 0;
-    for (uint32_t k = 0; k < per; k++) if (b + k < nSeg) sum += m->cnt[b + k];
+    uint32_t sum = 0, front = 0;
+    for (uint32_t k = 0; k < per; k++) if (b + k < nSeg) { sum += m->cnt[b + k]; front += m->nf[b + k]; }
     part[threadIdx.x] = sum;
+    __syncthreads();
+    if (filed) {
+        for (int o = 32; o > 0; o >>= 1) front += __shfl_down(front, o);
+        if ((threadIdx.x & 63) == 0 && front) atomicAdd(&frontTotal, front);
+    }
     __syncthreads();
     for (uint32_t d = 1; d < 1024; d <<= 1) {
         uint32_t v = threadIdx.x >= d ? part[threadIdx.x - d] : 0;
@@ -747,6 +754,7 @@
     if (threadIdx.x == 1023) {
         m->off[nSeg] = part[1023]; m->n = part[1023];
         if (blockIdx.x == 1 && shadowTotal) *shadowTotal += part[1023];
+        if (filed) { atomicAdd(filed + 2 * blockIdx.x, (unsigned long long)part[1023]); atomicAdd(filed + 2 * blockIdx.x + 1, (unsigned long long)frontTotal); }
     }
 }
 
@@ -960,7 +968,7 @@
             if (shadow) {
                 bool planesPass = false;
                 if constexpr (ST == 0 && FRAY_ARITH == 0) { if (S.certifiedSegments) planesPass = segment_certified(S, sa, sb); }
-                shadowBack = ray_gate_class(S, sa, sb - sa);
+                shadowBack = ray_gate_class<!(ST & 14)>(S, sa, sb - sa);
                 if constexpr (ST == 0) {
                     if (FRAY_ARITH == 0 ? planesPass && shadowBack == 0 : segment_surely_visible(S, sa, sb, shadowBack)) {
                         own = sc;
@@ -1108,7 +1116,7 @@
             path_shade<ST, false>(S, ps, h, TB, st, SB, cont, shadow, shadowBack, SQ, shadowEnds, c);
             STAMP(10);
         }
-        const uint32_t gate = cont ? ray_gate_class(S, ps.o, ps.d) : 0u;
+        const uint32_t gate = cont ? ray_gate_class<!(ST & 14)>(S, ps.o, ps.d) : 0u;
         const bool back = gate != 0;
         const uint32_t slotOut = seg_slot(outEnds, cont, back);
 #ifdef FRAY_SORT_BY_MATERIAL
diff --git a/fray_amd/csrc/render_impl.hpp b/fray_amd/csrc/render_impl.hpp
--- a/fray_amd/csrc/render_impl.hpp
+++ b/fray_amd/csrc/render_impl.hpp
@@ -47,7 +47,7 @@
         hipLaunchKernelGGL((k_pt_bounce<ST, false>), dim3(grid), dim3(256), 0, stream, BA);
         HIP_TRY(hipEventRecord(eb, stream));
         nTraceEvents += 2;
-        hipLaunchKernelGGL(k_scan, dim3(2), dim3(1024), 0, stream, meta + ((b + 1) & 1), meta + 2, (unsigned long long*)nullptr);
+        hipLaunchKernelGGL(k_scan, dim3(2), dim3(1024), 0, stream, meta + ((b + 1) & 1), meta + 2, (unsigned long long*)nullptr, (unsigned long long*)nullptr);
         HIP_TRY(hipEventRecord(ec, stream));
         hipLaunchKernelGGL(k_pt_shadow<ST>, dim3(grid), dim3(256), 0, stream, ShadowArgs{S, SQ, mSh, TB, sc->d_stats + 1, (unsigned long long*)((unsigned char*)sc->d_stats + kSegSkippedOffset)});
         HIP_TRY(hipEventRecord(ed, stream));
@@ -471,6 +471,7 @@
                 unsigned long long* segTotal;
                 unsigned long long* segSkipped;
                 unsigned long long* segCertified;
+                unsigned long long* segFiled;
             } lane[FRAY_PT_LANES];
             unsigned char* p = (unsigned char*)sc->d_work;
             float* sum = (float*)p; p += ((size_t)nItems * 12 + 255) / 256 * 256;
@@ -481,6 +482,7 @@
                 L.segTotal = (unsigned long long*)((unsigned char*)sc->d_stats + kSegTotalsOffset) + k;
                 L.segSkipped = (unsigned long long*)((unsigned char*)sc->d_stats + kSegSkippedOffset) + k;
                 L.segCertified = (unsigned long long*)((unsigned char*)sc->d_stats + kSegCertifiedOffset) + k;
+                L.segFiled = (unsigned long long*)((unsigned char*)sc->d_stats + kSegFiledOffset) + 4 * k;
                 p = carve_queue(p, nQueue, L.Q[0]);
                 p = carve_queue(p, nQueue, L.Q[1]);
                 p = carve_shadow(p, nQueue, L.SQ);
@@ -539,7 +541,7 @@
                         else hipLaunchKernelGGL((k_pt_bounce<ST, false>), dim3(grid), dim3(256), 0, ls, BA);
                         HIP_TRY(hipEventRecord(eb, ls));
                         nTraceEvents += 2;
-                        hipLaunchKernelGGL(k_scan, dim3(2), dim3(1024), 0, ls, L.meta + ((b + 1) & 1), L.meta + 2, L.segTotal);
+                        hipLaunchKernelGGL(k_scan, dim3(2), dim3(1024), 0, ls, L.meta + ((b + 1) & 1), L.meta + 2, L.segTotal, L.segFiled);
                         HIP_TRY(hipEventRecord(ec, ls));
                         bool contractedShadow = false;
                         if constexpr (!(ST & 2)) {
@@ -579,8 +581,8 @@
     HIP_TRY(hipEventRecord(sc->evB, stream));
     HIP_TRY(hipStreamSynchronize(stream));
     drain.armed = false;
-    struct Back { DStats ds[2]; unsigned long long segTotal[FRAY_PT_LANES], segSkipped[FRAY_PT_LANES], segCertified[FRAY_PT_LANES]; } back;
-    static_assert(offsetof(Back, segTotal) == kSegTotalsOffset && offsetof(Back, segSkipped) == kSegSkippedOffset && offsetof(Back, segCertified) == kSegCertifiedOffset,
+    struct Back { DStats ds[2]; unsigned long long segTotal[FRAY_PT_LANES], segSkipped[FRAY_PT_LANES], segCertified[FRAY_PT_LANES], segFiled[4 * FRAY_PT_LANES]; } back;
+    static_assert(offsetof(Back, segTotal) == kSegTotalsOffset && offsetof(Back, segSkipped) == kSegSkippedOffset && offsetof(Back, segCertified) == kSegCertifiedOffset && offsetof(Back, segFiled) == kSegFiledOffset,
                   "the shadow-queue totals, the skipped nodes and the certified segments follow the counter blocks");
     HIP_TRY(hipMemcpy(&back, sc->d_stats, sizeof back, hipMemcpyDeviceToHost));
     const DStats (&dsv)[2] = back.ds;
@@ -589,6 +591,11 @@
     sc->lastShadowCertified = 0;
     for (int k = 0; k < FRAY_PT_LANES; k++) sc->lastShadowCertified += (long long)back.segCertified[k];
     sc->lastShadowSegments += sc->lastShadowCertified;
+    sc->lastRaysFiled = sc->lastRaysFiledFront = 0;
+    for (int k = 0; k < FRAY_PT_LANES; k++) {
+        sc->lastRaysFiled += (long long)(back.segFiled[4 * k] + back.segFiled[4 * k + 2]);
+        sc->lastRaysFiledFront += (long long)(back.segFiled[4 * k + 1] + back.segFiled[4 * k + 3]);
+    }
     sc->lastShadowNodesSkipped = 0;
     for (int k = 0; k < FRAY_PT_LANES; k++) sc->lastShadowNodesSkipped += (long long)back.segSkipped[k];
     {
diff --git a/fray_amd/csrc/render_state.hpp b/fray_amd/csrc/render_state.hpp
--- a/fray_amd/csrc/render_state.hpp
+++ b/fray_amd/csrc/render_state.hpp
@@ -73,6 +73,8 @@
     bool skipNullSegments = true;
     bool segmentPlanes = true;
     bool certifiedSegments = true;
+    bool tightGates = true;
+    long long lastRaysFiled = 0, lastRaysFiledFront = 0;
     long long lastShadowCertified = 0;
     long long lastShadowNodesSkipped = 0;
     long long lastShadowSegments = 0;
@@ -107,7 +109,8 @@
 constexpr size_t kSegTotalsOffset = 2 * sizeof(DStats);
 constexpr size_t kSegSkippedOffset = kSegTotalsOffset + FRAY_PT_LANES * sizeof(unsigned long long);
 constexpr size_t kSegCertifiedOffset = kSegSkippedOffset + FRAY_PT_LANES * sizeof(unsigned long long);
-constexpr size_t kCursorOffset = (kSegCertifiedOffset + FRAY_PT_LANES * sizeof(unsigned long long) + 255) / 256 * 256;
+constexpr size_t kSegFiledOffset = kSegCertifiedOffset + FRAY_PT_LANES * sizeof(unsigned long long);
+constexpr size_t kCursorOffset = (kSegFiledOffset + 4 * FRAY_PT_LANES * sizeof(unsigned long long) + 255) / 256 * 256;
 constexpr size_t kStatsBytes = kCursorOffset + 3 * sizeof(DCursors);
 
 DCamera camera_begin_frame(const frayhip_camera& c, int W, int H);
diff --git a/fray_amd/csrc/scene_arena.hpp b/fray_amd/csrc/scene_arena.hpp
--- a/fray_amd/csrc/scene_arena.hpp
+++ b/fray_amd/csrc/scene_arena.hpp
@@ -8,6 +8,7 @@
 #include <vector>
 
 #include "dev_scene.hpp"
+#include "dev_misscert.hpp"
 
 namespace frayhip_arena {
 
@@ -17,11 +18,11 @@
 
 struct ArenaFacts {
     int32_t extGeometry, kdMeshes, textured, whittedNeedsRecursion, lightDraws, lightSampleCount, specFanMax;
-    int32_t nGates, gatesExact, nSegPlanes, nSegNodes, segCertAll;
+    int32_t nGates, gatesExact, nTightGates, nGuardChunks, nSegPlanes, nSegNodes, segCertAll;
     int32_t nNodes, nLights, nMeshes, nTextures;
     int32_t envPresent, envLoaded, envWidth[6], envHeight[6];
     int64_t envTexelOffset[6];
-    int32_t tNodes, tNodesX, tGates, tSegPlanes, tSegMasks, tPlanes, tSpheres, tCubes, tCsgs, tTexels, tShaders, tLayers, tLights, tMeshes, tTex;
+    int32_t tNodes, tNodesX, tGates, tGatesTight, tGuards, tSegPlanes, tSegMasks, tPlanes, tSpheres, tCubes, tCsgs, tTexels, tShaders, tLayers, tLights, tMeshes, tTex;
 };
 
 struct ArenaBuilt {
@@ -77,7 +78,7 @@
     return false;
 }
 
-inline bool arena_keeps_tris(const DMesh& M) { return !M.hasKd && M.nTris > 0 && M.nTris < FRAY_GATE_MIN_TRIS; }
+inline bool arena_keeps_tris(const DMesh& M) { return !M.hasKd && M.nTris > 0 && M.nTris <= FRAY_GATE_TIGHT_MAX_TRIS; }
 inline void fill_editable(const frayhip_scene_desc& d, const ArenaMeshTables* meshTables, ArenaFacts& F, unsigned char* const* tab)
 {
     const DMesh* const meshes = (const DMesh*)tab[F.tMeshes];
@@ -269,11 +270,14 @@
         if (nSegNodes) memcpy(tab[F.tSegMasks], masks, (size_t)nSegNodes * sizeof(uint32_t));
     }
     if (!nodesX.empty()) memcpy(tab[F.tNodesX], nodesX.data(), nodesX.size() * sizeof(DNodeX));
-    int nGates = 0;
+    int nGates = 0, nTightGates = 0, nGuards = 0;
     bool gatesExact = false;
     {
-        DGate gates[FRAY_MAX_GATES];
+        DGate gates[FRAY_MAX_GATES], tight[FRAY_MAX_GATES];
         int gateNode[FRAY_MAX_GATES];
+        DGuard guards[FRAY_MAX_GATES * FRAY_GATE_MAX_NORMALS];
+        memset(guards, 0, sizeof guards);
+        static_assert(FRAY_GATE_NORMALS_MAX == FRAY_GATE_MAX_NORMALS, "dev_misscert.hpp's table of normals is DGate's");
         double smallest = 1e300;
         for (int i = 0; i < d.n_nodes; i++)
             if (csgLocal[i].ok) for (int k = 0; k < 3; k++) smallest = std::min(smallest, std::max(csgLocal[i].hi[k] - csgLocal[i].lo[k], 1e-9));
@@ -287,6 +291,7 @@
                 if (huge) continue;
             } else continue;
             DGate g;
+            memset(&g, 0, sizeof g);
             for (int k = 0; k < 3; k++) { g.lo[k] = 1e300; g.hi[k] = -1e300; }
             for (int c = 0; c < 8; c++) {
                 const double p[3] = {c & 1 ? bmax[0] : bmin[0], c & 2 ? bmax[1] : bmin[1], c & 4 ? bmax[2] : bmin[2]};
@@ -296,16 +301,38 @@
                 }
             }
             g.exact = N.xfIdentity ? 1 : 0;
-            g.Mf = 0;
-            for (int k = 0; k < 3; k++) {
-                const double c = 0.5 * (bmin[k] + bmax[k]), half = std::max(bmax[k] - c, c - bmin[k]);
-                g.cf[k] = (float)c;
-                g.hf[k] = std::nextafterf((float)(half * (1.0 + 1e-12) + 1e-5 + std::fabs(c - (double)g.cf[k])), INFINITY);
-                g.Mf = std::max(g.Mf, std::nextafterf(std::fabs(g.cf[k]) + g.hf[k], INFINITY));
-            }
+            auto certBox = [](DGate& q, const double* lo, const double* hi) {
+                q.Mf = 0;
+                for (int k = 0; k < 3; k++) {
+                    const double c = 0.5 * (lo[k] + hi[k]), half = std::max(hi[k] - c, c - lo[k]);
+                    q.cf[k] = (float)c;
+                    q.hf[k] = std::nextafterf((float)(half * (1.0 + 1e-12) + 1e-5 + std::fabs(c - (double)q.cf[k])), INFINITY);
+                    q.Mf = std::max(q.Mf, std::nextafterf(std::fabs(q.cf[k]) + q.hf[k], INFINITY));
+                }
+            };
+            certBox(g, bmin, bmax);
             if (!(g.Mf < 1e9f)) g.exact = 0;
             for (int k = 0; k < 3; k++) { const double e = 1e-6 * (1.0 + std::fabs(g.lo[k]) + std::fabs(g.hi[k])); g.lo[k] -= e; g.hi[k] += e; }
+            DGate t = g;
+            if (g.exact && N.tlTris >= FRAY_GATE_MIN_TRIS && arena_keeps_tris(meshes[N.geomIndex]) && !F.extGeometry && !F.kdMeshes && !F.textured) {
+                double tlo[3], thi[3], normals[3 * FRAY_GATE_MAX_NORMALS];
+                int nn = 0;
+                if (gate_tight_build((const DTri*)tab[meshTables[N.geomIndex].tris], N.tlTris, tlo, thi, normals, nn)) {
+                    DGate q = g;
+                    certBox(q, tlo, thi);
+                    if (q.Mf < 1e9f) {
+                        for (int j = 0; j < nn; j++) {
+                            DGuard& U = guards[nGuards++];
+                            for (int k = 0; k < 3; k++) U.n[k] = (float)normals[3 * j + k];
+                            U.mask = 1u << nGates;
+                        }
+                        t = q;
+                        nTightGates++;
+                    }
+                }
+            }
             gateNode[nGates] = i;
+            tight[nGates] = t;
             gates[nGates++] = g;
         }
         gatesExact = nGates > 0;
@@ -314,11 +341,16 @@
             for (int q = 0; q < nGates; q++) nodes[gateNode[q]].gated = 1;
         memset(tab[F.tGates], 0, FRAY_MAX_GATES * sizeof(DGate));
         if (nGates) memcpy(tab[F.tGates], gates, (size_t)nGates * sizeof(DGate));
+        if (!gatesExact) nTightGates = 0;
+        memset(tab[F.tGatesTight], 0, FRAY_MAX_GATES * sizeof(DGate));
+        if (nGates) memcpy(tab[F.tGatesTight], gatesExact ? tight : gates, (size_t)nGates * sizeof(DGate));
+        if (!gatesExact) { nGuards = 0; memset(guards, 0, sizeof guards); }
+        memcpy(tab[F.tGuards], guards, sizeof guards);
     }
     if (!nodes.empty()) memcpy(tab[F.tNodes], nodes.data(), nodes.size() * sizeof(DNode));
     if (!tex.empty()) memcpy(tab[F.tTex], tex.data(), tex.size() * sizeof(DTexture));
 
-    F.nGates = nGates; F.gatesExact = gatesExact ? 1 : 0;
+    F.nGates = nGates; F.gatesExact = gatesExact ? 1 : 0; F.nTightGates = nTightGates; F.nGuardChunks = (nGuards + 3) / 4;
     F.nSegPlanes = nSegPlanes; F.nSegNodes = nSegNodes;
     bool segCertAll = true;
     for (int i = 0; i < d.n_nodes; i++) segCertAll = segCertAll && (nodes[i].segNode != 0 || nodes[i].gated != 0);
@@ -368,6 +400,10 @@
     F.tNodesX = A.last();
     A.reserve(FRAY_MAX_GATES * sizeof(DGate));
     F.tGates = A.last();
+    A.reserve(FRAY_MAX_GATES * sizeof(DGate));
+    F.tGatesTight = A.last();
+    A.reserve(FRAY_MAX_GATES * FRAY_GATE_MAX_NORMALS * sizeof(DGuard));
+    F.tGuards = A.last();
     A.reserve(FRAY_SEG_MAX_PLANES * sizeof(DSegPlane));
     F.tSegPlanes = A.last();
     A.reserve(FRAY_SEG_MAX_NODES * sizeof(uint32_t));
@@ -504,7 +540,7 @@
 }
 inline std::vector<int32_t> arena_editable_tables(const ArenaFacts& F)
 {
-    return {F.tNodes, F.tNodesX, F.tGates, F.tSegPlanes, F.tSegMasks, F.tPlanes, F.tSpheres, F.tCubes, F.tShaders, F.tLayers, F.tLights, F.tTex};
+    return {F.tNodes, F.tNodesX, F.tGates, F.tGatesTight, F.tGuards, F.tSegPlanes, F.tSegMasks, F.tPlanes, F.tSpheres, F.tCubes, F.tShaders, F.tLayers, F.tLights, F.tTex};
 }
 
 inline void arena_place(const ArenaFacts& F, const ArenaMeshTables* meshTables, const int64_t* texelOffset, unsigned char* const* write,
@@ -530,7 +566,9 @@
     S.nodes = (const FRAY_RO DNode*)addr[F.tNodes];
     S.nodesX = (const FRAY_RO DNodeX*)addr[F.tNodesX];
     S.gates = (const FRAY_RO DGate*)addr[F.tGates];
-    S.nGates = F.nGates; S.gatesExact = F.gatesExact;
+    S.gatesTight = (const FRAY_RO DGate*)addr[F.tGatesTight];
+    S.nGates = F.nGates; S.gatesExact = F.gatesExact; S.nTightGates = F.nTightGates; S.nGuardChunks = F.nGuardChunks;
+    S.guards = (const FRAY_RO DGuard*)addr[F.tGuards];
     S.segPlanes = (const FRAY_RO DSegPlane*)addr[F.tSegPlanes];
     S.segNodeMasks = (const FRAY_RO uint32_t*)addr[F.tSegMasks];
     S.nSegPlanes = F.nSegPlanes; S.nSegNodes = F.nSegNodes; S.segCertAll = F.segCertAll;
diff --git a/fray_amd/scene.py b/fray_amd/scene.py
--- a/fray_amd/scene.py
+++ b/fray_amd/scene.py
@@ -583,6 +583,12 @@
         v = C.c_int64(0)
         _check(lib.frayhip_scene_get_option(self._dev, name.encode(), C.byref(v)))
         return int(v.value)
+
+    def gate_figures(self):
+        self._need_dev()
+        v = (C.c_int64 * 4)()
+        _check(lib.frayhip_scene_gate_figures(self._dev, v))
+        return dict(zip(("tight_gates", "tight_gate_count", "rays_filed", "rays_filed_gate_free"), (int(x) for x in v)))
 
     def _frame(self, mode, seed, bucket_first, bucket_stride, spp_chunk, stats):
         return abi.Frame(mode=mode, seed=seed, bucket_first=bucket_first, bucket_stride=bucket_stride,
diff --git a/include/frayhip.h b/include/frayhip.h
--- a/include/frayhip.h
+++ b/include/frayhip.h
@@ -219,6 +219,7 @@
 
 int  frayhip_scene_set_option(frayhip_scene* s, const char* name, int64_t value);
 int  frayhip_scene_get_option(frayhip_scene* s, const char* name, int64_t* value);
+int  frayhip_scene_gate_figures(frayhip_scene* s, int64_t out[4]);
 
 int  frayhip_render(frayhip_scene* s, const frayhip_frame* f,
                     float* rgb, int32_t* hit_id, double* hit_dist, frayhip_stats* st);
```

Measured after the change: 13330 (median of 5 runs). No clear change (+0.1%).
